# alxn3/nbody-llm

Hardware: AMD Instinct MI355X
Metric: pairwise_interactions_per_sec (higher is better)
Workload: dtype f32

## Files before the change

nbody-llm_amd/csrc/kernels.h:

```cpp
#pragma once
#include <hip/hip_runtime.h>
#include <cstdint>
#include <vector>

#include "shard.h"

namespace nbody {

struct Tuning {
    int cross_sym = 1;
    int sym_packed = 1;
    int bf_fast_variant = 0;
    int bh_walk_duo = -1;
    int bh_walk_xcd = 1;
    int let_list_div = 4;
    int sym_ipt = 0;
    int sym_wpb = 4;
    int sym_rounds = 1;
    int sym_k = 0;
    int sym_min_bodies = 1024;
    int sym_reduce_split = 1;
    int sym_opp_rot = 1;
    int cross_slots = 3072;
    int cross_ipt = 0;
    int cross_wpb = 4;
    int bh_walk_split = 0;
    int bh_walk_order = 1;
    int bh_reduce_split = 1;
    int tree_max_tie = 64;
    int bf64_min_bodies = 10240;
    int bf64_ipt = 0;
    int bf64_rot = 0;
    int bf64_waves = 0;
    int bh_walk_variant = 0;
    int bh_walk_lds_block = 1024;
    int bh_hot_cap = 2048;
    int bh_walk_debug = 0;
    int sym_debug = 0;
};
const Tuning& tuning();
struct WalkPlan { int bodies_per_lane; int segments; };
WalkPlan walk_plan(size_t n_order, bool fast_math, int max_segments, float theta2);
void bind_tuning(const Tuning* t);

template <class F>
void launch_aos_to_soa(hipStream_t s, const F* aos, int stride, int n, typename ShardT<F>::V4* pos, typename ShardT<F>::V4* vel,
                       typename ShardT<F>::V4* acc);
template <class F>
void launch_soa_to_aos(hipStream_t s, F* aos, int stride, int n, const typename ShardT<F>::V4* pos, const typename ShardT<F>::V4* vel,
                       const typename ShardT<F>::V4* acc);
template <class F> void launch_drift_half(hipStream_t s, const ShardT<F>& sh, int n_upper, F dt, const typename RealTypes<F>::Bounds& b);
template <class F> void launch_compact(hipStream_t s, const ShardT<F>& sh, int n_upper);
template <class F> void launch_kick_drift(hipStream_t s, const ShardT<F>& sh, int n_upper, F dt);

void launch_bf_forces_strict(hipStream_t s, const Shard& sh, int n_upper, float g, float g_soft2);
void launch_bf_forces_fast(hipStream_t s, const Shard& sh, int n_upper, float g, float g_soft2);

struct SymPlan {
    int ipt = 8;
    int A = 0;
    int K = 0;
    int wpb = 16;
    int res_combine = 0;
    int k_res = 0;
    int sym_sets = 0;
    int opp = 0;
    int n_trav = 0;
    int n_planes = 0;
    int k_os = 0;
    size_t n_pad = 0;
    size_t plane_stride = 0;
    std::vector<int> bounds;
    std::vector<int> bounds_long;
};
SymPlan make_sym_plan(int n_upper);
int sym_bodies_per_lane(size_t n);
uint64_t sym_main_pairs(const SymPlan& p, size_t n);
void launch_bf_sym_main(hipStream_t s, const Shard& sh, const SymPlan& p, const int* d_bounds, float4* planes,
                        int n_upper, float g_soft2);
void launch_bf_os(hipStream_t s, const Shard& sh, int A, int K, float4* planes, size_t plane_stride, float g_soft2);
void launch_bf_sym_tail(hipStream_t s, const Shard& sh, const SymPlan& p, float4* planes, int n_upper, float g,
                        float g_soft2, const float* kick_dt);

struct CrossPartners {
    static constexpr int kMax = 8;
    int n = 0;
    int seg[kMax];
    int c0[kMax], c1[kMax];
    int a0[kMax], a1[kMax];
};
struct CrossPlan {
    static constexpr int kMaxPlanes = 256;
    int ipt = 8;
    int A = 0;
    CrossPartners parts;
    int n_recv = 0;
    int recv_from[CrossPartners::kMax];
    int k_res = 0;
    std::vector<int4> slices;
};
CrossPlan make_cross_plan(int rank, int world, int seg_cap, int n_own_upper);
void launch_bf_cross(hipStream_t s, const Shard& sh, const CrossPlan& p, const int4* d_slices, float4* res_planes,
                     float4* xplanes, float4* send, size_t plane_stride, float g_soft2);

constexpr int kMaxSplit = 64, kMaxAnc = 192;
constexpr size_t kSplitInts = size_t(kMaxSplit) + 1 + kMaxSplit + size_t(kMaxSplit) * kMaxAnc;
struct TreeDev {
    const float4* nodes = nullptr;
    int n_nodes = 0;
    const int* order = nullptr;
    int n_order = 0;
    int n_split = 1;
    const int* split_first = nullptr;
    const int* split_anc = nullptr;
    const int* split_n_anc = nullptr;
    float4* split_planes = nullptr;
    size_t split_stride = 0;
    float4* nested_stack = nullptr;
    size_t nested_stride = 0;
    float4* walk = nullptr;
    float4* hot = nullptr;
    int* unified = nullptr;
    int* hot_info = nullptr;
    int hot_cap = 0;
    int hot_threshold = 0;
    const int* poison = nullptr;
    const int* n_order_dev = nullptr;
    int store_work = 0;
    float4* bfs = nullptr;
    void* bfs_ws = nullptr;
    size_t bfs_cap = 0;
};
struct TreeDevWork {
    const unsigned long long* keys = nullptr;
    const signed char* delta = nullptr;
    const int* base = nullptr;
    const int* ids = nullptr;
    const unsigned long long* keys2 = nullptr;
    const int* wpre = nullptr;
    const void* incl = nullptr;
};
struct TreeCatLists {
    int* flags = nullptr;
    int* base = nullptr;
    int* own_order = nullptr;
    int* info = nullptr;
};
template <class P4>
struct TreeCat : TreeCatLists {
    P4* pos = nullptr;
};
size_t tree_build_workspace_bytes(size_t n_cap);
size_t tree_build_tmp_bytes(size_t n_cap);
inline size_t tree_cat_align(size_t b) { return (b + 255) / 256 * 256; }
template <class P4> size_t tree_cat_bytes(size_t n_cap) { return tree_cat_align(n_cap * sizeof(P4)) + 3 * tree_cat_align(n_cap * 4) + 256; }
template <class P4>
TreeCat<P4> tree_cat_layout(void* buf, size_t n_cap) {
    char* p = static_cast<char*>(buf);
    TreeCat<P4> c;
    c.pos = reinterpret_cast<P4*>(p); p += tree_cat_align(n_cap * sizeof(P4));
    c.flags = reinterpret_cast<int*>(p); p += tree_cat_align(n_cap * 4);
    c.base = reinterpret_cast<int*>(p); p += tree_cat_align(n_cap * 4);
    c.own_order = reinterpret_cast<int*>(p); p += tree_cat_align(n_cap * 4);
    c.info = reinterpret_cast<int*>(p);
    return c;
}
void launch_tree_cat(hipStream_t s, const Shard& sh, const TreeCat<float4>& c);
void launch_tree_cat(hipStream_t s, const ShardT<double>& sh, const TreeCat<double4>& c);
int launch_tree_own_order(hipStream_t s, const int* order, const TreeCatLists& c, int n_total_upper, void* tmp, size_t tmp_bytes);
struct TreeSplitReq { int n_split = 0; int* first = nullptr; int* n_anc = nullptr; int* anc = nullptr; int max_anc = 0; const int* info = nullptr; int* poison = nullptr; };
int build_octree_device(hipStream_t s, const float4* pos, const int* d_count, int n_upper, const float center[3],
                        float width, void* workspace, size_t n_cap, float4* nodes, int node_cap, int* order,
                        int* out_info, TreeDevWork* work, int want_hot = 0 , const TreeSplitReq* split = nullptr);
size_t bfs_workspace_bytes(size_t n_cap);
int build_bfs_layout(hipStream_t s, const float4* nodes, int n_nodes, void* workspace, size_t n_cap, float4* out);
}
namespace nbody64 { struct Node64; }
namespace nbody {
int build_octree_device(hipStream_t s, const double4* pos, const int* d_count, int n_upper, const double center[3], double width,
                        void* workspace, size_t n_cap, nbody64::Node64* nodes, int node_cap, int* order, int* out_info,
                        TreeDevWork* work, int want_hot = 0, const TreeSplitReq* split = nullptr);
int tree_sort_keys(hipStream_t s, const float4* pos, const int* d_count, int n_upper, const float center[3], float width,
                   void* workspace, size_t n_cap, int* out_info, TreeDevWork* work);
int tree_emit_sorted(hipStream_t s, const float4* pos, const int* d_count, int n_upper, float width, void* workspace, size_t n_cap,
                     float4* nodes, int node_cap, int* order, int* out_info, int want_hot, const int* edge, const TreeSplitReq* split = nullptr);
int tree_scan_sorted(hipStream_t s, const float4* pos, const int* d_count, int n_upper, void* workspace, size_t n_cap, int* out_info,
                     const int* edge, const float4* weight_src = nullptr );
__host__ __device__ inline int body_weight(float visits) { const int v = int(visits) >> 4; return v < 1 ? 1 : v; }
int tree_emit_nodes(hipStream_t s, const float4* pos, const int* d_count, int n_upper, float width, void* workspace, size_t n_cap,
                    float4* nodes, int node_cap, int slice_cap, int* order, int* out_info, int want_hot, const int* edge,
                    const int* node_offset, int* parent, unsigned char* depth);
void launch_tree_split_anc(hipStream_t s, const TreeDevWork& work, int n, int n_nodes, int n_split, int* first,
                           int* n_anc, int* anc, int max_anc, const int* info = nullptr ,
                           int* poison = nullptr );

#define NBODY_WALK_COUNTER_SLOTS 1024u
void launch_walk_split_scan(hipStream_t s, const float4* nodes, const int* range, int n_split, int* first, int* n_anc, int* anc, int first_given = 0);
void launch_bh_walk(hipStream_t s, const Shard& sh, const TreeDev& t, float g, float g_soft2, float theta2,
                    int fast_math, unsigned long long* counters , int leaf_direct = 0,
                    const float* kick_dt = nullptr ,
                    int* kicked = nullptr );
void launch_bh_reduce(hipStream_t s, const Shard& sh, const TreeDev& t, int fast_math, const float* kick_dt, int* kicked);

void launch_energy(hipStream_t s, const Shard& sh, int n_upper, double g_soft2, double* out2);

}
```

nbody-llm_amd/csrc/kernels_bf_sym.hip:

```cpp
#include "kernels.h"
#include "bf_pair.h"
#include "real.h"

#include <algorithm>

namespace nbody {

namespace {

#ifdef NBODY_TUNING
__device__ unsigned long long nbody_sym_stamps[3 * 8192];
#endif

}

template <int IPT>
__device__ __forceinline__ void sym_rest_wave(const float4* __restrict__ pos, int n, int A, int opp, int group, int slice,
                                              int n_slices, float& ax, float& ay, float& az, float eps2);

template <int IPT, int NW>
__device__ __forceinline__ void sym_rest_block(const float4* __restrict__ pos, int n, int A, int opp, int group,
                                               float4* __restrict__ plane, float eps2, float (*red)[3][64]);

template <int IPT, int WPB, int DBG = 0, bool PK = false>
__global__ __launch_bounds__(WPB * 64) void k_bf_sym(const float4* __restrict__ pos, const int* __restrict__ count,
                                                     int A, int K, const int* __restrict__ bounds, int n_trav, int opp,
                                                     float4* __restrict__ planes, size_t plane_stride, float eps2,
                                                     int res_combine) {
    const int lane = threadIdx.x & 63;
    const int wslot = __builtin_amdgcn_readfirstlane(threadIdx.x >> 6);
    const int n_main_blocks = (A * K + WPB - 1) / WPB;
    if (int(blockIdx.x) >= n_main_blocks) {
        __shared__ float red[WPB - 1][3][64];
        sym_rest_block<IPT, WPB>(pos, *count, A, opp, blockIdx.x - n_main_blocks,
                                 planes + size_t(n_trav + (res_combine ? K / WPB : K)) * plane_stride, eps2, red);
        return;
    }
    const int gw = blockIdx.x * WPB + (wslot & 3) * (WPB / 4) + (wslot >> 2);
    if (gw >= A * K) return;
    const int a = gw / K;
    const int part = gw - a * K;
    const int n = *count;
    const int Cn = A * IPT;
    const int* __restrict__ cuts = bounds + ((opp && a < (A >> 1)) ? 128 : 0);
    const int k0 = cuts[part], k1 = cuts[part + 1];
    const int src_lane = ((lane + 63) & 63) * 4;
    const int src_lane2 = ((lane + 62) & 63) * 4;
    float eps2v = eps2;
    asm volatile("" : "+v"(eps2v));

    float xi[IPT], yi[IPT], zi[IPT], mi[IPT], axi[IPT], ayi[IPT], azi[IPT];
#pragma unroll
    for (int q = 0; q < IPT; ++q) {
        const int i = (a * IPT + q) * 64 + lane;
        const float4 p = (i < n) ? pos[i] : make_float4(PAD_POS, PAD_POS, PAD_POS, 0.f);
        xi[q] = p.x; yi[q] = p.y; zi[q] = p.z; mi[q] = p.w;
        axi[q] = ayi[q] = azi[q] = 0.f;
    }

    auto chunk_of = [&](int k) {
        int c = (a + 1) * IPT + k;
        if (c >= Cn) c -= Cn;
        return c;
    };
    auto load_chunk = [&](int k) {
        const int j = chunk_of(k) * 64 + lane;
        return (j < n) ? pos[j] : make_float4(PAD_POS, PAD_POS, PAD_POS, 0.f);
    };

    [[maybe_unused]] unsigned long long t_beg = 0, r_beg = 0;
    if (DBG & 4) { t_beg = __builtin_amdgcn_s_memtime(); r_beg = __builtin_amdgcn_s_memrealtime(); }
    float4 nxt = (k0 < k1) ? load_chunk(k0) : make_float4(0.f, 0.f, 0.f, 0.f);
    v2f xi2[IPT / 2], yi2[IPT / 2], zi2[IPT / 2], mi2[IPT / 2], axi2[IPT / 2], ayi2[IPT / 2], azi2[IPT / 2];
    if (PK) {
        pack_pairs<IPT>(xi, xi2); pack_pairs<IPT>(yi, yi2); pack_pairs<IPT>(zi, zi2); pack_pairs<IPT>(mi, mi2);
        pack_pairs<IPT>(axi, axi2); pack_pairs<IPT>(ayi, ayi2); pack_pairs<IPT>(azi, azi2);
    }
    for (int k = k0; k < k1; ++k) {
        float xj = nxt.x, yj = nxt.y, zj = nxt.z, mj = nxt.w;
        float axj = 0.f, ayj = 0.f, azj = 0.f;
        v2f axj2 = {0.f, 0.f}, ayj2 = {0.f, 0.f}, azj2 = {0.f, 0.f};
        if (k + 1 < k1) nxt = load_chunk(k + 1);
        switch ((4 * (k1 - k) - 1) / (k1 - k0)) {
            case 3: __builtin_amdgcn_s_setprio(3); break;
            case 2: __builtin_amdgcn_s_setprio(2); break;
            case 1: __builtin_amdgcn_s_setprio(1); break;
            default: __builtin_amdgcn_s_setprio(0); break;
        }
        if (PK) {
            for (int s = 0; s < 64; s += 2) {
                const float x1 = rotl(xj, src_lane), y1 = rotl(yj, src_lane), z1 = rotl(zj, src_lane), m1 = rotl(mj, src_lane);
                pair_evals_pk<IPT / 2, DBG>(xi2, yi2, zi2, mi2, axi2, ayi2, azi2, xj, yj, zj, mj, axj2, ayj2, azj2, eps2v);
                axj2.x = rotl(axj2.x, src_lane); ayj2.x = rotl(ayj2.x, src_lane); azj2.x = rotl(azj2.x, src_lane);
                axj2.y = rotl(axj2.y, src_lane); ayj2.y = rotl(ayj2.y, src_lane); azj2.y = rotl(azj2.y, src_lane);
                xj = rotl(x1, src_lane); yj = rotl(y1, src_lane); zj = rotl(z1, src_lane); mj = rotl(m1, src_lane);
                pair_evals_pk<IPT / 2, DBG>(xi2, yi2, zi2, mi2, axi2, ayi2, azi2, x1, y1, z1, m1, axj2, ayj2, azj2, eps2v);
                axj2.x = rotl(axj2.x, src_lane); ayj2.x = rotl(ayj2.x, src_lane); azj2.x = rotl(azj2.x, src_lane);
                axj2.y = rotl(axj2.y, src_lane); ayj2.y = rotl(ayj2.y, src_lane); azj2.y = rotl(azj2.y, src_lane);
            }
        } else {
            float x1 = rotl(xj, src_lane), y1 = rotl(yj, src_lane), z1 = rotl(zj, src_lane), m1 = rotl(mj, src_lane);
#pragma unroll 2
            for (int s = 0; s < 64; ++s) {
                const float x2 = rotl(xj, src_lane2), y2 = rotl(yj, src_lane2), z2 = rotl(zj, src_lane2), m2 = rotl(mj, src_lane2);
                pair_evals<IPT, DBG>(xi, yi, zi, mi, axi, ayi, azi, xj, yj, zj, mj, axj, ayj, azj, eps2v);
                axj = rotl(axj, src_lane); ayj = rotl(ayj, src_lane); azj = rotl(azj, src_lane);
                xj = x1; yj = y1; zj = z1; mj = m1;
                x1 = x2; y1 = y2; z1 = z2; m1 = m2;
            }
        }
        if (PK) { axj = axj2.x + axj2.y; ayj = ayj2.x + ayj2.y; azj = azj2.x + azj2.y; }
        const int d = k / IPT + 1;
        planes[size_t(d - 1) * plane_stride + size_t(chunk_of(k)) * 64 + lane] = make_float4(axj, ayj, azj, 0.f);
    }
    if (PK) { unpack_pairs<IPT>(axi2, axi); unpack_pairs<IPT>(ayi2, ayi); unpack_pairs<IPT>(azi2, azi); }

#ifdef NBODY_TUNING
    if (DBG & 4) {
        const unsigned long long t_end = __builtin_amdgcn_s_memtime(), r_end = __builtin_amdgcn_s_memrealtime();
        if (lane == 0 && gw < 8192) {
            nbody_sym_stamps[gw * 3 + 0] = t_end - t_beg;
            nbody_sym_stamps[gw * 3 + 1] = r_end - r_beg;
            const unsigned hw = __builtin_amdgcn_s_getreg((4 ) | (0 << 6) | (31 << 11));
            const unsigned xcc = __builtin_amdgcn_s_getreg((20 ) | (0 << 6) | (31 << 11));
            nbody_sym_stamps[gw * 3 + 2] = (unsigned long long)(k1 - k0) | ((unsigned long long)hw << 16) | ((unsigned long long)(xcc & 0xF) << 48);
        }
    }
#endif
    if (res_combine) {
        __shared__ float comb[WPB - 1][3 * IPT][64];
        const int first_part = (part / WPB) * WPB;
        const int rel = part - first_part;
        if (rel > 0) {
#pragma unroll
            for (int q = 0; q < IPT; ++q) {
                comb[rel - 1][3 * q + 0][lane] = axi[q];
                comb[rel - 1][3 * q + 1][lane] = ayi[q];
                comb[rel - 1][3 * q + 2][lane] = azi[q];
            }
        }
        __syncthreads();
        if (rel == 0) {
            float4* __restrict__ out = planes + size_t(n_trav + part / WPB) * plane_stride;
#pragma unroll
            for (int q = 0; q < IPT; ++q) {
                float sx = axi[q], sy = ayi[q], sz = azi[q];
                for (int w = 0; w < WPB - 1; ++w) { sx += comb[w][3 * q + 0][lane]; sy += comb[w][3 * q + 1][lane]; sz += comb[w][3 * q + 2][lane]; }
                out[size_t(a * IPT + q) * 64 + lane] = make_float4(sx, sy, sz, 0.f);
            }
        }
        return;
    }
    float4* __restrict__ out = planes + size_t(n_trav + part) * plane_stride;
#pragma unroll
    for (int q = 0; q < IPT; ++q) out[size_t(a * IPT + q) * 64 + lane] = make_float4(axi[q], ayi[q], azi[q], 0.f);
}

template <int IPT, int WPB, bool PK>
__global__ __launch_bounds__(WPB * 64) void k_bf_os(const float4* __restrict__ pos_all,
                                                    const int* __restrict__ seg_count, int n_seg, int seg_cap,
                                                    int my_seg, int A, int K, float4* __restrict__ planes,
                                                    size_t plane_stride, float eps2) {
    __shared__ float4 stage[WPB][2][64];
    const int lane = threadIdx.x & 63;
    const int wslot = __builtin_amdgcn_readfirstlane(threadIdx.x >> 6);
    const int gw = blockIdx.x * WPB + (wslot & 3) * (WPB / 4) + (wslot >> 2);
    if (gw >= A * K) return;
    const int a = gw / K, part = gw - a * K;
    const int n_own = seg_count[my_seg];
    const float4* __restrict__ own = pos_all + size_t(my_seg) * seg_cap;
    float eps2v = eps2;
    asm volatile("" : "+v"(eps2v));

    float xi[IPT], yi[IPT], zi[IPT], mi[IPT], axi[IPT], ayi[IPT], azi[IPT];
#pragma unroll
    for (int q = 0; q < IPT; ++q) {
        const int i = (a * IPT + q) * 64 + lane;
        const float4 p = (i < n_own) ? own[i] : make_float4(PAD_POS, PAD_POS, PAD_POS, 0.f);
        xi[q] = p.x; yi[q] = p.y; zi[q] = p.z; mi[q] = p.w;
        axi[q] = ayi[q] = azi[q] = 0.f;
    }
    long long R = 0;
    for (int s = 0; s < n_seg; ++s) if (s != my_seg) R += seg_count[s];
    const long long r0 = R * part / K, r1 = R * (part + 1) / K;
    long long seg_first = 0;
    float dummy_x = 0.f, dummy_y = 0.f, dummy_z = 0.f;
    v2f dummy2 = {0.f, 0.f};
    v2f xi2[IPT / 2], yi2[IPT / 2], zi2[IPT / 2], mi2[IPT / 2], axi2[IPT / 2], ayi2[IPT / 2], azi2[IPT / 2];
    if (PK) {
        pack_pairs<IPT>(xi, xi2); pack_pairs<IPT>(yi, yi2); pack_pairs<IPT>(zi, zi2); pack_pairs<IPT>(mi, mi2);
        pack_pairs<IPT>(axi, axi2); pack_pairs<IPT>(ayi, ayi2); pack_pairs<IPT>(azi, azi2);
    }
    for (int s = 0; s < n_seg; ++s) {
        if (s == my_seg) continue;
        const int ns = seg_count[s];
        const long long lo = r0 > seg_first ? r0 : seg_first;
        const long long hi = r1 < seg_first + ns ? r1 : seg_first + ns;
        const float4* __restrict__ ps = pos_all + size_t(s) * seg_cap - seg_first;
        int buf = 0;
        if (lo < hi) {
            const long long j = lo + lane;
            stage[wslot][0][lane] = (j < hi) ? ps[j] : make_float4(PAD_POS, PAD_POS, PAD_POS, 0.f);
        }
        for (long long c0 = lo; c0 < hi; c0 += 64) {
            const long long jn = c0 + 64 + lane;
            float4 nxt = make_float4(PAD_POS, PAD_POS, PAD_POS, 0.f);
            if (c0 + 64 < hi && jn < hi) nxt = ps[jn];
            const int cnt = int(hi - c0 < 64 ? hi - c0 : 64);
            switch (int((4 * (r1 - c0) - 1) / (r1 - r0))) {
                case 3: __builtin_amdgcn_s_setprio(3); break;
                case 2: __builtin_amdgcn_s_setprio(2); break;
                case 1: __builtin_amdgcn_s_setprio(1); break;
                default: __builtin_amdgcn_s_setprio(0); break;
            }
            float4 pj = stage[wslot][buf][0];
            for (int t = 0; t < cnt; ++t) {
                const float4 pn = stage[wslot][buf][(t + 1) & 63];
                if (PK)
                    pair_evals_pk<IPT / 2, 0, false>(xi2, yi2, zi2, mi2, axi2, ayi2, azi2, pj.x, pj.y, pj.z, pj.w, dummy2,
                                                     dummy2, dummy2, eps2v);
                else
                    pair_evals<IPT, 0, false>(xi, yi, zi, mi, axi, ayi, azi, pj.x, pj.y, pj.z, pj.w, dummy_x, dummy_y,
                                              dummy_z, eps2v);
                pj = pn;
            }
            buf ^= 1;
            stage[wslot][buf][lane] = nxt;
        }
        seg_first += ns;
    }
    if (PK) { unpack_pairs<IPT>(axi2, axi); unpack_pairs<IPT>(ayi2, ayi); unpack_pairs<IPT>(azi2, azi); }
    float4* __restrict__ out = planes + size_t(part) * plane_stride;
#pragma unroll
    for (int q = 0; q < IPT; ++q) out[size_t(a * IPT + q) * 64 + lane] = make_float4(axi[q], ayi[q], azi[q], 0.f);
}

template <int IPT>
__device__ __forceinline__ void sym_rest_wave(const float4* __restrict__ pos, int n, int A, int opp, int group, int slice,
                                              int n_slices, float& ax, float& ay, float& az, float eps2) {
    constexpr int SET = 64 * IPT;
    const int lane = threadIdx.x & 63;
    const int i = group * 64 + lane;
    const int a = (group * 64) / SET;
    const float4 pi = (i < n) ? pos[i] : make_float4(PAD_POS, PAD_POS, PAD_POS, 0.f);
    ax = ay = az = 0.f;
    const int n_win = (A % 2 == 0 && A > 1 && !opp) ? 2 : 1;
    for (int w = 0; w < n_win; ++w) {
        int set = (w == 0) ? a : a + A / 2;
        if (set >= A) set -= A;
        const int j0 = set * SET + SET * slice / n_slices;
        const int j1 = min(n, set * SET + SET * (slice + 1) / n_slices);
#pragma unroll 8
        for (int j = j0; j < j1; ++j) {
            const float4 pj = pos[j];
            const float dx = pj.x - pi.x, dy = pj.y - pi.y, dz = pj.z - pi.z;
            const float r2 = __builtin_fmaf(dz, dz, __builtin_fmaf(dy, dy, __builtin_fmaf(dx, dx, eps2)));
            const float rinv = __builtin_amdgcn_rsqf(r2);
            float sj = pj.w * ((rinv * rinv) * rinv);
            sj = (j == i) ? 0.f : sj;
            ax = __builtin_fmaf(dx, sj, ax);
            ay = __builtin_fmaf(dy, sj, ay);
            az = __builtin_fmaf(dz, sj, az);
        }
    }
}

template <int IPT, int NW>
__device__ __forceinline__ void sym_rest_block(const float4* __restrict__ pos, int n, int A, int opp, int group,
                                               float4* __restrict__ plane, float eps2, float (*red)[3][64]) {
    const int lane = threadIdx.x & 63;
    const int wv = __builtin_amdgcn_readfirstlane(threadIdx.x >> 6);
    float ax, ay, az;
    sym_rest_wave<IPT>(pos, n, A, opp, group, wv, NW, ax, ay, az, eps2);
    if (wv > 0) { red[wv - 1][0][lane] = ax; red[wv - 1][1][lane] = ay; red[wv - 1][2][lane] = az; }
    __syncthreads();
    if (wv == 0) {
#pragma unroll
        for (int w = 0; w < NW - 1; ++w) { ax += red[w][0][lane]; ay += red[w][1][lane]; az += red[w][2][lane]; }
        plane[group * 64 + lane] = make_float4(ax, ay, az, 0.f);
    }
}

template <int IPT>
__global__ __launch_bounds__(512) void k_bf_sym_rest(const float4* __restrict__ pos, const int* __restrict__ count,
                                                     int A, float4* __restrict__ plane, float eps2) {
    __shared__ float red[7][3][64];
    sym_rest_block<IPT, 8>(pos, *count, A, 0, blockIdx.x, plane, eps2, red);
}

template <bool KICK>
__global__ __launch_bounds__(256) void k_bf_sym_reduce(const float4* __restrict__ planes, int n_planes,
                                                       size_t plane_stride, const int* __restrict__ count, float g,
                                                       float4* __restrict__ acc, float4* __restrict__ pos,
                                                       float4* __restrict__ vel, float dt, const int* __restrict__ seg_count,
                                                       int n_seg, unsigned long long* __restrict__ inter, int opp_plane,
                                                       int opp_first) {
    const int i = blockIdx.x * 256 + threadIdx.x;
    if (inter && i == 0) {
        long long tot = 0;
        for (int s = 0; s < n_seg; ++s) tot += seg_count[s];
        if (tot > 0) atomicAdd(inter, (unsigned long long)(*count) * (unsigned long long)(tot - 1));
    }
    if (i >= *count) return;
    float sx = 0.f, sy = 0.f, sz = 0.f, cx = 0.f, cy = 0.f, cz = 0.f;
    for (int p = 0; p < n_planes; ++p) {
        if (p == opp_plane && i < opp_first) continue;
        const float4 v = planes[size_t(p) * plane_stride + i];
        const float yx = v.x - cx, yy = v.y - cy, yz = v.z - cz;
        const float tx = sx + yx, ty = sy + yy, tz = sz + yz;
        cx = (tx - sx) - yx; cy = (ty - sy) - yy; cz = (tz - sz) - yz;
        sx = tx; sy = ty; sz = tz;
    }
    const float4 a = make_float4(g * sx, g * sy, g * sz, 0.f);
    acc[i] = a;
    if (KICK) kick_half_drift(pos, vel, i, a.x, a.y, a.z, dt);
}

template <bool KICK, int Q>
__global__ __launch_bounds__(64 * Q) void k_bf_sym_reduce_split(const float4* __restrict__ planes, int n_planes, size_t plane_stride,
                                                                const int* __restrict__ count, float g, float4* __restrict__ acc,
                                                                float4* __restrict__ pos, float4* __restrict__ vel, float dt,
                                                                const int* __restrict__ seg_count, int n_seg,
                                                                unsigned long long* __restrict__ inter, int opp_plane, int opp_first) {
    __shared__ float part[Q][3][64];
    const int lane = threadIdx.x & 63, q = threadIdx.x >> 6;
    const int i = blockIdx.x * 64 + lane;
    if (inter && blockIdx.x == 0 && threadIdx.x == 0) {
        long long tot = 0;
        for (int s = 0; s < n_seg; ++s) tot += seg_count[s];
        if (tot > 0) atomicAdd(inter, (unsigned long long)(*count) * (unsigned long long)(tot - 1));
    }
    const int n = *count;
    float sx = 0.f, sy = 0.f, sz = 0.f, cx = 0.f, cy = 0.f, cz = 0.f;
    if (i < n) {
        const int p0 = int((long long)n_planes * q / Q), p1 = int((long long)n_planes * (q + 1) / Q);
        for (int p = p0; p < p1; ++p) {
            if (p == opp_plane && i < opp_first) continue;
            const float4 v = planes[size_t(p) * plane_stride + i];
            const float yx = v.x - cx, yy = v.y - cy, yz = v.z - cz;
            const float tx = sx + yx, ty = sy + yy, tz = sz + yz;
            cx = (tx - sx) - yx; cy = (ty - sy) - yy; cz = (tz - sz) - yz;
            sx = tx; sy = ty; sz = tz;
        }
    }
    part[q][0][lane] = sx; part[q][1][lane] = sy; part[q][2][lane] = sz;
    __syncthreads();
    if (q != 0 || i >= n) return;
    sx = sy = sz = cx = cy = cz = 0.f;
    for (int w = 0; w < Q; ++w) {
        const float yx = part[w][0][lane] - cx, yy = part[w][1][lane] - cy, yz = part[w][2][lane] - cz;
        const float tx = sx + yx, ty = sy + yy, tz = sz + yz;
        cx = (tx - sx) - yx; cy = (ty - sy) - yy; cz = (tz - sz) - yz;
        sx = tx; sy = ty; sz = tz;
    }
    const float4 a = make_float4(g * sx, g * sy, g * sz, 0.f);
    acc[i] = a;
    if (KICK) kick_half_drift(pos, vel, i, a.x, a.y, a.z, dt);
}

}
#ifdef NBODY_TUNING
namespace nbody { int read_sym_stamps(unsigned long long* out, int n_waves); }
extern "C" int nbody_sym_read_stamps(unsigned long long* out, int n_waves) { return nbody::read_sym_stamps(out, n_waves); }
#endif
namespace nbody {

int sym_bodies_per_lane(size_t n) {
    const Tuning& t = tuning();
    if (!t.sym_packed || t.sym_wpb != 4 || t.sym_ipt == 8) return 8;
    if (t.sym_ipt == 4) return 4;
    return n <= 10240 ? 4 : 8;
}

SymPlan make_sym_plan(int n_upper) {
    SymPlan p;
    const int IPT = sym_bodies_per_lane(size_t(n_upper));
    p.ipt = IPT;
    p.A = (n_upper + 64 * IPT - 1) / (64 * IPT);
    p.sym_sets = (p.A + 1) / 2 - 1;
    const int L = IPT * p.sym_sets;
    const int want = tuning().sym_wpb;
    p.wpb = want == 8 ? 8 : want == 12 ? 12 : want == 16 ? 16 : 4;
    int K = 1;
    if (p.wpb == 4) {
        K = L <= 100 ? L : L <= 160 ? (L + 1) / 2 : 64;
    } else {
        const int resident_wgs_per_cu = (p.wpb == 8) ? 2 : 1;
        const int slots = 256 * resident_wgs_per_cu * p.wpb;
        double best = 0.0;
        const int k_hi = std::min(126, std::min(L, std::max(1, slots * std::max(1, tuning().sym_rounds) * 4 / p.A)));
        for (int k = 1; k <= k_hi; ++k) {
            const long long waves = (long long)p.A * k;
            const long long rounds = (waves + slots - 1) / slots;
            if (rounds > 4 * std::max(1, tuning().sym_rounds) && k > 1) break;
            const double fill = double(waves) / double(rounds * slots);
            const double even = (L % k == 0) ? 1.0 : double(L / k) / double(L / k + 1);
            const double per_wave = double(L) / k / (double(L) / k + 0.3);
            if (fill * even * per_wave > best + 1e-9) { best = fill * even * per_wave; K = k; }
        }
    }
    if (tuning().sym_k > 0) K = std::min(126, tuning().sym_k);
    if (K > L) K = L;
    if (K < 1) K = 1;
    p.K = K;
    p.res_combine = (K % p.wpb == 0) ? 1 : 0;
    p.k_res = p.res_combine ? K / p.wpb : K;
    p.opp = (tuning().sym_opp_rot && p.A % 2 == 0 && p.sym_sets >= 1) ? 1 : 0;
    p.n_trav = p.sym_sets + p.opp;
    p.n_planes = p.n_trav + p.k_res + 1;
    p.n_pad = size_t(p.A) * 64 * IPT;
    p.plane_stride = p.n_pad;
    p.bounds.resize(K + 1);
    for (int part = 0; part <= K; ++part) p.bounds[part] = int((long long)L * part / K);
    const int L_long = L + (p.opp ? IPT : 0);
    p.bounds_long.resize(K + 1);
    for (int part = 0; part <= K; ++part) p.bounds_long[part] = int((long long)L_long * part / K);
    return p;
}

#ifdef NBODY_TUNING
int read_sym_stamps(unsigned long long* out, int n_waves) {
    return hipMemcpyFromSymbol(out, HIP_SYMBOL(nbody_sym_stamps), sizeof(unsigned long long) * 3 * n_waves) == hipSuccess ? 0 : -1;
}
#endif

uint64_t sym_main_pairs(const SymPlan& p, size_t n) {
    const size_t set = size_t(64) * p.ipt;
    auto size_of = [&](int a) { size_t lo = size_t(a) * set; return lo >= n ? size_t(0) : std::min(set, n - lo); };
    uint64_t pairs = 0;
    for (int a = 0; a < p.A; ++a)
        for (int d = 1; d <= p.sym_sets; ++d) pairs += uint64_t(size_of(a)) * uint64_t(size_of((a + d) % p.A));
    if (p.opp)
        for (int a = 0; a < p.A / 2; ++a) pairs += uint64_t(size_of(a)) * uint64_t(size_of(a + p.A / 2));
    return pairs;
}

void launch_bf_sym_main(hipStream_t s, const Shard& sh, const SymPlan& p, const int* d_bounds, float4* planes,
                        int n_upper, float g_soft2) {
    if (n_upper <= 0 || p.sym_sets <= 0) return;
    const int main_blocks = (p.A * p.K + p.wpb - 1) / p.wpb;
    const int rest_blocks = int(p.n_pad / 64);
    const dim3 grid(main_blocks + rest_blocks), block(p.wpb * 64);
#define SYM_LAUNCH(WPB, DBG) hipLaunchKernelGGL((k_bf_sym<8, WPB, DBG, PKV>), grid, block, 0, s, sh.own_pos(), sh.own_count(), p.A, p.K, d_bounds, p.n_trav, p.opp, planes, p.plane_stride, g_soft2, p.res_combine)
#ifdef NBODY_TUNING
    const int dbg = tuning().sym_debug;
#else
    constexpr int dbg = 0;
#endif
    if (p.ipt == 4) {
        hipLaunchKernelGGL((k_bf_sym<4, 4, 0, true>), grid, block, 0, s, sh.own_pos(), sh.own_count(), p.A, p.K, d_bounds, p.n_trav, p.opp, planes, p.plane_stride, g_soft2, p.res_combine);
        return;
    }
    if (tuning().sym_packed) {
        constexpr bool PKV = true;
        if (dbg == 4) {
#ifdef NBODY_TUNING
            if (p.wpb == 12) SYM_LAUNCH(12, 4); else if (p.wpb == 8) SYM_LAUNCH(8, 4); else if (p.wpb == 4) SYM_LAUNCH(4, 4); else SYM_LAUNCH(16, 4);
#endif
        } else {
            if (p.wpb == 12) SYM_LAUNCH(12, 0); else if (p.wpb == 8) SYM_LAUNCH(8, 0); else if (p.wpb == 4) SYM_LAUNCH(4, 0); else SYM_LAUNCH(16, 0);
        }
    } else {
        constexpr bool PKV = false;
        if (dbg >= 4 && dbg <= 7) {
#ifdef NBODY_TUNING
            if (dbg == 4) { if (p.wpb == 12) SYM_LAUNCH(12, 4); else if (p.wpb == 8) SYM_LAUNCH(8, 4); else if (p.wpb == 4) SYM_LAUNCH(4, 4); else SYM_LAUNCH(16, 4); }
            else if (dbg == 5) SYM_LAUNCH(16, 5);
            else if (dbg == 6) SYM_LAUNCH(16, 6);
            else SYM_LAUNCH(16, 7);
#endif
        } else {
            if (p.wpb == 12) SYM_LAUNCH(12, 0); else if (p.wpb == 8) SYM_LAUNCH(8, 0); else if (p.wpb == 4) SYM_LAUNCH(4, 0); else SYM_LAUNCH(16, 0);
        }
    }
#undef SYM_LAUNCH
}

void launch_bf_os(hipStream_t s, const Shard& sh, int A, int K, float4* planes, size_t plane_stride, float g_soft2) {
    if (A <= 0 || K <= 0) return;
    const int wpb = 12;
    if (tuning().sym_packed)
        hipLaunchKernelGGL((k_bf_os<8, 12, true>), dim3((A * K + wpb - 1) / wpb), dim3(wpb * 64), 0, s, sh.pos_all,
                           sh.seg_count, sh.n_seg, sh.seg_cap, sh.my_seg, A, K, planes, plane_stride, g_soft2);
    else
        hipLaunchKernelGGL((k_bf_os<8, 12, false>), dim3((A * K + wpb - 1) / wpb), dim3(wpb * 64), 0, s, sh.pos_all,
                           sh.seg_count, sh.n_seg, sh.seg_cap, sh.my_seg, A, K, planes, plane_stride, g_soft2);
}

void launch_bf_sym_tail(hipStream_t s, const Shard& sh, const SymPlan& p, float4* planes, int n_upper, float g,
                        float g_soft2, const float* kick_dt) {
    if (n_upper <= 0) return;
    if (p.sym_sets == 0) {
        float4* resident0 = planes + size_t(p.n_trav) * p.plane_stride;
        (void)hipMemsetAsync(resident0, 0, size_t(p.k_res) * p.plane_stride * sizeof(float4), s);
        if (p.ipt == 4)
            hipLaunchKernelGGL(k_bf_sym_rest<4>, dim3(int(p.n_pad / 64)), dim3(512), 0, s, sh.own_pos(),
                               sh.own_count(), p.A, planes + size_t(p.n_trav + p.k_res) * p.plane_stride, g_soft2);
        else
        hipLaunchKernelGGL(k_bf_sym_rest<8>, dim3(int(p.n_pad / 64)), dim3(512), 0, s, sh.own_pos(),
                           sh.own_count(), p.A, planes + size_t(p.n_trav + p.k_res) * p.plane_stride, g_soft2);
    }
    const float dt = kick_dt ? *kick_dt : 0.f;
#define REDUCE_ARGS planes, p.n_planes, p.plane_stride, sh.own_count(), g, sh.acc, sh.own_pos(), sh.vel, dt, sh.seg_count, sh.n_seg, sh.inter, (p.opp ? p.n_trav - 1 : -1), int(p.n_pad / 2)
    if (tuning().sym_reduce_split && p.n_planes >= 16) {
        const dim3 grid((n_upper + 63) / 64);
        if (n_upper <= 16384) {
            if (kick_dt) hipLaunchKernelGGL((k_bf_sym_reduce_split<true, 16>), grid, dim3(1024), 0, s, REDUCE_ARGS);
            else hipLaunchKernelGGL((k_bf_sym_reduce_split<false, 16>), grid, dim3(1024), 0, s, REDUCE_ARGS);
        } else {
            if (kick_dt) hipLaunchKernelGGL((k_bf_sym_reduce_split<true, 4>), grid, dim3(256), 0, s, REDUCE_ARGS);
            else hipLaunchKernelGGL((k_bf_sym_reduce_split<false, 4>), grid, dim3(256), 0, s, REDUCE_ARGS);
        }
    } else {
        const dim3 grid((n_upper + 255) / 256);
        if (kick_dt) hipLaunchKernelGGL(k_bf_sym_reduce<true>, grid, dim3(256), 0, s, REDUCE_ARGS);
        else hipLaunchKernelGGL(k_bf_sym_reduce<false>, grid, dim3(256), 0, s, REDUCE_ARGS);
    }
#undef REDUCE_ARGS
}

}
```

nbody-llm_amd/csrc/kernels_integrate.hip:

```cpp
#include "real.h"
#include "retain.h"

#include <algorithm>

namespace nbody {

template <class F>
__global__ __launch_bounds__(256) void k_aos_to_soa(const F* __restrict__ aos, int stride, int n, typename Real<F>::V4* __restrict__ pos,
                                                    typename Real<F>::V4* __restrict__ vel, typename Real<F>::V4* __restrict__ acc) {
    const int k = blockIdx.x * 256 + threadIdx.x;
    if (k >= n) return;
    const F* p = aos + size_t(k) * stride;
    pos[k] = Real<F>::make4(p[0], p[1], p[2], p[9]);
    if (vel) vel[k] = Real<F>::make4(p[3], p[4], p[5], F(0));
    if (acc) acc[k] = Real<F>::make4(p[6], p[7], p[8], F(0));
}

template <class F>
__global__ __launch_bounds__(256) void k_soa_to_aos(F* __restrict__ aos, int stride, int n, const typename Real<F>::V4* __restrict__ pos,
                                                    const typename Real<F>::V4* __restrict__ vel,
                                                    const typename Real<F>::V4* __restrict__ acc) {
    const int k = blockIdx.x * 256 + threadIdx.x;
    if (k >= n) return;
    const typename Real<F>::V4 p = pos[k], v = vel[k], a = acc[k];
    F* o = aos + size_t(k) * stride;
    o[0] = p.x; o[1] = p.y; o[2] = p.z;
    o[3] = v.x; o[4] = v.y; o[5] = v.z;
    o[6] = a.x; o[7] = a.y; o[8] = a.z;
    o[9] = p.w;
}

template <class F>
__global__ __launch_bounds__(256) void k_drift_half(typename Real<F>::V4* __restrict__ pos, const typename Real<F>::V4* __restrict__ vel,
                                                    const int* __restrict__ count, unsigned char* __restrict__ keep,
                                                    int* __restrict__ escaped, F dt, typename Real<F>::Bounds b,
                                                    const int* __restrict__ poison) {
    if (poison && *poison) return;
    const int k = blockIdx.x * 256 + threadIdx.x;
    if (k >= *count) return;
    typename Real<F>::V4 p = pos[k];
    const typename Real<F>::V4 v = vel[k];
    p.x += (v.x * Real<F>::half) * dt;
    p.y += (v.y * Real<F>::half) * dt;
    p.z += (v.z * Real<F>::half) * dt;
    pos[k] = p;
    const bool in = (p.x >= b.lo[0]) && (p.x <= b.hi[0]) && (p.y >= b.lo[1]) && (p.y <= b.hi[1]) &&
                    (p.z >= b.lo[2]) && (p.z <= b.hi[2]);
    keep[k] = in ? 1 : 0;
    if (!in) atomicAdd(escaped, 1);
}

template <class F>
__global__ __launch_bounds__(256) void k_kick_drift(typename Real<F>::V4* __restrict__ pos, typename Real<F>::V4* __restrict__ vel,
                                                    const typename Real<F>::V4* __restrict__ acc, const int* __restrict__ count,
                                                    F dt, int* __restrict__ poison) {
    if (poison && *poison) return;
    const int k = blockIdx.x * 256 + threadIdx.x;
    if (k == 0 && poison) atomicAdd(poison + 1, 1);
    if (k >= *count) return;
    typename Real<F>::V4 p = pos[k], v = vel[k];
    const typename Real<F>::V4 a = acc[k];
    v.x += a.x * dt;
    v.y += a.y * dt;
    v.z += a.z * dt;
    p.x += (v.x * Real<F>::half) * dt;
    p.y += (v.y * Real<F>::half) * dt;
    p.z += (v.z * Real<F>::half) * dt;
    vel[k] = v;
    pos[k] = p;
}

template <class F>
__global__ __launch_bounds__(kCompactTile) void k_compact(typename Real<F>::V4* __restrict__ pos, typename Real<F>::V4* __restrict__ vel,
                                                          typename Real<F>::V4* __restrict__ acc, const unsigned char* __restrict__ keep,
                                                          int* __restrict__ count, int* __restrict__ escaped,
                                                          unsigned long long* __restrict__ tile_state, int* __restrict__ epoch_p,
                                                          const int* __restrict__ poison, int* __restrict__ ids) {
    if (poison && *poison) return;
    if (*escaped == 0) return;
    typename Real<F>::V4 p = Real<F>::make4(0, 0, 0, 0), v = p, a = p;
    int id = 0;
    retain_tile(keep, count, escaped, tile_state, epoch_p,
                [&](int k) { p = pos[k]; v = vel[k]; a = acc[k]; if (ids) id = ids[k]; },
                [&](int d) { pos[d] = p; vel[d] = v; acc[d] = a; if (ids) ids[d] = id; });
}

static inline int blocks_for(int n, int bs) { return n <= 0 ? 0 : (n + bs - 1) / bs; }

template <class F>
void launch_aos_to_soa(hipStream_t s, const F* aos, int stride, int n, typename ShardT<F>::V4* pos, typename ShardT<F>::V4* vel,
                       typename ShardT<F>::V4* acc) {
    if (n <= 0) return;
    hipLaunchKernelGGL(k_aos_to_soa<F>, dim3(blocks_for(n, 256)), dim3(256), 0, s, aos, stride, n, pos, vel, acc);
}
template <class F>
void launch_soa_to_aos(hipStream_t s, F* aos, int stride, int n, const typename ShardT<F>::V4* pos, const typename ShardT<F>::V4* vel,
                       const typename ShardT<F>::V4* acc) {
    if (n <= 0) return;
    hipLaunchKernelGGL(k_soa_to_aos<F>, dim3(blocks_for(n, 256)), dim3(256), 0, s, aos, stride, n, pos, vel, acc);
}
template <class F>
void launch_drift_half(hipStream_t s, const ShardT<F>& sh, int n_upper, F dt, const typename RealTypes<F>::Bounds& b) {
    if (n_upper <= 0) return;
    hipLaunchKernelGGL(k_drift_half<F>, dim3(blocks_for(n_upper, 256)), dim3(256), 0, s, sh.own_pos(), sh.vel, sh.own_count(), sh.keep,
                       sh.escaped, dt, b, sh.poison);
}
template <class F>
void launch_compact(hipStream_t s, const ShardT<F>& sh, int n_upper) {
    if (n_upper <= 0) return;
    hipLaunchKernelGGL(k_compact<F>, dim3(blocks_for(n_upper, kCompactTile)), dim3(kCompactTile), 0, s, sh.own_pos(), sh.vel, sh.acc,
                       sh.keep, sh.own_count(), sh.escaped, sh.tile_state, sh.epoch, sh.poison, sh.ids);
}
template <class F>
void launch_kick_drift(hipStream_t s, const ShardT<F>& sh, int n_upper, F dt) {
    const int blocks = blocks_for(n_upper, 256);
    if (blocks == 0 && !sh.poison) return;
    hipLaunchKernelGGL(k_kick_drift<F>, dim3(std::max(1, blocks)), dim3(256), 0, s, sh.own_pos(), sh.vel, sh.acc, sh.own_count(), dt,
                       sh.poison);
}

#define NBODY_INTEGRATE_LAUNCHERS(F, V4)                                                                              \
    template void launch_aos_to_soa<F>(hipStream_t, const F*, int, int, V4*, V4*, V4*);                               \
    template void launch_soa_to_aos<F>(hipStream_t, F*, int, int, const V4*, const V4*, const V4*);                   \
    template void launch_drift_half<F>(hipStream_t, const ShardT<F>&, int, F, const RealTypes<F>::Bounds&);           \
    template void launch_compact<F>(hipStream_t, const ShardT<F>&, int);                                              \
    template void launch_kick_drift<F>(hipStream_t, const ShardT<F>&, int, F);
NBODY_INTEGRATE_LAUNCHERS(float, float4)
NBODY_INTEGRATE_LAUNCHERS(double, double4)
#undef NBODY_INTEGRATE_LAUNCHERS

}

namespace nbody64 {
void launch_aos_to_pos(hipStream_t s, const double* aos, int stride_d, int n, double4* pos) {
    nbody::launch_aos_to_soa<double>(s, aos, stride_d, n, pos, nullptr, nullptr);
}
}
```

nbody-llm_amd/csrc/nbody_api.cpp:

```cpp
#include "nbody_engine.h"
#include "nbody_let.h"
#include "nbody_pot.h"
#include "nbody_field.h"
#include "nbody_tracer.h"
#include "nbody_external.h"
#include "nbody_diag.h"
#include "nbody_pairs.h"
#include "nbody_fof.h"
#include "nbody_cells.h"

#include <algorithm>
#include <chrono>
#include <cmath>
#include <cstdio>
#include <cstdlib>
#include <cstring>
#include <memory>
#include <string>
#include <thread>
#include <vector>


static thread_local std::string g_create_err;

int fail(NbodyHandle* h, int code, const std::string& msg) {
    if (h) h->err = msg; else g_create_err = msg;
    return code;
}

int comm_check(NbodyHandle* h) {
    if (!h->tp) return NBODY_OK;
    int rc = h->tp->check();
    return rc ? fail(h, rc, h->tp->error()) : NBODY_OK;
}

namespace {

int use_device(NbodyHandle* h) {
    nbody::bind_tuning(&h->tune);
    HIP_TRY(h, hipSetDevice(h->device));
    return NBODY_OK;
}

int check_stride(NbodyHandle* h, size_t stride) {
    const size_t e = h->f64 ? sizeof(double) : sizeof(float);
    if (stride >= 10 * e && stride % e == 0) return NBODY_OK;
    return fail(h, NBODY_ERR_INVALID, h->f64 ? "f64 handle: stride must be a multiple of 8 and >= 80 bytes" : "stride must be a multiple of 4 and >= 40 bytes");
}

const char* tree_quadrupole_refusal(const NbodyHandle* h) {
    if (h->cfg.method != NBODY_BARNES_HUT) return "this mode needs a Barnes-Hut handle (brute-force handles have no tree to expand)";
    if (h->f64 || h->cfg.dtype != NBODY_F32) return "this mode is not possible on NBODY_F64 handles (the cells' tensors exist for NBODY_F32)";
    if (h->let || h->cfg.shard_mode != NBODY_SHARD_INDEX) return "this mode is not possible on NBODY_SHARD_SPATIAL handles";
    if (h->cfg.world_size != 1) return "this mode is not possible on handles of a multi-rank world (world_size > 1)";
    return nullptr;
}

int potentials_device(NbodyHandle* h, int mode, size_t* n_own, nbody::PotBodies* bodies, double* g, bool field = false) {
    if (mode != NBODY_POTENTIAL_PAIRS && mode != NBODY_POTENTIAL_TREE && mode != NBODY_POTENTIAL_TREE_QUADRUPOLE)
        return fail(h, NBODY_ERR_INVALID, "mode must be NBODY_POTENTIAL_PAIRS, NBODY_POTENTIAL_TREE or NBODY_POTENTIAL_TREE_QUADRUPOLE");
    if (mode == NBODY_POTENTIAL_TREE_QUADRUPOLE)
        if (const char* why = tree_quadrupole_refusal(h)) return fail(h, NBODY_ERR_INVALID, std::string("NBODY_POTENTIAL_TREE_QUADRUPOLE: ") + why);
    if (h->let && field)
        return fail(h, NBODY_ERR_INVALID, "nbody_field_at is not possible on NBODY_SHARD_SPATIAL handles: a rank holds neither the world's bodies nor the tree around a foreign point");
    if (h->let && mode == NBODY_POTENTIAL_PAIRS)
        return fail(h, NBODY_ERR_INVALID, "NBODY_POTENTIAL_PAIRS is not possible on NBODY_SHARD_SPATIAL handles (a rank does not hold the world's bodies): NBODY_POTENTIAL_TREE is the mode for them");
    if (mode != NBODY_POTENTIAL_PAIRS && h->cfg.method != NBODY_BARNES_HUT) return fail(h, NBODY_ERR_INVALID, "NBODY_POTENTIAL_TREE needs a Barnes-Hut handle");
    if (h->f64) return nbody64::potentials_device(h, mode, n_own, bodies, g, field);
    return nbody32::potentials_device(h, mode, n_own, bodies, g, field);
}

void free_all(NbodyHandle* h) {
    if (!h) return;
    (void)hipSetDevice(h->device);
    if (h->stream) (void)hipStreamSynchronize(h->stream);
    if (h->comm_stream) (void)hipStreamSynchronize(h->comm_stream);
    h->tp.reset();
    if (h->ev_drifted) (void)hipEventDestroy(h->ev_drifted);
    if (h->ev_gathered) (void)hipEventDestroy(h->ev_gathered);
    if (h->comm_stream) (void)hipStreamDestroy(h->comm_stream);
    for (auto& ev : h->ev_pending) { (void)hipEventDestroy(ev.first); (void)hipEventDestroy(ev.second); }
    for (auto& ev : h->ev_free) { (void)hipEventDestroy(ev.first); (void)hipEventDestroy(ev.second); }
    nbody::let::destroy(h);
    nbody32::destroy(h);
    nbody64::destroy(h);
    h->mem.release_all();
    if (h->stream) (void)hipStreamDestroy(h->stream);
    delete h;
}

int create_impl(const NbodyConfig* cfg, NbodyHandle** out) {
    if (!cfg || !out) return fail(nullptr, NBODY_ERR_INVALID, "null argument");
    constexpr uint32_t kOldConfigSize = 48;
    NbodyConfig full{};
    if (cfg->struct_size == kOldConfigSize) { std::memcpy(&full, cfg, kOldConfigSize); full.struct_size = sizeof(NbodyConfig); cfg = &full; }
    if (cfg->struct_size != sizeof(NbodyConfig)) return fail(nullptr, NBODY_ERR_INVALID, "NbodyConfig.struct_size mismatch");
    if (cfg->shard_mode != NBODY_SHARD_INDEX && cfg->shard_mode != NBODY_SHARD_SPATIAL) return fail(nullptr, NBODY_ERR_INVALID, "unknown shard_mode");
    if (cfg->shard_mode == NBODY_SHARD_SPATIAL && (cfg->method != NBODY_BARNES_HUT || cfg->math_mode != NBODY_MATH_FAST || cfg->dtype != NBODY_F32))
        return fail(nullptr, NBODY_ERR_INVALID, "NBODY_SHARD_SPATIAL is the fast-math f32 Barnes-Hut path (halo exchange over the device-built tree)");
    if (cfg->method != NBODY_BRUTE_FORCE && cfg->method != NBODY_BARNES_HUT) return fail(nullptr, NBODY_ERR_INVALID, "unknown method");
    if (cfg->math_mode != NBODY_MATH_STRICT && cfg->math_mode != NBODY_MATH_FAST) return fail(nullptr, NBODY_ERR_INVALID, "unknown math_mode");
    if (cfg->leaf_mode != NBODY_LEAF_REFERENCE && cfg->leaf_mode != NBODY_LEAF_DIRECT) return fail(nullptr, NBODY_ERR_INVALID, "unknown leaf_mode");
    if (cfg->tree_build != NBODY_TREE_HOST && cfg->tree_build != NBODY_TREE_DEVICE && cfg->tree_build != NBODY_TREE_AUTO)
        return fail(nullptr, NBODY_ERR_INVALID, "unknown tree_build");
    if (cfg->world_size < 1 || cfg->rank < 0 || cfg->rank >= cfg->world_size) return fail(nullptr, NBODY_ERR_INVALID, "bad rank/world_size");
    if (cfg->capacity == 0 || cfg->capacity > (1ull << 30)) return fail(nullptr, NBODY_ERR_INVALID, "capacity must be in [1, 2^30]");
    if (cfg->dtype != NBODY_F32 && cfg->dtype != NBODY_F64) return fail(nullptr, NBODY_ERR_INVALID, "unknown dtype");
    if (cfg->dtype == NBODY_F64 && cfg->world_size != 1 && cfg->shard_mode != NBODY_SHARD_INDEX)
        return fail(nullptr, NBODY_ERR_INVALID, "f64 worlds are sharded by index blocks (NBODY_SHARD_INDEX)");

    int ndev = 0;
    if (hipGetDeviceCount(&ndev) != hipSuccess || ndev <= 0)
        return fail(nullptr, NBODY_ERR_NO_DEVICE, "no HIP device (this library has no CPU fallback)");
    int dev = cfg->device;
    if (dev < 0) {
        const char* lr = std::getenv("LOCAL_RANK");
        dev = lr ? std::atoi(lr) % ndev : 0;
    }
    if (dev >= ndev) return fail(nullptr, NBODY_ERR_INVALID, "device ordinal out of range");

    NbodyHandle* h = new NbodyHandle();
    h->cfg = *cfg;
    if (h->cfg.tree_build == NBODY_TREE_AUTO)
        h->cfg.tree_build = cfg->math_mode == NBODY_MATH_FAST ? NBODY_TREE_DEVICE : NBODY_TREE_HOST;
    if (h->cfg.dtype == NBODY_F64) {
        if (cfg->tree_build == NBODY_TREE_AUTO) h->cfg.tree_build = h->cfg.math_mode == NBODY_MATH_FAST ? NBODY_TREE_DEVICE : NBODY_TREE_HOST;
        if (cfg->world_size > 1 && h->cfg.math_mode != NBODY_MATH_FAST) h->cfg.tree_build = NBODY_TREE_HOST;
    }
    if (h->cfg.shard_mode == NBODY_SHARD_SPATIAL) h->cfg.tree_build = NBODY_TREE_DEVICE;
    cfg = &h->cfg;
    h->device = dev;
    *out = nullptr;
    auto bail = [&](int rc) { g_create_err = h->err; free_all(h); return rc; };
#define CREATE_TRY(expr)                                                                                  \
    do {                                                                                                  \
        const int rc_ = [&] { HIP_TRY(h, expr); return int(NBODY_OK); }();                                \
        if (rc_) return bail(rc_);                                                                        \
    } while (0)
    CREATE_TRY(hipSetDevice(dev));
    CREATE_TRY(hipStreamCreateWithFlags(&h->stream, hipStreamNonBlocking));
    CREATE_TRY(h->mem.pin(h->h_poison, 8 * sizeof(int)));
    if (cfg->method == NBODY_BARNES_HUT) {
        int threads = cfg->host_threads > 0 ? cfg->host_threads : std::min(16, std::max(1, int(std::thread::hardware_concurrency()) - 2));
        h->pool.reset(new nbody::WorkerPool(std::max(1, threads)));
        CREATE_TRY(h->mem.dev(h->d_counters, 2 * NBODY_WALK_COUNTER_SLOTS * sizeof(unsigned long long)));
        CREATE_TRY(hipMemsetAsync(h->d_counters, 0, 2 * NBODY_WALK_COUNTER_SLOTS * sizeof(unsigned long long), h->stream));
        CREATE_TRY(h->mem.pin(h->h_counters, 2 * NBODY_WALK_COUNTER_SLOTS * sizeof(unsigned long long)));
    }
#undef CREATE_TRY
    ShardShape& sh = h->shape;
    sh.n_seg = cfg->world_size;
    sh.my_seg = cfg->rank;
    sh.seg_cap = int((cfg->capacity + cfg->world_size - 1) / cfg->world_size);
    if (cfg->dtype == NBODY_F64) {
        int rc64 = nbody64::create(h);
        if (rc64) return bail(rc64);
        *out = h;
        return NBODY_OK;
    }
    const bool spatial = cfg->shard_mode == NBODY_SHARD_SPATIAL;
    if (spatial) {
        sh.n_seg = 1;
        sh.my_seg = 0;
        if (cfg->world_size > 1) sh.seg_cap = int(std::min<uint64_t>(cfg->capacity, 4 * uint64_t(sh.seg_cap) + 64));
    }
    {
        int rc = nbody32::create(h);
        if (rc) return bail(rc);
    }
    if (spatial) {
        int rc_let = nbody::let::create(h);
        if (rc_let) return bail(rc_let);
    }
    {
        nbody::Tuning& t = h->tune;
        const struct { const char* env; int* knob; } table[] = {
            {"NBODY_BF_VARIANT", &t.bf_fast_variant}, {"NBODY_CROSS_SYM", &t.cross_sym}, {"NBODY_SYM_PACKED", &t.sym_packed},
            {"NBODY_BH_SPLIT", &t.bh_walk_split}, {"NBODY_SYM_WPB", &t.sym_wpb}, {"NBODY_SYM_IPT", &t.sym_ipt}, {"NBODY_BH_DUO", &t.bh_walk_duo}, {"NBODY_BH_XCD", &t.bh_walk_xcd},
#ifdef NBODY_TUNING
            {"NBODY_BH_VARIANT", &t.bh_walk_variant}, {"NBODY_BH_HOT", &t.bh_hot_cap}, {"NBODY_BH_LDS_BLOCK", &t.bh_walk_lds_block},
#endif
        };
        for (const auto& e : table)
            if (const char* v = std::getenv(e.env)) *e.knob = std::atoi(v);
    }
    *out = h;
    return NBODY_OK;
}

}

extern "C" {

int nbody_abi_version(void) { return NBODY_ABI_VERSION; }

int nbody_device_count(void) {
    int n = 0;
    if (hipGetDeviceCount(&n) != hipSuccess) return 0;
    return n;
}

const char* nbody_last_error(const NbodyHandle* h) { return h ? h->err.c_str() : g_create_err.c_str(); }

int nbody_create(const NbodyConfig* cfg, NbodyHandle** out) { return create_impl(cfg, out); }

void nbody_destroy(NbodyHandle* h) { free_all(h); }

int nbody_clone(const NbodyHandle* src, NbodyHandle** out) {
    if (!src || !out) return fail(nullptr, NBODY_ERR_INVALID, "null argument");
    NbodyHandle* s = const_cast<NbodyHandle*>(src);
    int rc = use_device(s);
    if (rc) return rc;
    rc = nbody32::resolve_async(s);
    if (rc) return rc;
    NbodyHandle* h = nullptr;
    rc = create_impl(&src->cfg, &h);
    if (rc) return rc;
    h->tune = src->tune;
    h->ext = src->ext;
    if (src->f64) rc = nbody64::clone_state(s, h);
    else {
        rc = nbody32::clone_state(s, h);
        if (!rc && src->let) rc = nbody::let::clone_state(s, h);
        if (!rc) rc = nbody::tracer::clone_state(s, h);
    }
    if (rc) { g_create_err = h->err; free_all(h); return rc; }
    *out = h;
    return NBODY_OK;
}

int nbody_upload(NbodyHandle* h, const void* aos, size_t n, size_t stride) {
    if (!h || (!aos && n)) return fail(h, NBODY_ERR_INVALID, "null argument");
    int rc = check_stride(h, stride);
    if (rc) return rc;
    if (n > h->cfg.capacity) return fail(h, NBODY_ERR_CAPACITY, "more bodies than NbodyConfig.capacity");
    rc = use_device(h);
    if (rc) return rc;
    if (h->f64) return nbody64::upload(h, aos, n, stride);
    if (h->let) return nbody::let::upload(h, aos, n, stride);
    return nbody32::upload(h, aos, n, stride);
}

int nbody_download(NbodyHandle* h, void* aos, size_t cap, size_t stride, size_t* n_out) {
    if (!h) return NBODY_ERR_INVALID;
    int rc = check_stride(h, stride);
    if (rc) return rc;
    rc = use_device(h);
    if (rc) return rc;
    if (h->f64) return nbody64::download(h, aos, cap, stride, n_out);
    return nbody32::download(h, aos, cap, stride, n_out);
}

int nbody_count(NbodyHandle* h, size_t* n_out) {
    if (!h || !n_out) return NBODY_ERR_INVALID;
    int rc = use_device(h);
    if (rc) return rc;
    if (h->f64) return nbody64::count(h, n_out);
    return nbody32::count(h, n_out);
}

int nbody_count_global(NbodyHandle* h, size_t* n_out) {
    if (!h || !n_out) return NBODY_ERR_INVALID;
    int rc = use_device(h);
    if (rc) return rc;
    if (h->f64) return nbody64::count_global(h, n_out);
    if (h->let) return nbody::let::count_global(h, n_out);
    return nbody32::count_global(h, n_out);
}

int nbody_add_point(NbodyHandle* h, const void* particle) {
    if (!h || !particle) return NBODY_ERR_INVALID;
    int rc = use_device(h);
    if (rc) return rc;
    if (h->f64) return nbody64::add_point(h, particle);
    if (h->let) return nbody::let::add_point(h, particle);
    return nbody32::add_point(h, particle);
}

int nbody_remove_point(NbodyHandle* h, size_t index) {
    if (!h) return NBODY_ERR_INVALID;
    int rc = use_device(h);
    if (rc) return rc;
    if (h->f64) return nbody64::remove_point(h, index);
    if (h->let) return nbody::let::remove_point(h, index);
    return nbody32::remove_point(h, index);
}

int nbody_set_settings_f64(NbodyHandle* h, double g, double g_soft, double dt, double theta2) {
    if (!h) return NBODY_ERR_INVALID;
    if (h->f64) return nbody64::set_settings(h, g, g_soft, dt, theta2);
    nbody32::bodies(h).set_settings(float(g), float(g_soft), float(dt), float(theta2));
    return NBODY_OK;
}

int nbody_set_settings(NbodyHandle* h, float g, float g_soft, float dt, float theta2) {
    return nbody_set_settings_f64(h, double(g), double(g_soft), double(dt), double(theta2));
}

int nbody_get_settings_f64(const NbodyHandle* h, double* g, double* g_soft, double* dt, double* theta2) {
    if (!h) return NBODY_ERR_INVALID;
    return with_bodies(h, [&](const auto& b) { b.get_settings(g, g_soft, dt, theta2); return int(NBODY_OK); });
}

int nbody_get_settings(const NbodyHandle* h, float* g, float* g_soft, float* dt, float* theta2) {
    if (!h) return NBODY_ERR_INVALID;
    return with_bodies(h, [&](const auto& b) { b.get_settings(g, g_soft, dt, theta2); return int(NBODY_OK); });
}

int nbody_set_bounds_f64(NbodyHandle* h, const double center[3], double width) {
    if (!h || !center) return NBODY_ERR_INVALID;
    if (h->f64) return nbody64::set_bounds(h, center, width);
    const float c[3] = {float(center[0]), float(center[1]), float(center[2])};
    nbody32::bodies(h).set_bounds(c, float(width));
    return NBODY_OK;
}

int nbody_set_bounds(NbodyHandle* h, const float center[3], float width) {
    if (!h || !center) return NBODY_ERR_INVALID;
    const double c[3] = {double(center[0]), double(center[1]), double(center[2])};
    return nbody_set_bounds_f64(h, c, double(width));
}

int nbody_init(NbodyHandle* h) {
    if (!h) return NBODY_ERR_INVALID;
    if (h->f64) return nbody64::init(h);
    return nbody32::init(h);
}

int nbody_step_by(NbodyHandle* h, float dt) {
    if (!h) return NBODY_ERR_INVALID;
    int rc = use_device(h);
    if (rc) return rc;
    if (h->f64) return nbody64::step_by(h, double(dt));
    if (h->let) return nbody::let::step(h, dt);
    return nbody32::step_by(h, dt);
}

int nbody_step_by_f64(NbodyHandle* h, double dt) {
    if (!h) return NBODY_ERR_INVALID;
    int rc = use_device(h);
    if (rc) return rc;
    if (h->f64) return nbody64::step_by(h, dt);
    if (h->let) return nbody::let::step(h, float(dt));
    return nbody32::step_by(h, float(dt));
}

int nbody_steps(NbodyHandle* h, int k) {
    if (!h || k < 0) return NBODY_ERR_INVALID;
    int rc = use_device(h);
    if (rc) return rc;
    if (h->f64) return nbody64::steps(h, k);
    if (h->let) {
        for (int i = 0; i < k; ++i) { rc = nbody::let::step(h, nbody32::bodies(h).dt); if (rc) return rc; }
        return NBODY_OK;
    }
    return nbody32::steps(h, k);
}

int nbody_update_forces(NbodyHandle* h) {
    if (!h) return NBODY_ERR_INVALID;
    int rc = use_device(h);
    if (rc) return rc;
    if (h->f64) return nbody64::update_forces(h);
    if (h->let) return nbody32::bodies(h).bounds_set ? nbody::let::update_forces(h) : fail(h, NBODY_ERR_INVALID, "nbody_set_bounds has not been called");
    return nbody32::update_forces(h);
}

namespace {
int external_enter(NbodyHandle* h, const char* call) {
    int rc = use_device(h);
    if (rc) return rc;
    if (const char* why = nbody::ext::refusal(h)) return fail(h, NBODY_ERR_INVALID, std::string(call) + ": " + why);
    return nbody32::resolve_async(h);
}
double g_of(const NbodyHandle* h) { return with_bodies(h, [](const auto& b) { return double(b.g); }); }
int external_potentials(NbodyHandle* h, bool want_phi, double* phi, size_t cap, size_t* n_out, double* energy, const char* call) {
    return with_bodies(h, [&](auto& b) {
        const int rc = b.sync_count(h, h->stream);
        if (rc) return rc;
        const size_t n = b.n_local;
        if (n_out) *n_out = n;
        if (want_phi && n > cap) return fail(h, NBODY_ERR_CAPACITY, std::string(call) + ": buffer too small");
        if (want_phi && n && !phi) return fail(h, NBODY_ERR_INVALID, std::string(call) + ": phi is NULL");
        return nbody::ext::potentials(h, b.sh, n, double(b.g), phi, energy);
    });
}
}

int nbody_set_external_field(NbodyHandle* h, const NbodyExternalComponent* comps, size_t n) {
    if (!h) return NBODY_ERR_INVALID;
    int rc = external_enter(h, "nbody_set_external_field");
    if (rc) return rc;
    const std::string why = nbody::ext::invalid(comps, n, !h->f64);
    if (!why.empty()) return fail(h, NBODY_ERR_INVALID, "nbody_set_external_field: " + why);
    if (n > 0 && h->f64 && nbody64::get_integrator(h) == NBODY_INTEGRATOR_HERMITE4)
        return fail(h, NBODY_ERR_INVALID, "nbody_set_external_field: the handle runs the Hermite integrator, which would need the field's jerk (out of scope)");
    h->ext = ExternalField{};
    h->ext.n = int(n);
    std::copy(comps, comps + n, h->ext.given);
    return NBODY_OK;
}

int nbody_get_external_field(const NbodyHandle* h, NbodyExternalComponent* comps, size_t cap, size_t* n_out) {
    if (!h) return NBODY_ERR_INVALID;
    NbodyHandle* hh = const_cast<NbodyHandle*>(h);
    if (const char* why = nbody::ext::refusal(h)) return fail(hh, NBODY_ERR_INVALID, std::string("nbody_get_external_field: ") + why);
    const size_t n = size_t(h->ext.n);
    if (n_out) *n_out = n;
    if (n > cap) return fail(hh, NBODY_ERR_CAPACITY, "nbody_get_external_field: buffer too small");
    if (n && !comps) return fail(hh, NBODY_ERR_INVALID, "nbody_get_external_field: comps is NULL");
    std::copy(h->ext.given, h->ext.given + n, comps);
    return NBODY_OK;
}

int nbody_external_potentials(NbodyHandle* h, double* phi, size_t cap, size_t* n_out) {
    if (!h) return NBODY_ERR_INVALID;
    int rc = external_enter(h, "nbody_external_potentials");
    if (rc) return rc;
    return external_potentials(h, true, phi, cap, n_out, nullptr, "nbody_external_potentials");
}

int nbody_external_energy(NbodyHandle* h, double* potential) {
    if (!h) return NBODY_ERR_INVALID;
    int rc = external_enter(h, "nbody_external_energy");
    if (rc) return rc;
    if (!potential) return fail(h, NBODY_ERR_INVALID, "nbody_external_energy: potential is NULL");
    return external_potentials(h, false, nullptr, 0, nullptr, potential, "nbody_external_energy");
}

int nbody_external_at(NbodyHandle* h, const double* xyz, size_t n_points, double* acc, double* phi) {
    if (!h) return NBODY_ERR_INVALID;
    int rc = external_enter(h, "nbody_external_at");
    if (rc) return rc;
    if (n_points > (size_t(1) << 30)) return fail(h, NBODY_ERR_INVALID, "nbody_external_at: n_points must not exceed 2^30");
    if (!xyz && n_points > 0) return fail(h, NBODY_ERR_INVALID, "nbody_external_at: xyz is NULL");
    return nbody::ext::at(h, g_of(h), xyz, n_points, acc, phi);
}

namespace {
int diag_enter(NbodyHandle* h, const char* call) {
    int rc = use_device(h);
    if (rc) return rc;
    if (const char* why = nbody::diag::refusal(h)) return fail(h, NBODY_ERR_INVALID, std::string(call) + ": " + why);
    return nbody32::resolve_async(h);
}
}

int nbody_moments(NbodyHandle* h, double out[10]) {
    if (!h) return NBODY_ERR_INVALID;
    int rc = diag_enter(h, "nbody_moments");
    if (rc) return rc;
    if (!out) return fail(h, NBODY_ERR_INVALID, "nbody_moments: out is NULL");
    return with_bodies(h, [&](auto& b) { return nbody::diag::moments(h, b.sh, b.n_local, out); });
}

int nbody_lagrangian_radii(NbodyHandle* h, const double center[3], const double* fractions, size_t n_frac, double* radii, double* mass_out) {
    if (!h) return NBODY_ERR_INVALID;
    int rc = diag_enter(h, "nbody_lagrangian_radii");
    if (rc) return rc;
    if (n_frac > (size_t(1) << 20)) return fail(h, NBODY_ERR_INVALID, "nbody_lagrangian_radii: n_frac must not exceed 2^20");
    if (n_frac > 0 && !fractions) return fail(h, NBODY_ERR_INVALID, "nbody_lagrangian_radii: fractions is NULL");
    if (n_frac > 0 && !radii) return fail(h, NBODY_ERR_INVALID, "nbody_lagrangian_radii: radii is NULL");
    for (size_t k = 0; k < n_frac; ++k)
        if (!(fractions[k] >= 0.0 && fractions[k] <= 1.0))
            return fail(h, NBODY_ERR_INVALID, "nbody_lagrangian_radii: fraction " + std::to_string(k) + " is not in [0, 1]");
    return with_bodies(h, [&](auto& b) { return nbody::diag::lagrangian_radii(h, b.sh, b.n_local, center, fractions, n_frac, radii, mass_out); });
}

int nbody_partners(NbodyHandle* h, int32_t* partner, double* energy, size_t cap, size_t* n_out) {
    if (!h) return NBODY_ERR_INVALID;
    int rc = diag_enter(h, "nbody_partners");
    if (rc) return rc;
    return with_bodies(h, [&](auto& b) { return nbody::pairs::partners(h, b.sh, b.n_local, double(b.g), double(b.g_soft), partner, energy, cap, n_out); });
}

int nbody_bound_pairs(NbodyHandle* h, NbodyBoundPair* pairs, size_t cap, size_t* n_pairs, double* binding_sum) {
    if (!h) return NBODY_ERR_INVALID;
    int rc = diag_enter(h, "nbody_bound_pairs");
    if (rc) return rc;
    return with_bodies(h, [&](auto& b) { return nbody::pairs::bound_pairs(h, b.sh, b.n_local, double(b.g), double(b.g_soft), pairs, cap, n_pairs, binding_sum); });
}

namespace {
int contact_radius(NbodyHandle* h, const char* call, double radius) {
    if (std::isfinite(radius) && radius > 0.0) return NBODY_OK;
    return fail(h, NBODY_ERR_INVALID, std::string(call) + ": radius must be finite and > 0");
}
}

int nbody_nearest(NbodyHandle* h, int32_t* nearest, double* dist2, size_t cap, size_t* n_out) {
    if (!h) return NBODY_ERR_INVALID;
    int rc = diag_enter(h, "nbody_nearest");
    if (rc) return rc;
    return with_bodies(h, [&](auto& b) { return nbody::pairs::nearest(h, b.sh, b.n_local, nearest, dist2, cap, n_out); });
}

int nbody_contacts(NbodyHandle* h, double radius, NbodyContact* list, size_t cap, size_t* n_contacts) {
    if (!h) return NBODY_ERR_INVALID;
    int rc = diag_enter(h, "nbody_contacts");
    if (!rc) rc = contact_radius(h, "nbody_contacts", radius);
    if (rc) return rc;
    return with_bodies(h, [&](auto& b) { return nbody::pairs::contacts(h, b.sh, b.n_local, radius, list, cap, n_contacts); });
}

int nbody_merge_contacts(NbodyHandle* h, double radius, NbodyContact* list, size_t cap, size_t* n_contacts) {
    if (!h) return NBODY_ERR_INVALID;
    int rc = diag_enter(h, "nbody_merge_contacts");
    if (!rc) rc = contact_radius(h, "nbody_merge_contacts", radius);
    if (rc) return rc;
    if (h->f64) return nbody64::merge_contacts(h, radius, list, cap, n_contacts);
    return nbody32::merge_contacts(h, radius, list, cap, n_contacts);
}

namespace {
int fof_enter(NbodyHandle* h, const char* call, double linking_length) {
    int rc = diag_enter(h, call);
    if (rc) return rc;
    if (std::isfinite(linking_length) && linking_length > 0.0) return NBODY_OK;
    return fail(h, NBODY_ERR_INVALID, std::string(call) + ": linking_length must be finite and > 0");
}
}

int nbody_fof_labels(NbodyHandle* h, double linking_length, int32_t* label, size_t cap, size_t* n_out, size_t* n_groups_out) {
    if (!h) return NBODY_ERR_INVALID;
    int rc = fof_enter(h, "nbody_fof_labels", linking_length);
    if (rc) return rc;
    return with_bodies(h, [&](auto& b) { return nbody::fof::labels(h, b.sh, b.n_local, linking_length, label, cap, n_out, n_groups_out); });
}

int nbody_fof_groups(NbodyHandle* h, double linking_length, int min_members, NbodyGroup* groups, size_t group_cap, size_t* n_groups,
                     int32_t* members, size_t member_cap, size_t* n_members) {
    if (!h) return NBODY_ERR_INVALID;
    int rc = fof_enter(h, "nbody_fof_groups", linking_length);
    if (rc) return rc;
    if (min_members < 1) return fail(h, NBODY_ERR_INVALID, "nbody_fof_groups: min_members must be >= 1");
    return with_bodies(h, [&](auto& b) {
        return nbody::fof::groups(h, b.sh, b.n_local, linking_length, min_members, groups, group_cap, n_groups, members, member_cap, n_members);
    });
}

namespace {
int search_refusal(NbodyHandle* h, const char* call) {
    if (const char* why = nbody::diag::refusal(h)) return fail(h, NBODY_ERR_INVALID, std::string(call) + ": " + why);
    return NBODY_OK;
}
}

int nbody_set_pair_search(NbodyHandle* h, int mode) {
    if (!h) return NBODY_ERR_INVALID;
    if (int rc = search_refusal(h, "nbody_set_pair_search")) return rc;
    if (mode != NBODY_SEARCH_ALL_PAIRS && mode != NBODY_SEARCH_CELLS)
        return fail(h, NBODY_ERR_INVALID, "nbody_set_pair_search: mode must be NBODY_SEARCH_ALL_PAIRS (0) or NBODY_SEARCH_CELLS (1)");
    h->search.mode = mode;
    return NBODY_OK;
}

int nbody_get_pair_search(const NbodyHandle* h, int* mode) {
    if (!h) return NBODY_ERR_INVALID;
    NbodyHandle* hh = const_cast<NbodyHandle*>(h);
    if (int rc = search_refusal(hh, "nbody_get_pair_search")) return rc;
    if (!mode) return fail(hh, NBODY_ERR_INVALID, "nbody_get_pair_search: mode is NULL");
    *mode = h->search.mode;
    return NBODY_OK;
}

int nbody_pair_search_stats(NbodyHandle* h, uint64_t out[4]) {
    if (!h) return NBODY_ERR_INVALID;
    if (int rc = search_refusal(h, "nbody_pair_search_stats")) return rc;
    if (!out) return fail(h, NBODY_ERR_INVALID, "nbody_pair_search_stats: out is NULL");
    std::copy(h->search.last, h->search.last + 4, out);
    return NBODY_OK;
}

int nbody_host_cell_grid(const double* xyz, size_t n, double length, double lo[3], double* side, uint64_t* key, int* usable) {
    if ((!xyz && n) || !lo || !side || !usable) return NBODY_ERR_INVALID;
    if (!(std::isfinite(length) && length > 0.0)) return NBODY_ERR_INVALID;
    nbody::cells::Grid g;
    (void)nbody::cells::host_grid(xyz, n, 3, length, &g, key);
    std::copy(g.lo, g.lo + 3, lo);
    *side = g.side;
    *usable = g.usable;
    return NBODY_OK;
}

namespace {
int tracer_enter(NbodyHandle* h, const char* call) {
    int rc = use_device(h);
    if (rc) return rc;
    if (const char* why = nbody::tracer::refusal(h)) return fail(h, NBODY_ERR_INVALID, std::string(call) + ": " + why);
    return nbody32::resolve_async(h);
}
}

int nbody_tracers_upload(NbodyHandle* h, const void* aos, size_t n, size_t stride, size_t capacity) {
    if (!h) return NBODY_ERR_INVALID;
    int rc = tracer_enter(h, "nbody_tracers_upload");
    if (rc) return rc;
    if (!aos && n) return fail(h, NBODY_ERR_INVALID, "nbody_tracers_upload: null argument");
    if (stride < 40 || stride % 4) return fail(h, NBODY_ERR_INVALID, "nbody_tracers_upload: stride must be a multiple of 4 and >= 40 bytes");
    return nbody::tracer::upload(h, aos, n, stride, capacity);
}

int nbody_tracers_download(NbodyHandle* h, void* aos, size_t cap, size_t stride, size_t* n_out) {
    if (!h) return NBODY_ERR_INVALID;
    int rc = tracer_enter(h, "nbody_tracers_download");
    if (rc) return rc;
    if (stride < 40 || stride % 4) return fail(h, NBODY_ERR_INVALID, "nbody_tracers_download: stride must be a multiple of 4 and >= 40 bytes");
    return nbody::tracer::download(h, aos, cap, stride, n_out);
}

int nbody_tracers_count(NbodyHandle* h, size_t* n_out) {
    if (!h) return NBODY_ERR_INVALID;
    int rc = tracer_enter(h, "nbody_tracers_count");
    if (rc) return rc;
    if (!n_out) return fail(h, NBODY_ERR_INVALID, "nbody_tracers_count: null argument");
    return nbody::tracer::count(h, n_out);
}

int nbody_tracer_stats(NbodyHandle* h, uint64_t out[2]) {
    if (!h) return NBODY_ERR_INVALID;
    int rc = tracer_enter(h, "nbody_tracer_stats");
    if (rc) return rc;
    if (!out) return fail(h, NBODY_ERR_INVALID, "nbody_tracer_stats: null argument");
    return nbody::tracer::stats(h, out);
}

int nbody_host_tracer_plan(size_t n_tracers, size_t n_bodies, int out[4]) {
    if (!out) return NBODY_ERR_INVALID;
    const nbody::TracerPlan p = nbody::tracer_plan(n_tracers, n_bodies);
    out[0] = p.ipt; out[1] = p.groups; out[2] = p.K; out[3] = p.slice_len;
    return NBODY_OK;
}

int nbody_elapsed(const NbodyHandle* h, float* out) {
    if (!h || !out) return NBODY_ERR_INVALID;
    *out = with_bodies(h, [](const auto& b) { return float(b.elapsed); });
    return NBODY_OK;
}

int nbody_elapsed_f64(const NbodyHandle* h, double* out) {
    if (!h || !out) return NBODY_ERR_INVALID;
    *out = with_bodies(h, [](const auto& b) { return double(b.elapsed); });
    return NBODY_OK;
}

int nbody_sync(NbodyHandle* h) {
    if (!h) return NBODY_ERR_INVALID;
    int rc = use_device(h);
    if (rc) return rc;
    rc = nbody32::resolve_async(h);
    if (rc) return rc;
    HIP_TRY(h, hipStreamSynchronize(h->stream));
    return comm_check(h);
}

int nbody_set_profiling(NbodyHandle* h, int on) {
    if (!h) return NBODY_ERR_INVALID;
    h->profiling = on != 0;
    h->profile_every = on > 1 ? on : 1;
    h->profile_tick = 0;
    return NBODY_OK;
}

int nbody_stats(NbodyHandle* h, NbodyStats* out) {
    if (!h || !out) return NBODY_ERR_INVALID;
    int rc = use_device(h);
    if (rc) return rc;
    rc = nbody32::resolve_async(h);
    if (rc) return rc;
    rc = drain_events(h);
    if (rc) return rc;
    if (h->f64) return nbody64::stats(h, out);
    return nbody32::stats(h, out);
}

int nbody_reset_stats(NbodyHandle* h) {
    if (!h) return NBODY_ERR_INVALID;
    int rc = use_device(h);
    if (rc) return rc;
    rc = nbody32::resolve_async(h);
    if (rc) return rc;
    rc = drain_events(h);
    if (rc) return rc;
    uint64_t nodes = h->stats.tree_nodes;
    h->stats = NbodyStats{};
    h->stats.tree_nodes = nodes;
    if (h->let) { rc = nbody::let::reset_stats(h); if (rc) return rc; }
    rc = h->f64 ? nbody64::reset_stats(h) : nbody32::reset_stats(h);
    if (rc) return rc;
    rc = nbody::tracer::reset_stats(h);
    if (rc) return rc;
    if (h->d_counters) {
        HIP_TRY(h, hipMemsetAsync(h->d_counters, 0, 2 * NBODY_WALK_COUNTER_SLOTS * sizeof(unsigned long long), h->stream));
        HIP_TRY(h, hipStreamSynchronize(h->stream));
    }
    return NBODY_OK;
}

int nbody_energy(NbodyHandle* h, double* kinetic, double* potential) {
    if (!h) return NBODY_ERR_INVALID;
    int rc = use_device(h);
    if (rc) return rc;
    if (h->f64) return nbody64::energy(h, kinetic, potential);
    if (h->let && h->cfg.world_size > 1)
        return fail(h, NBODY_ERR_INVALID, "nbody_energy is not supported on NBODY_SHARD_SPATIAL handles of a world of more than one rank");
    return nbody32::energy(h, kinetic, potential);
}

int nbody_potentials(NbodyHandle* h, int mode, double* phi, size_t cap, size_t* n_out, uint64_t counts[2]) {
    if (!h) return NBODY_ERR_INVALID;
    int rc = use_device(h);
    if (rc) return rc;
    size_t n = 0;
    nbody::PotBodies bodies;
    double g = 0.0;
    rc = potentials_device(h, mode, &n, &bodies, &g);
    if (rc) return rc;
    return nbody::pot::download(h, n, g, phi, cap, n_out, counts);
}

namespace {
int probes_begin(NbodyHandle* h, const char* who, int mode, const double* xyz, size_t n_points, nbody::PotBodies* bodies, double* g) {
    if (n_points > (size_t(1) << 30)) return fail(h, NBODY_ERR_INVALID, std::string(who) + ": n_points must not exceed 2^30");
    if (!xyz && n_points > 0) return fail(h, NBODY_ERR_INVALID, std::string(who) + ": xyz is NULL");
    h->field.n_points = n_points;
    h->field.nodes = nullptr; h->field.n_nodes = 0; h->field.K = 1; h->field.quad = nullptr;
    size_t n = 0;
    return potentials_device(h, mode, &n, bodies, g, true);
}
}

int nbody_field_at(NbodyHandle* h, int mode, const double* xyz, size_t n_points, double* acc, double* phi, uint64_t counts[2]) {
    if (!h) return NBODY_ERR_INVALID;
    int rc = use_device(h);
    if (rc) return rc;
    nbody::PotBodies bodies;
    double g = 0.0;
    rc = probes_begin(h, "nbody_field_at", mode, xyz, n_points, &bodies, &g);
    if (rc) return rc;
    nbody::field::Out out;
    out.acc = acc; out.phi = phi;
    return nbody::field::run(h, mode, bodies, g, xyz, n_points, out, counts);
}

int nbody_tidal_at(NbodyHandle* h, int mode, const double* xyz, size_t n_points, double* tidal6, uint64_t counts[2]) {
    if (!h) return NBODY_ERR_INVALID;
    int rc = use_device(h);
    if (rc) return rc;
    if (mode == NBODY_POTENTIAL_TREE_QUADRUPOLE)
        return fail(h, NBODY_ERR_INVALID, "nbody_tidal_at: NBODY_POTENTIAL_TREE_QUADRUPOLE is not supported (the quadrupole term's share of the tensor is out of scope): NBODY_POTENTIAL_TREE is the tree mode");
    if (h->let)
        return fail(h, NBODY_ERR_INVALID, "nbody_tidal_at is not possible on NBODY_SHARD_SPATIAL handles: a rank holds neither the world's bodies nor the tree around a foreign point");
    nbody::PotBodies bodies;
    double g = 0.0;
    rc = probes_begin(h, "nbody_tidal_at", mode, xyz, n_points, &bodies, &g);
    if (rc) {
        const std::string why = h->err;
        return why.find("nbody_tidal_at") == std::string::npos ? fail(h, rc, "nbody_tidal_at: " + why) : rc;
    }
    nbody::field::Out out;
    out.tidal6 = tidal6; out.tidal = true;
    return nbody::field::run(h, mode, bodies, g, xyz, n_points, out, counts);
}

int nbody_energy_world(NbodyHandle* h, int mode, double* kinetic, double* potential) {
    if (!h) return NBODY_ERR_INVALID;
    int rc = use_device(h);
    if (rc) return rc;
    size_t n = 0;
    nbody::PotBodies bodies;
    double g = 0.0;
    rc = potentials_device(h, mode, &n, &bodies, &g);
    if (rc) return rc;
    return nbody::pot::energy(h, bodies, n, g, kinetic, potential);
}

int nbody_tree_export(NbodyHandle* h, float* com_mass, float* width, int32_t* skip, size_t cap, size_t* n_nodes) {
    if (!h) return NBODY_ERR_INVALID;
    if (h->cfg.method != NBODY_BARNES_HUT) return fail(h, NBODY_ERR_INVALID, "not a Barnes-Hut handle");
    if (h->f64) {
        if (com_mass || width) return fail(h, NBODY_ERR_INVALID, "f64 handle: use nbody_tree_export_f64");
        return nbody_tree_export_f64(h, nullptr, nullptr, skip, cap, n_nodes);
    }
    if (h->let)
        return fail(h, NBODY_ERR_INVALID, "nbody_tree_export is not supported on NBODY_SHARD_SPATIAL handles");
    {
        int rc = use_device(h);
        if (rc) return rc;
        rc = nbody32::resolve_async(h);
        if (rc) return rc;
    }
    return nbody32::bodies(h).tree.export_nodes(h, com_mass, width, skip, cap, n_nodes);
}

namespace {
const char* quadrupole_refusal(const NbodyHandle* h) {
    if (h->cfg.method != NBODY_BARNES_HUT) return "brute-force handles sum every pair exactly: there is no expansion to raise";
    if (h->f64 || h->cfg.dtype != NBODY_F32) return "NBODY_F64 handles walk monopoles only (quadrupoles exist for NBODY_F32)";
    if (h->cfg.math_mode != NBODY_MATH_FAST) return "NBODY_MATH_STRICT reproduces the reference's monopole sums: quadrupoles need NBODY_MATH_FAST";
    if (h->let || h->cfg.shard_mode != NBODY_SHARD_INDEX) return "NBODY_SHARD_SPATIAL handles walk monopoles only";
    if (h->cfg.world_size != 1) return "sharded worlds (world_size > 1) walk monopoles only";
    return nullptr;
}
}

int nbody_set_multipole(NbodyHandle* h, int order) {
    if (!h) return NBODY_ERR_INVALID;
    if (order != NBODY_MULTIPOLE_MONOPOLE && order != NBODY_MULTIPOLE_QUADRUPOLE)
        return fail(h, NBODY_ERR_INVALID, "nbody_set_multipole: order must be NBODY_MULTIPOLE_MONOPOLE (1) or NBODY_MULTIPOLE_QUADRUPOLE (2)");
    if (order == NBODY_MULTIPOLE_QUADRUPOLE)
        if (const char* why = quadrupole_refusal(h)) return fail(h, NBODY_ERR_INVALID, std::string("nbody_set_multipole: ") + why);
    if (order != h->multipole) {
        int rc = use_device(h);
        if (!rc) rc = nbody32::resolve_async(h);
        if (rc) return rc;
    }
    h->multipole = order;
    return NBODY_OK;
}

int nbody_get_multipole(const NbodyHandle* h, int* order) {
    if (!h || !order) return NBODY_ERR_INVALID;
    *order = h->multipole;
    return NBODY_OK;
}

int nbody_set_integrator(NbodyHandle* h, int integrator) {
    if (!h) return NBODY_ERR_INVALID;
    if (integrator != NBODY_INTEGRATOR_LEAPFROG && integrator != NBODY_INTEGRATOR_HERMITE4)
        return fail(h, NBODY_ERR_INVALID, "nbody_set_integrator: integrator must be NBODY_INTEGRATOR_LEAPFROG (0) or NBODY_INTEGRATOR_HERMITE4 (1)");
    if (integrator == NBODY_INTEGRATOR_HERMITE4) {
        const char* why = h->cfg.method != NBODY_BRUTE_FORCE ? "Barnes-Hut handles step with the leapfrog only"
                        : !h->f64                           ? "NBODY_F32 handles step with the leapfrog only"
                        : h->cfg.world_size != 1            ? "handles of a multi-rank world step with the leapfrog only"
                                                            : nullptr;
        if (why) return fail(h, NBODY_ERR_INVALID, std::string("nbody_set_integrator(NBODY_INTEGRATOR_HERMITE4): ") + why + " (brute-force NBODY_F64 handles with world_size == 1 take it)");
        if (nbody::ext::on(h))
            return fail(h, NBODY_ERR_INVALID, "nbody_set_integrator(NBODY_INTEGRATOR_HERMITE4): an external field is set, and the Hermite step would need its jerk (nbody_set_external_field with n == 0 removes it)");
    }
    if (!h->f64) return NBODY_OK;
    int rc = use_device(h);
    if (rc) return rc;
    return nbody64::set_integrator(h, integrator);
}

int nbody_get_integrator(const NbodyHandle* h, int* integrator) {
    if (!h || !integrator) return NBODY_ERR_INVALID;
    *integrator = h->f64 ? nbody64::get_integrator(h) : NBODY_INTEGRATOR_LEAPFROG;
    return NBODY_OK;
}

int nbody_download_jerk(NbodyHandle* h, double* jerk3, size_t cap, size_t* n_out) {
    if (!h) return NBODY_ERR_INVALID;
    if (!h->f64) return fail(h, NBODY_ERR_INVALID, "nbody_download_jerk: the handle runs the leapfrog integrator (nbody_set_integrator)");
    int rc = use_device(h);
    if (rc) return rc;
    return nbody64::download_jerk(h, jerk3, cap, n_out);
}

int nbody_suggest_dt(NbodyHandle* h, double eta, double* dt_out) {
    if (!h || !dt_out) return h ? fail(h, NBODY_ERR_INVALID, "null argument") : NBODY_ERR_INVALID;
    if (!h->f64) return fail(h, NBODY_ERR_INVALID, "nbody_suggest_dt: the handle runs the leapfrog integrator (nbody_set_integrator)");
    int rc = use_device(h);
    if (rc) return rc;
    return nbody64::suggest_dt(h, eta, dt_out);
}

int nbody_set_block_steps(NbodyHandle* h, double eta, int max_level) {
    if (!h) return NBODY_ERR_INVALID;
    if (!h->f64) return fail(h, NBODY_ERR_INVALID, "nbody_set_block_steps: the handle runs the leapfrog integrator (nbody_set_integrator)");
    int rc = use_device(h);
    if (rc) return rc;
    return nbody64::set_block_steps(h, eta, max_level);
}

int nbody_get_block_steps(const NbodyHandle* h, double* eta, int* max_level) {
    if (!h || !h->f64) return NBODY_ERR_INVALID;
    return nbody64::get_block_steps(h, eta, max_level);
}

int nbody_download_levels(NbodyHandle* h, int32_t* level, size_t cap, size_t* n_out) {
    if (!h) return NBODY_ERR_INVALID;
    if (!h->f64) return fail(h, NBODY_ERR_INVALID, "nbody_download_levels: the handle runs the leapfrog integrator (nbody_set_integrator)");
    int rc = use_device(h);
    if (rc) return rc;
    return nbody64::download_levels(h, level, cap, n_out);
}

int nbody_block_step_counts(NbodyHandle* h, uint64_t out[2]) {
    if (!h || !out) return h ? fail(h, NBODY_ERR_INVALID, "null argument") : NBODY_ERR_INVALID;
    if (!h->f64) return fail(h, NBODY_ERR_INVALID, "nbody_block_step_counts: the handle runs the leapfrog integrator (nbody_set_integrator)");
    return nbody64::block_step_counts(h, out);
}

int nbody_debug_hermite_forces_of(NbodyHandle* h, const int32_t* ids, size_t n_ids, double* acc3, double* jerk3) {
    if (!h) return NBODY_ERR_INVALID;
    if (!h->f64) return fail(h, NBODY_ERR_INVALID, "nbody_debug_hermite_forces_of: the handle runs the leapfrog integrator (nbody_set_integrator)");
    int rc = use_device(h);
    if (rc) return rc;
    return nbody64::debug_hermite_forces_of(h, ids, n_ids, acc3, jerk3);
}

int nbody_tree_export_quadrupoles(NbodyHandle* h, float* q6, size_t cap, size_t* n_nodes) {
    if (!h) return NBODY_ERR_INVALID;
    if (h->cfg.method != NBODY_BARNES_HUT) return fail(h, NBODY_ERR_INVALID, "not a Barnes-Hut handle");
    if (!h->quad_pass && !h->quad_call)
        return fail(h, NBODY_ERR_INVALID, "nbody_tree_export_quadrupoles: neither did the last force pass walk with quadrupoles (nbody_set_multipole) nor was the last tree built by a call in NBODY_POTENTIAL_TREE_QUADRUPOLE");
    int rc = use_device(h);
    return rc ? rc : nbody32::tree_export_quadrupoles(h, q6, cap, n_nodes);
}

int nbody_tree_export_f64(NbodyHandle* h, double* com_mass, double* width, int32_t* skip, size_t cap, size_t* n_nodes) {
    if (!h) return NBODY_ERR_INVALID;
    if (h->cfg.method != NBODY_BARNES_HUT) return fail(h, NBODY_ERR_INVALID, "not a Barnes-Hut handle");
    if (!h->f64) return fail(h, NBODY_ERR_INVALID, "f32 handle: use nbody_tree_export");
    int rc = use_device(h);
    return rc ? rc : nbody64::bodies(h).tree.export_nodes(h, com_mass, width, skip, cap, n_nodes);
}

extern "C++" {
namespace {
template <class F>
void cells_from_preorder(const F* com_mass, const int32_t* skip, size_t n, const F root_center[3], F root_width, float* min_max6, int32_t* depth) {
    struct Open { size_t end; F c[3]; F half; int depth; };
    std::vector<Open> stack;
    for (size_t i = 0; i < n; ++i) {
        while (!stack.empty() && stack.back().end <= i) stack.pop_back();
        Open me;
        me.end = size_t(skip[i]);
        if (stack.empty()) {
            for (int k = 0; k < 3; ++k) me.c[k] = root_center[k];
            me.half = root_width * F(0.5);
            me.depth = 0;
        } else {
            const Open& p = stack.back();
            me.half = p.half * F(0.5);
            for (int k = 0; k < 3; ++k) me.c[k] = com_mass[4 * i + k] > p.c[k] ? p.c[k] + me.half : p.c[k] - me.half;
            me.depth = p.depth + 1;
        }
        if (min_max6)
            for (int k = 0; k < 3; ++k) {
                min_max6[6 * i + k] = float(me.c[k] + (-me.half));
                min_max6[6 * i + 3 + k] = float(me.c[k] + me.half);
            }
        if (depth) depth[i] = me.depth;
        if (me.end > i + 1) stack.push_back(me);
    }
}
}
}

int nbody_tree_export_cells(NbodyHandle* h, float* min_max6, int32_t* depth, size_t cap, size_t* n_nodes) {
    if (!h) return NBODY_ERR_INVALID;
    size_t n = 0;
    int rc = h->f64 ? nbody_tree_export_f64(h, nullptr, nullptr, nullptr, 0, &n) : nbody_tree_export(h, nullptr, nullptr, nullptr, 0, &n);
    if (rc) return rc;
    if (n_nodes) *n_nodes = n;
    if (!min_max6 && !depth) return NBODY_OK;
    if (n > cap) return fail(h, NBODY_ERR_CAPACITY, "tree export buffer too small");
    return with_bodies(h, [&](auto& b) {
        using F = std::remove_reference_t<decltype(b.width)>;
        std::vector<F> cm(4 * n);
        std::vector<int32_t> sk(n);
        const int rc2 = b.tree.export_nodes(h, cm.data(), nullptr, sk.data(), n, &n);
        if (!rc2) cells_from_preorder<F>(cm.data(), sk.data(), n, b.center, b.width, min_max6, depth);
        return rc2;
    });
}

int nbody_comm_unique_id(void* id_bytes) {
    if (!id_bytes) return NBODY_ERR_INVALID;
    const char* v = std::getenv("NBODY_TRANSPORT");
    std::string err;
    int rc = nbody::transport_make_id((v && std::strcmp(v, "ipc") == 0) ? nbody::kTransportIpc : nbody::kTransportRccl, id_bytes, &err);
    return rc ? fail(nullptr, rc, err) : NBODY_OK;
}

int nbody_comm_local_id(void* id_bytes) {
    if (!id_bytes) return NBODY_ERR_INVALID;
    std::string err;
    int rc = nbody::transport_make_id(nbody::kTransportIpc, id_bytes, &err);
    return rc ? fail(nullptr, rc, err) : NBODY_OK;
}

struct Agreement {
    int32_t abi, method, math_mode, leaf_mode, tree_build, dtype, shard_mode, world, seg_cap;
    int32_t cross_sym, sym_packed, bf_variant, walk_variant, walk_split;
    uint64_t capacity;
};
static const char* const kAgreementFields[] = {"ABI version", "method", "math_mode", "leaf_mode", "tree_build", "dtype", "shard_mode", "world_size",
                                               "shard capacity", "NBODY_CROSS_SYM", "NBODY_SYM_PACKED", "NBODY_BF_VARIANT", "NBODY_BH_VARIANT",
                                               "NBODY_BH_SPLIT"};

int nbody_comm_init(NbodyHandle* h, const void* id_bytes) {
    if (!h || !id_bytes) return NBODY_ERR_INVALID;
    int rc = use_device(h);
    if (rc) return rc;
    h->comm_ready = false;
    h->tp.reset();
    {
        std::string err;
        int code = NBODY_ERR_COMM;
        h->tp.reset(nbody::transport_create(id_bytes, h->cfg.rank, h->cfg.world_size, h->device, &err, &code));
        if (!h->tp) return fail(h, code, err);
    }
    if (!h->comm_stream) {
        HIP_TRY(h, hipStreamCreateWithFlags(&h->comm_stream, hipStreamNonBlocking));
        HIP_TRY(h, hipEventCreateWithFlags(&h->ev_drifted, hipEventDisableTiming));
        HIP_TRY(h, hipEventCreateWithFlags(&h->ev_gathered, hipEventDisableTiming));
    }
    Agreement mine{NBODY_ABI_VERSION, h->cfg.method, h->cfg.math_mode, h->cfg.leaf_mode, h->cfg.tree_build, h->cfg.dtype, h->cfg.shard_mode,
                   h->cfg.world_size, h->shape.seg_cap, nbody::tuning().cross_sym, nbody::tuning().sym_packed, nbody::tuning().bf_fast_variant, nbody::tuning().bh_walk_variant,
                   nbody::tuning().bh_walk_split, h->cfg.capacity};
    std::vector<Agreement> all(size_t(h->cfg.world_size));
    TP_TRY(h, h->tp->host_all_gather(&mine, all.data(), sizeof(Agreement)));
    for (int r = 0; r < h->cfg.world_size; ++r) {
        const int32_t* a = reinterpret_cast<const int32_t*>(&all[size_t(r)]);
        const int32_t* m = reinterpret_cast<const int32_t*>(&mine);
        for (size_t f = 0; f < sizeof(kAgreementFields) / sizeof(kAgreementFields[0]); ++f)
            if (a[f] != m[f]) {
                h->tp.reset();
                return fail(h, NBODY_ERR_COMM, std::string("nbody_comm_init: rank ") + std::to_string(r) + " and rank " + std::to_string(h->cfg.rank) + " disagree on " +
                                                   kAgreementFields[f] + " (" + std::to_string(a[f]) + " vs " + std::to_string(m[f]) + "): every rank of a world must be created alike");
            }
        if (all[size_t(r)].capacity != mine.capacity) {
            h->tp.reset();
            return fail(h, NBODY_ERR_COMM, "nbody_comm_init: ranks disagree on NbodyConfig.capacity");
        }
    }
    h->comm_ready = true;
    return NBODY_OK;
}

namespace {
struct Knob { const char* name; int nbody::Tuning::*field; bool tuning_build_only; };
const Knob kKnobs[] = {
    {"cross_sym", &nbody::Tuning::cross_sym, false}, {"sym_packed", &nbody::Tuning::sym_packed, false},
    {"bf_fast_variant", &nbody::Tuning::bf_fast_variant, false}, {"sym_wpb", &nbody::Tuning::sym_wpb, false}, {"sym_ipt", &nbody::Tuning::sym_ipt, false}, {"let_list_div", &nbody::Tuning::let_list_div, false}, {"bh_walk_duo", &nbody::Tuning::bh_walk_duo, false}, {"bh_walk_xcd", &nbody::Tuning::bh_walk_xcd, false},
    {"sym_rounds", &nbody::Tuning::sym_rounds, false}, {"sym_k", &nbody::Tuning::sym_k, false},
    {"sym_min_bodies", &nbody::Tuning::sym_min_bodies, false}, {"sym_reduce_split", &nbody::Tuning::sym_reduce_split, false},
    {"sym_opp_rot", &nbody::Tuning::sym_opp_rot, false},
    {"cross_slots", &nbody::Tuning::cross_slots, false}, {"cross_ipt", &nbody::Tuning::cross_ipt, false},
    {"cross_wpb", &nbody::Tuning::cross_wpb, false}, {"bh_walk_split", &nbody::Tuning::bh_walk_split, false},
    {"bh_walk_order", &nbody::Tuning::bh_walk_order, false}, {"bh_reduce_split", &nbody::Tuning::bh_reduce_split, false},
    {"tree_max_tie", &nbody::Tuning::tree_max_tie, false},
    {"bf64_min_bodies", &nbody::Tuning::bf64_min_bodies, false}, {"bf64_ipt", &nbody::Tuning::bf64_ipt, false},
    {"bf64_rot", &nbody::Tuning::bf64_rot, false}, {"bf64_waves", &nbody::Tuning::bf64_waves, false},
    {"bh_walk_variant", &nbody::Tuning::bh_walk_variant, true}, {"bh_walk_lds_block", &nbody::Tuning::bh_walk_lds_block, true},
    {"bh_hot_cap", &nbody::Tuning::bh_hot_cap, true}, {"bh_walk_debug", &nbody::Tuning::bh_walk_debug, true},
    {"sym_debug", &nbody::Tuning::sym_debug, true},
};
}

int nbody_set_tuning(NbodyHandle* h, const char* name, int value) {
    if (!h || !name) return NBODY_ERR_INVALID;
    for (const Knob& k : kKnobs)
        if (std::strcmp(k.name, name) == 0) {
#ifndef NBODY_TUNING
            if (k.tuning_build_only && value != nbody::Tuning{}.*(k.field))
                return fail(h, NBODY_ERR_INVALID, std::string("nbody_set_tuning: '") + name + "' selects code only the tuning build carries (make -C nbody-llm_amd/csrc tuning)");
#endif
            if (h->comm_ready && (std::strcmp(name, "cross_sym") == 0 || std::strcmp(name, "sym_packed") == 0 || std::strcmp(name, "bf_fast_variant") == 0))
                return fail(h, NBODY_ERR_INVALID, std::string("nbody_set_tuning: '") + name + "' is part of what the ranks agreed on at nbody_comm_init: set it before");
            h->tune.*(k.field) = value;
            return NBODY_OK;
        }
    return fail(h, NBODY_ERR_INVALID, std::string("nbody_set_tuning: unknown knob '") + name + "'");
}

int nbody_get_tuning(const NbodyHandle* h, const char* name, int* value) {
    if (!h || !name || !value) return NBODY_ERR_INVALID;
    for (const Knob& k : kKnobs)
        if (std::strcmp(k.name, name) == 0) { *value = h->tune.*(k.field); return NBODY_OK; }
    return NBODY_ERR_INVALID;
}

int nbody_get_config(const NbodyHandle* h, NbodyConfig* out) {
    if (!h || !out) return NBODY_ERR_INVALID;
    *out = h->cfg;
    return NBODY_OK;
}

int nbody_is_tuning_build(void) {
#ifdef NBODY_TUNING
    return 1;
#else
    return 0;
#endif
}

int nbody_comm_transport(const NbodyHandle* h, char* out, size_t cap) {
    if (!h || !out || cap == 0) return NBODY_ERR_INVALID;
    std::snprintf(out, cap, "%s", h->tp ? h->tp->name() : "none");
    return NBODY_OK;
}

int nbody_download_ids(NbodyHandle* h, int32_t* ids, size_t cap, size_t* n_out) {
    if (!h) return NBODY_ERR_INVALID;
    int rc = use_device(h);
    if (rc) return rc;
    if (!h->let) return fail(h, NBODY_ERR_INVALID, "nbody_download_ids is for NBODY_SHARD_SPATIAL handles (index-block shards: nbody_local_range)");
    return nbody::let::download_ids(h, ids, cap, n_out);
}

int nbody_let_stats(NbodyHandle* h, NbodyLetStats* out) {
    if (!h || !out) return NBODY_ERR_INVALID;
    if (!h->let) return fail(h, NBODY_ERR_INVALID, "not an NBODY_SHARD_SPATIAL handle");
    return nbody::let::stats(h, out);
}

int nbody_debug_let_phase(NbodyHandle* h, int phase, float dt) {
    if (!h) return NBODY_ERR_INVALID;
    int rc = use_device(h);
    if (rc) return rc;
    if (!h->let) return fail(h, NBODY_ERR_INVALID, "not an NBODY_SHARD_SPATIAL handle");
    return nbody::let::debug_phase(h, phase, dt);
}

int nbody_debug_let_exchange(NbodyHandle* h, NbodyHandle* peer, int which) {
    if (!h || !peer) return NBODY_ERR_INVALID;
    int rc = use_device(h);
    if (rc) return rc;
    if (!h->let || !peer->let) return fail(h, NBODY_ERR_INVALID, "not an NBODY_SHARD_SPATIAL handle");
    return nbody::let::debug_exchange(h, peer, which);
}

int nbody_debug_let_set_prune(NbodyHandle* h, int prune);

int nbody_local_range(const NbodyHandle* h, size_t* first, size_t* count) {
    if (!h) return NBODY_ERR_INVALID;
    if (first) *first = h->first_global;
    if (count) *count = h->n_at_upload;
    return NBODY_OK;
}

int nbody_debug_step_begin(NbodyHandle* h, float dt) {
    if (!h) return NBODY_ERR_INVALID;
    if (h->f64) return fail(h, NBODY_ERR_INVALID, "f64 handles are single-shard");
    int rc = use_device(h);
    return rc ? rc : nbody32::step_begin(h, dt);
}

int nbody_debug_import_segment(NbodyHandle* h, NbodyHandle* peer) {
    if (!h || !peer) return NBODY_ERR_INVALID;
    if (h->f64 || peer->f64) return fail(h, NBODY_ERR_INVALID, "f64 handles are single-shard");
    auto& b = nbody32::bodies(h);
    const Shard& from = nbody32::bodies(peer).sh;
    if (b.sh.n_seg != from.n_seg || b.sh.seg_cap != from.seg_cap) return fail(h, NBODY_ERR_INVALID, "peer has a different sharding");
    int rc = use_device(h);
    if (rc) return rc;
    const int s = from.my_seg;
    HIP_TRY(h, hipStreamSynchronize(peer->stream));
    HIP_TRY(h, hipMemcpyAsync(b.sh.pos_all + size_t(s) * b.sh.seg_cap, from.own_pos(), size_t(b.sh.seg_cap) * sizeof(float4), hipMemcpyDeviceToDevice, h->stream));
    HIP_TRY(h, hipMemcpyAsync(b.sh.seg_count + s, from.own_count(), sizeof(int), hipMemcpyDeviceToDevice, h->stream));
    HIP_TRY(h, hipStreamSynchronize(h->stream));
    b.count_dirty = true;
    return NBODY_OK;
}

int nbody_debug_step_forces(NbodyHandle* h, float dt) {
    if (!h) return NBODY_ERR_INVALID;
    if (h->f64) return fail(h, NBODY_ERR_INVALID, "f64 handles are single-shard");
    int rc = use_device(h);
    return rc ? rc : nbody32::step_forces(h, dt);
}

int nbody_debug_import_partials(NbodyHandle* h, NbodyHandle* peer) {
    if (!h || !peer) return NBODY_ERR_INVALID;
    if (h->f64 || peer->f64) return fail(h, NBODY_ERR_INVALID, "f64 handles are single-shard");
    int rc = use_device(h);
    return rc ? rc : nbody32::debug_import_partials(h, peer);
}

int nbody_debug_step_end(NbodyHandle* h, float dt) {
    if (!h) return NBODY_ERR_INVALID;
    if (h->f64) return fail(h, NBODY_ERR_INVALID, "f64 handles are single-shard");
    int rc = use_device(h);
    return rc ? rc : nbody32::step_finish(h, dt);
}

int nbody_host_cross_plan(int rank, int world, int seg_cap, int n_own, int* ipt, int* n_sets, int* n_parts, int* parts,
                          int* n_recv, int* recv_from) {
    if (world < 2 || rank < 0 || rank >= world || seg_cap <= 0 || n_own < 0 || n_own > seg_cap) return NBODY_ERR_INVALID;
    if (world > 2 * (nbody::CrossPartners::kMax - 1)) return NBODY_ERR_INVALID;
    const nbody::CrossPlan p = nbody::make_cross_plan(rank, world, seg_cap, n_own);
    if (ipt) *ipt = p.ipt;
    if (n_sets) *n_sets = p.A;
    if (n_parts) *n_parts = p.parts.n;
    if (parts)
        for (int i = 0; i < p.parts.n; ++i) {
            parts[5 * i + 0] = p.parts.seg[i]; parts[5 * i + 1] = p.parts.c0[i]; parts[5 * i + 2] = p.parts.c1[i];
            parts[5 * i + 3] = p.parts.a0[i]; parts[5 * i + 4] = p.parts.a1[i];
        }
    if (n_recv) *n_recv = p.n_recv;
    if (recv_from) for (int i = 0; i < p.n_recv; ++i) recv_from[i] = p.recv_from[i];
    return NBODY_OK;
}

int nbody_host_launch_plan(size_t n_bodies, float theta2, int fast_math, int out[3]) {
    if (!out) return NBODY_ERR_INVALID;
    nbody::bind_tuning(nullptr);
    const nbody::WalkPlan p = nbody::walk_plan(n_bodies, fast_math != 0, nbody::kMaxSplit, theta2);
    out[0] = p.bodies_per_lane; out[1] = p.segments; out[2] = nbody::sym_bodies_per_lane(n_bodies);
    return NBODY_OK;
}

int nbody_host_exchange_layout(const int* matrix, int world, int rank, long long clamp, int packed_send, size_t send_stride,
                               size_t* out_at, size_t* n_out, size_t* in_at, size_t* n_in, size_t* total_in) {
    if (!matrix || world < 1 || world > 16 || rank < 0 || rank >= world || !out_at || !n_out || !in_at || !n_in) return NBODY_ERR_INVALID;
    const size_t t = nbody::let::exchange_layout(matrix, world, rank, clamp, packed_send != 0, send_stride, out_at, n_out, in_at, n_in);
    if (total_in) *total_in = t;
    return NBODY_OK;
}

int nbody_host_build_tree(const float* pos4, size_t n, const float center[3], float width, int threads,
                          float* com_mass, float* node_width, int32_t* skip, int32_t* leaf_body, int32_t* order,
                          size_t cap, size_t* n_nodes) {
    if ((!pos4 && n) || !center || !n_nodes) return NBODY_ERR_INVALID;
    if (n > (1ull << 30)) return NBODY_ERR_INVALID;
    static thread_local std::unique_ptr<nbody::WorkerPool> tl_pool;
    static thread_local int tl_threads = 0;
    static thread_local nbody::BuildScratch scratch;
    static thread_local nbody::HostTree tree;
    const int want = threads > 0 ? threads : 1;
    if (!tl_pool || tl_threads != want) { tl_pool.reset(new nbody::WorkerPool(want)); tl_threads = want; }
    nbody::WorkerPool& pool = *tl_pool;
    int cnt = int(n);
    nbody::build_octree(pos4, 1, int(n), &cnt, center, width, pool, scratch, tree);
    if (tree.too_deep) return NBODY_ERR_TREE_DEPTH;
    *n_nodes = tree.n_nodes;
    if (!com_mass) return NBODY_OK;
    if (tree.n_nodes > cap) return NBODY_ERR_CAPACITY;
    for (size_t i = 0; i < tree.n_nodes; ++i) {
        const nbody::NodeRec& r = tree.nodes[i];
        com_mass[4 * i] = r.a.x; com_mass[4 * i + 1] = r.a.y; com_mass[4 * i + 2] = r.a.z; com_mass[4 * i + 3] = r.a.m;
        if (node_width) node_width[i] = std::sqrt(r.b.w2);
        if (skip) skip[i] = r.b.skip;
        if (leaf_body) leaf_body[i] = r.b.body;
    }
    if (order) std::memcpy(order, tree.order, tree.n_order * sizeof(int32_t));
    return NBODY_OK;
}

}
```

nbody-llm_amd/csrc/nbody_f32.cpp:

```cpp
#include "nbody_engine.h"
#include "nbody_let.h"
#include "nbody_pot.h"
#include "nbody_tracer.h"
#include "nbody_external.h"
#include "nbody_pairs.h"

#include <algorithm>
#include <cmath>
#include <cstdlib>
#include <string>
#include <vector>

namespace nbody32 {

struct State : EngineBodies<float> {
    nbody::SymPlan sym_plan;
    int* d_sym_bounds = nullptr;
    float4* d_planes = nullptr;
    size_t planes_cap = 0;
    int sym_waves = 0;
    uint64_t sym_pairs = 0;
    size_t sym_pairs_n = 0;
    nbody::CrossPlan cross;
    bool cross_on = false;
    int4* d_cross_slices = nullptr;
    size_t cross_slices_cap = 0;
    float4* d_xplanes = nullptr;
    float4* d_send = nullptr;
    size_t xplanes_cap = 0, send_cap = 0;
    int recv_plane0 = 0;
    bool tail_pending = false;
    bool partials_in_flight = false;
    hipEvent_t ev_partials_ready = nullptr, ev_partials_done = nullptr;
    bool kick_pending = false;
    float kick_dt = 0.f;
    bool tracer_kick = false;

    bool async_bh = false;
    struct PendingStep { float dt; float elapsed_before; };
    std::vector<PendingStep> pending;
    bool last_step_async = false;
    bool host_tree_once = false;

    float4* d_walk = nullptr;
    int* d_unified = nullptr;
    size_t walk_cap = 0;
    float4* d_bfs = nullptr;
    void* d_bfs_ws = nullptr;
    size_t bfs_cap = 0;
    float4* d_hot = nullptr;
    int hot_cap = 0;
    int* d_hot_info = nullptr;
    int* h_hot_info = nullptr;
    int hot_threshold = 0;
    size_t hot_threshold_n = 0;
};

namespace {

using engine::total_upper;

int exchange_begin(NbodyHandle* h) {
    State& s = *h->f32;
    if (s.sh.n_seg == 1 && !h->comm_ready) return NBODY_OK;
    if (!h->comm_ready) return fail(h, NBODY_ERR_COMM, "world_size > 1 but nbody_comm_init has not been called");
    HIP_TRY(h, hipEventRecord(h->ev_drifted, h->stream));
    HIP_TRY(h, hipStreamWaitEvent(h->comm_stream, h->ev_drifted, 0));
    TP_TRY(h, h->tp->group_begin());
    TP_TRY(h, h->tp->all_gather(s.sh.pos_all, size_t(s.sh.seg_cap) * sizeof(float4), h->comm_stream));
    TP_TRY(h, h->tp->all_gather(s.sh.seg_count, sizeof(int), h->comm_stream));
    TP_TRY(h, h->tp->group_end());
    HIP_TRY(h, hipEventRecord(h->ev_gathered, h->comm_stream));
    h->exchange_in_flight = true;
    return NBODY_OK;
}

int exchange_wait(NbodyHandle* h) {
    if (!h->exchange_in_flight) return NBODY_OK;
    HIP_TRY(h, hipStreamWaitEvent(h->stream, h->ev_gathered, 0));
    h->exchange_in_flight = false;
    return NBODY_OK;
}

int fail_if_hip(NbodyHandle* h, hipError_t e) { return e == hipSuccess ? NBODY_OK : fail(h, NBODY_ERR_HIP, hipGetErrorString(e)); }

int sharded_counts_exact(NbodyHandle* h) {
    State& s = *h->f32;
    if (!h->comm_ready) return fail(h, NBODY_ERR_COMM, "world_size > 1 but nbody_comm_init has not been called");
    int rc = exchange_wait(h);
    if (rc) return rc;
    HIP_TRY(h, hipStreamSynchronize(h->stream));
    TP_TRY(h, h->tp->all_gather(s.sh.seg_count, sizeof(int), h->stream));
    s.count_dirty = true;
    return s.sync_count(h, h->stream);
}

int sharded_add_point(NbodyHandle* h, const void* particle) {
    State& s = *h->f32;
    int rc = sharded_counts_exact(h);
    if (rc) return rc;
    const int G = s.sh.n_seg, last = G - 1;
    if (total_upper(s) >= h->cfg.capacity || s.seg_count_host[last] >= s.sh.seg_cap)
        return fail(h, NBODY_ERR_CAPACITY, "capacity exhausted (a push goes to the end of the vector: the last rank's block is full)");
    if (s.sh.my_seg == last) return s.push_one(h, h->stream, particle);
    s.seg_count_host[last] += 1;
    return NBODY_OK;
}

int sharded_remove_point(NbodyHandle* h, size_t index) {
    State& s = *h->f32;
    int rc = sharded_counts_exact(h);
    if (rc) return rc;
    const int G = s.sh.n_seg, me = s.sh.my_seg;
    if (index >= total_upper(s)) return fail(h, NBODY_ERR_INVALID, "swap_remove index out of range");
    int r = 0, last = G - 1;
    size_t j = index;
    while (j >= size_t(s.seg_count_host[r])) { j -= size_t(s.seg_count_host[r]); ++r; }
    while (s.seg_count_host[last] == 0) --last;
    const size_t tail = size_t(s.seg_count_host[last]) - 1;
    if (r == last) {
        if (me == r && j != tail) {
            HIP_TRY(h, hipMemcpyAsync(s.sh.own_pos() + j, s.sh.own_pos() + tail, sizeof(float4), hipMemcpyDeviceToDevice, h->stream));
            HIP_TRY(h, hipMemcpyAsync(s.sh.vel + j, s.sh.vel + tail, sizeof(float4), hipMemcpyDeviceToDevice, h->stream));
            HIP_TRY(h, hipMemcpyAsync(s.sh.acc + j, s.sh.acc + tail, sizeof(float4), hipMemcpyDeviceToDevice, h->stream));
        }
    } else if (me == last || me == r) {
        rc = s.ensure_aos(h, 2);
        if (rc) return rc;
        if (me == last) {
            nbody::launch_soa_to_aos(h->stream, s.d_aos, 10, 1, s.sh.own_pos() + tail, s.sh.vel + tail, s.sh.acc + tail);
            TP_TRY(h, h->tp->send(s.d_aos, 40, r, h->stream));
        } else {
            TP_TRY(h, h->tp->recv(s.d_aos, 40, last, h->stream));
            nbody::launch_aos_to_soa(h->stream, s.d_aos, 10, 1, s.sh.own_pos() + j, s.sh.vel + j, s.sh.acc + j);
        }
        HIP_TRY(h, hipGetLastError());
    }
    if (me == last) {
        s.n_local = tail;
        rc = s.push_own_count(h, h->stream);
        if (rc) return rc;
    } else {
        HIP_TRY(h, hipStreamSynchronize(h->stream));
    }
    s.seg_count_host[last] -= 1;
    return comm_check(h);
}

constexpr size_t kShardedSymMinBodies = 2048;

int ensure_sym_plan(NbodyHandle* h) {
    State& s = *h->f32;
    const size_t set = size_t(64) * size_t(nbody::sym_bodies_per_lane(std::max<size_t>(1, s.n_local)));
    const int A = int((std::max<size_t>(1, s.n_local) + set - 1) / set);
    const int knobs = nbody::tuning().sym_wpb * 100 + nbody::tuning().sym_rounds + nbody::tuning().sym_k * 10000 + nbody::tuning().sym_ipt * 1000000 + (nbody::tuning().sym_opp_rot ? 500000000 : 0);
    if (s.sym_plan.A == A && s.sym_plan.ipt * 64 == int(set) && s.d_sym_bounds && s.sym_waves == knobs) return NBODY_OK;
    s.sym_waves = knobs;
    s.sym_plan = nbody::make_sym_plan(int(std::max<size_t>(1, s.n_local)));
    nbody::SymPlan& p = s.sym_plan;
    s.cross_on = false;
    if (s.sh.n_seg > 1) {
        const size_t cap_pad = (size_t(s.sh.seg_cap) + 63) / 64 * 64;
        p.plane_stride = std::max(p.n_pad, cap_pad);
        if (nbody::tuning().cross_sym && s.sh.n_seg <= 2 * (nbody::CrossPartners::kMax - 1)) {
            s.cross = nbody::make_cross_plan(s.sh.my_seg, s.sh.n_seg, s.sh.seg_cap, int(std::max<size_t>(1, s.n_local)));
            s.cross_on = true;
            s.recv_plane0 = p.n_planes + s.cross.k_res;
            p.n_planes += s.cross.k_res + s.cross.n_recv;
        } else {
            const int a_os = int((p.n_pad + 511) / 512);
            p.k_os = std::max(1, std::min(256, 3072 / std::max(1, a_os)));
            p.plane_stride = std::max(p.plane_stride, size_t(a_os) * 512);
            p.n_planes += p.k_os;
        }
    }
    if (!s.d_sym_bounds) HIP_TRY(h, h->mem.dev(s.d_sym_bounds, 2 * 128 * sizeof(int)));
    HIP_TRY(h, hipMemcpyAsync(s.d_sym_bounds, p.bounds.data(), p.bounds.size() * sizeof(int), hipMemcpyHostToDevice, h->stream));
    HIP_TRY(h, hipMemcpyAsync(s.d_sym_bounds + 128, p.bounds_long.data(), p.bounds_long.size() * sizeof(int), hipMemcpyHostToDevice, h->stream));
    HIP_TRY(h, hipStreamSynchronize(h->stream));
    HIP_TRY(h, grow_dev(h, s.d_planes, s.planes_cap, size_t(p.n_planes) * p.plane_stride, sizeof(float4), Grow::exact));
    if (s.cross_on) {
        const nbody::CrossPlan& c = s.cross;
        if (c.slices.size() > s.cross_slices_cap)
            HIP_TRY(h, grow_dev(h, s.d_cross_slices, s.cross_slices_cap, c.slices.size() + 64, sizeof(int4), Grow::exact));
        if (!c.slices.empty()) {
            HIP_TRY(h, hipMemcpyAsync(s.d_cross_slices, c.slices.data(), c.slices.size() * sizeof(int4), hipMemcpyHostToDevice, h->stream));
            HIP_TRY(h, hipStreamSynchronize(h->stream));
        }
        const size_t xneed = size_t(std::max(1, c.parts.n)) * size_t(c.A) * p.plane_stride;
        HIP_TRY(h, grow_dev(h, s.d_xplanes, s.xplanes_cap, xneed, sizeof(float4), Grow::exact));
        const size_t sneed = size_t(std::max(1, c.parts.n)) * p.plane_stride;
        HIP_TRY(h, grow_dev(h, s.d_send, s.send_cap, sneed, sizeof(float4), Grow::exact));
    }
    return NBODY_OK;
}

int bf_forces(NbodyHandle* h) {
    State& s = *h->f32;
    const float eps2 = s.g_soft * s.g_soft;
    const bool fast = h->cfg.math_mode == NBODY_MATH_FAST && nbody::tuning().bf_fast_variant == 0;
    const bool sharded = s.sh.n_seg > 1;
    const bool sym = fast && (sharded ? size_t(s.sh.seg_cap) >= kShardedSymMinBodies : s.n_local >= size_t(std::max(1024, nbody::tuning().sym_min_bodies)));
    const size_t tot = total_upper(s);
    if (sym) {
        int rc = ensure_sym_plan(h);
        if (rc) return rc;
        if (s.sym_pairs_n != s.n_local) {
            s.sym_pairs = nbody::sym_main_pairs(s.sym_plan, s.n_local);
            s.sym_pairs_n = s.n_local;
        }
    }
    const nbody::SymPlan& p = s.sym_plan;
    uint64_t timed = 0;
    if (!(sym && sharded)) {
        int rc = exchange_wait(h);
        if (rc) return rc;
    }
    if (!sym) {
        ForceTimer t(h);
        if (h->cfg.math_mode == NBODY_MATH_STRICT) nbody::launch_bf_forces_strict(h->stream, s.sh, int(s.n_local), s.g, eps2);
        else nbody::launch_bf_forces_fast(h->stream, s.sh, int(s.n_local), s.g, eps2);
        timed = tot > 0 ? uint64_t(s.n_local) * uint64_t(tot - 1) : 0;
    } else if (!sharded) {
        {
            ForceTimer t(h);
            nbody::launch_bf_sym_main(h->stream, s.sh, p, s.d_sym_bounds, s.d_planes, int(s.n_local), eps2);
        }
        timed = 2 * s.sym_pairs;
        s.tail_pending = true;
    } else {
        nbody::launch_bf_sym_main(h->stream, s.sh, p, s.d_sym_bounds, s.d_planes, int(s.n_local), eps2);
        {
            int rc = exchange_wait(h);
            if (rc) return rc;
        }
        if (s.cross_on) {
            const nbody::CrossPlan& c = s.cross;
            {
                ForceTimer t(h);
                nbody::launch_bf_cross(h->stream, s.sh, c, s.d_cross_slices,
                                       s.d_planes + size_t(s.recv_plane0 - c.k_res) * p.plane_stride, s.d_xplanes,
                                       s.d_send, p.plane_stride, eps2);
            }
            for (int i = 0; i < c.parts.n; ++i) {
                const long long set = 64LL * c.ipt;
                const long long own = std::max(0LL, std::min<long long>(s.n_local, set * c.parts.a1[i]) - set * c.parts.a0[i]);
                const long long theirs = std::max(0LL, std::min<long long>(s.seg_count_host[c.parts.seg[i]], 64LL * c.parts.c1[i]) - 64LL * c.parts.c0[i]);
                timed += 2ull * uint64_t(own) * uint64_t(theirs);
            }
        } else {
            ForceTimer t(h);
            nbody::launch_bf_os(h->stream, s.sh, int((p.n_pad + 511) / 512), p.k_os, s.d_planes + size_t(p.n_planes - p.k_os) * p.plane_stride, p.plane_stride, eps2);
            timed = uint64_t(s.n_local) * uint64_t(tot - s.n_local);
        }
        s.tail_pending = true;
    }
    HIP_TRY(h, hipGetLastError());
    if (tot > 0 && h->timed_this) h->stats.force_kernel_interactions += timed;
    return NBODY_OK;
}

int bh_walk_device_tree(NbodyHandle* h, bool* fell_back);
int bh_walk_device_tree_async(NbodyHandle* h);
int bh_walk_host_tree(NbodyHandle* h);
int step_end(NbodyHandle* h, float dt);
int step_impl(NbodyHandle* h, float dt);

int setup_nested_walk(NbodyHandle* h, nbody::TreeDev* td) {
    State& s = *h->f32;
    if (h->cfg.math_mode != NBODY_MATH_STRICT || h->cfg.leaf_mode != NBODY_LEAF_REFERENCE) return NBODY_OK;
    int rc = s.tree.ensure_stack(h, s.sh.seg_cap, (s.tree.on_device ? 43 : s.tree.host.max_depth) + 2);
    if (rc) return rc;
    td->nested_stack = s.tree.d_stack;
    td->nested_stride = s.tree.stack_lanes;
    return NBODY_OK;
}

int setup_lds_walk(NbodyHandle* h, nbody::TreeDev* td, size_t n_tree) {
#ifndef NBODY_TUNING
    (void)h; (void)td; (void)n_tree;
    return NBODY_OK;
#else
    State& s = *h->f32;
    if (h->cfg.math_mode == NBODY_MATH_FAST && nbody::tuning().bh_walk_variant == 5 && (s.tree.on_device || s.tree.host.max_depth <= 42)) {
        if (s.bfs_cap < s.tree.node_cap) {
            s.bfs_cap = 0;
            HIP_TRY(h, h->mem.dev(s.d_bfs, s.tree.node_cap * 2 * sizeof(float4)));
            HIP_TRY(h, h->mem.dev(s.d_bfs_ws, nbody::bfs_workspace_bytes(s.tree.node_cap)));
            s.bfs_cap = s.tree.node_cap;
        }
        td->bfs = s.d_bfs; td->bfs_ws = s.d_bfs_ws; td->bfs_cap = s.bfs_cap;
        return NBODY_OK;
    }
    if (h->cfg.math_mode != NBODY_MATH_FAST || nbody::tuning().bh_walk_variant != 3 || nbody::tuning().bh_hot_cap <= 0) return NBODY_OK;
    const int M = std::min(nbody::tuning().bh_hot_cap, 5000);
    if (s.walk_cap < s.tree.node_cap) {
        s.walk_cap = 0;
        HIP_TRY(h, h->mem.dev(s.d_walk, (s.tree.node_cap + 1) * 2 * sizeof(float4)));
        HIP_TRY(h, h->mem.dev(s.d_unified, (s.tree.node_cap + 1) * sizeof(int)));
        s.walk_cap = s.tree.node_cap;
    }
    if (s.hot_cap != M) {
        s.hot_cap = 0;
        HIP_TRY(h, h->mem.dev(s.d_hot, size_t(M) * 2 * sizeof(float4)));
        HIP_TRY(h, hipMemsetAsync(s.d_hot, 0, size_t(M) * 2 * sizeof(float4), h->stream));
        s.hot_cap = M;
        s.hot_threshold_n = 0;
    }
    if (!s.d_hot_info) {
        HIP_TRY(h, h->mem.dev(s.d_hot_info, 2 * sizeof(int)));
        HIP_TRY(h, hipMemsetAsync(s.d_hot_info, 0, 2 * sizeof(int), h->stream));
        HIP_TRY(h, h->mem.pin(s.h_hot_info, 2 * sizeof(int)));
        s.h_hot_info[0] = s.h_hot_info[1] = 0;
    }
    if (s.hot_threshold_n == 0 || n_tree > 2 * s.hot_threshold_n || 2 * n_tree < s.hot_threshold_n) {
        s.hot_threshold = int(std::max<size_t>(8, n_tree / 64));
        s.hot_threshold_n = std::max<size_t>(1, n_tree);
    } else {
        const int flagged = s.h_hot_info[1];
        if (flagged > M) s.hot_threshold = s.hot_threshold + s.hot_threshold / 8 + 1;
        else if (flagged < M - M / 3 && s.hot_threshold > 2) s.hot_threshold = s.hot_threshold - s.hot_threshold / 8 - 1;
    }
    td->walk = s.d_walk; td->unified = s.d_unified; td->hot = s.d_hot; td->hot_info = s.d_hot_info;
    td->hot_cap = M; td->hot_threshold = s.hot_threshold;
    return NBODY_OK;
#endif
}

int fill_quadrupoles(NbodyHandle* h, const nbody::TreeDev& td, bool any_nodes) {
    State& s = *h->f32;
    HIP_TRY(h, grow_dev(h, h->d_quad, h->quad_cap, s.tree.node_cap, nbody::kQuadRecBytes, Grow::quarter));
    const bool counted_on_device = td.n_order_dev != nullptr;
    if (any_nodes) nbody::launch_tree_quad(h->stream, td.nodes, td.n_nodes, h->d_quad, counted_on_device ? s.tree.bufs.d_info : nullptr, td.poison);
    return NBODY_OK;
}

int tracer_tree_forces(NbodyHandle* h, const nbody::TreeDev& td) {
    State& s = *h->f32;
    const bool kick = s.tracer_kick;
    s.tracer_kick = false;
    return nbody::tracer::tree_forces(h, td, kick ? &s.kick_dt : nullptr);
}

int walk_tree(NbodyHandle* h, nbody::TreeDev& td, size_t n_tree) {
    State& s = *h->f32;
    if (h->pot.walking) {
        h->quad_call = h->pot.quad;
        if (h->pot.quad) {
            int rc = fill_quadrupoles(h, td, td.n_nodes > 0);
            if (rc) return rc;
        }
    }
    if (h->pot.walking == kWalkField) {
        FieldBufs& f = h->field;
        f.nodes = td.nodes; f.n_nodes = td.n_nodes; f.K = td.n_split;
        f.first = td.split_first; f.anc = td.split_anc; f.n_anc = td.split_n_anc;
        f.quad = h->pot.quad ? h->d_quad : nullptr;
        HIP_TRY(h, hipGetLastError());
        return NBODY_OK;
    }
    if (h->pot.walking) {
        const size_t stride = (size_t(std::max(td.n_order, 1)) + 63) / 64 * 64;
        int rc = nbody::pot::ensure_planes(h, size_t(td.n_split) * stride);
        if (rc) return rc;
        if (h->pot.quad)
            nbody::launch_bh_pot_walk_quad(h->stream, s.sh.own_pos(), td, h->d_quad, s.g_soft * s.g_soft, s.theta2, h->pot.d_planes, stride,
                                           h->pot.d_sum, h->pot.d_counts);
        else
            nbody::launch_bh_pot_walk(h->stream, s.sh.own_pos(), td, s.g_soft * s.g_soft, s.theta2, h->pot.d_planes, stride, h->pot.d_sum,
                                      h->pot.d_counts);
        HIP_TRY(h, hipGetLastError());
        return NBODY_OK;
    }
    h->quad_pass = h->multipole == NBODY_MULTIPOLE_QUADRUPOLE;
    h->quad_call = false;
    if (h->quad_pass) {
        int rc = fill_quadrupoles(h, td, td.n_order > 0);
        if (rc) return rc;
        ForceTimer t(h);
        int kicked = 0;
        nbody::launch_bh_walk_quad(h->stream, s.sh, td, h->d_quad, s.g, s.g_soft * s.g_soft, s.theta2, h->d_counters,
                                   h->cfg.leaf_mode == NBODY_LEAF_DIRECT, s.kick_pending ? &s.kick_dt : nullptr, &kicked);
        if (kicked) s.kick_pending = false;
        HIP_TRY(h, hipGetLastError());
        return tracer_tree_forces(h, td);
    }
    int rc = setup_nested_walk(h, &td);
    if (!rc) rc = setup_lds_walk(h, &td, n_tree);
    if (rc) return rc;
    {
        ForceTimer t(h);
        int kicked = 0;
        nbody::launch_bh_walk(h->stream, s.sh, td, s.g, s.g_soft * s.g_soft, s.theta2,
                              h->cfg.math_mode == NBODY_MATH_FAST, h->d_counters, h->cfg.leaf_mode == NBODY_LEAF_DIRECT,
                              s.kick_pending ? &s.kick_dt : nullptr, &kicked);
        if (kicked) s.kick_pending = false;
    }
    if (td.hot_cap > 0) HIP_TRY(h, hipMemcpyAsync(s.h_hot_info, s.d_hot_info, 2 * sizeof(int), hipMemcpyDeviceToHost, h->stream));
    HIP_TRY(h, hipGetLastError());
    return tracer_tree_forces(h, td);
}

int split_segments(const NbodyHandle* h, const TreeBuilt& t) {
    State& s = *h->f32;
    if (h->pot.walking == kWalkField) return field_split_plan(h->field.n_points, size_t(t.n_nodes));
    return walk_split_plan(t.n_order, h->cfg.math_mode != NBODY_MATH_STRICT || h->pot.walking, s.theta2, size_t(t.n_nodes)).segments;
}
int walk_built(NbodyHandle* h, const TreeBuilt& t, int K) {
    State& s = *h->f32;
    nbody::TreeDev td;
    td.nodes = s.tree.d_nodes; td.n_nodes = t.n_nodes;
    td.order = t.order; td.n_order = int(t.n_order);
    walk_split_view(s.tree.split, K, size_t(s.sh.seg_cap), &td);
    return walk_tree(h, td, t.n_tree);
}

int bh_forces(NbodyHandle* h) {
    State& s = *h->f32;
    {
        int rc = exchange_wait(h);
        if (rc) return rc;
    }
    s.last_step_async = false;
    if (h->cfg.tree_build == NBODY_TREE_DEVICE && !s.host_tree_once) {
        const bool plain_walk = h->cfg.math_mode == NBODY_MATH_STRICT || nbody::tuning().bh_walk_variant == 0;
        if (s.async_bh && (plain_walk || h->multipole == NBODY_MULTIPOLE_QUADRUPOLE) && !nbody::tuning().bh_walk_debug) return bh_walk_device_tree_async(h);
        int rc = resolve_async(h);
        if (rc) return rc;
        bool fell_back = false;
        rc = bh_walk_device_tree(h, &fell_back);
        if (rc || !fell_back) return rc;
    }
    s.host_tree_once = false;
    return bh_walk_host_tree(h);
}

int bh_walk_host_tree(NbodyHandle* h) {
    State& s = *h->f32;
    Shard& sh = s.sh;
    TreeBuilt t;
    int rc = s.tree.build_on_host(h, s, &t);
    if (rc) return rc;
    const int K = split_segments(h, t);
    rc = s.tree.split.ensure(h, K, size_t(sh.seg_cap));
    if (!rc) rc = s.tree.split.list_on_host(h, h->stream, s.tree.host.nodes, t.n_nodes, K);
    if (rc) return rc;
    return walk_built(h, t, K);
}

int bh_walk_device_tree(NbodyHandle* h, bool* fell_back) {
    State& s = *h->f32;
    TreeBuilt t;
    int rc = s.tree.build_on_device(h, s, nbody::tuning().bh_walk_variant == 3, nullptr, &t);
    *fell_back = t.fell_back;
    if (rc || t.fell_back) return rc;
    const int K = split_segments(h, t);
    rc = s.tree.split.ensure(h, K, size_t(s.sh.seg_cap));
    if (rc) return rc;
    if (t.n_tree > 0) s.tree.split.list_on_device(h->stream, s.tree.work, int(t.n_tree), t.n_nodes, K);
    return walk_built(h, t, K);
}

int bh_walk_device_tree_async(NbodyHandle* h) {
    State& s = *h->f32;
    Shard& sh = s.sh;
    auto t1 = clk::now();
    TreeBuildBufs& tb = s.tree.bufs;
    int rc = tb.ensure(h, size_t(sh.seg_cap), 0);
    if (rc) return rc;
    const size_t n_upper = s.n_local;
    rc = s.tree.ensure_dev(h, TreeTypes<float>::kNodesPerBody * n_upper + 64, n_upper);
    if (rc) return rc;
    if (s.pending.empty()) HIP_TRY(h, hipMemsetAsync(h->d_poison + 1, 0, sizeof(int), h->stream));
    const int K = walk_split_plan(n_upper, h->cfg.math_mode != NBODY_MATH_STRICT, s.theta2, n_upper).segments;
    rc = s.tree.split.ensure(h, K, size_t(sh.seg_cap));
    if (rc) return rc;
    const nbody::TreeSplitReq req = s.tree.split.request(K, tb.d_info, h->d_poison);
    nbody::TreeDevWork& work = s.tree.work;
    if (nbody::build_octree_device(h->stream, sh.own_pos(), sh.own_count(), int(n_upper), s.center, s.width, tb.ws, size_t(sh.seg_cap),
                                   s.tree.d_nodes, int(s.tree.node_cap), s.tree.d_order, tb.d_info, &work, 0, n_upper > 0 ? &req : nullptr) != 0)
        return fail(h, NBODY_ERR_HIP, "device octree build: rocPRIM call failed");
    HIP_TRY(h, hipGetLastError());
    h->stats.tree_build_ms += ms_since(t1);
    s.tree.on_device = true;
    if (n_upper == 0)
        s.tree.split.list_on_device(h->stream, work, 0, int(s.tree.node_cap), K, tb.d_info, h->d_poison);
    nbody::TreeDev td;
    td.nodes = s.tree.d_nodes; td.n_nodes = int(s.tree.node_cap);
    td.order = s.tree.d_order; td.n_order = int(n_upper);
    td.n_order_dev = tb.d_info + 2;
    td.poison = h->d_poison;
    walk_split_view(s.tree.split, K, size_t(sh.seg_cap), &td);
    rc = walk_tree(h, td, n_upper);
    if (rc) return rc;
    s.last_step_async = true;
    s.count_dirty = true;
    return NBODY_OK;
}

int partials_begin(NbodyHandle* h) {
    State& s = *h->f32;
    if (!(s.cross_on && s.tail_pending) || s.cross.parts.n + s.cross.n_recv == 0) return NBODY_OK;
    if (!h->comm_ready) return fail(h, NBODY_ERR_COMM, "world_size > 1 but nbody_comm_init has not been called");
    const nbody::CrossPlan& c = s.cross;
    const size_t S = s.sym_plan.plane_stride;
    const size_t bytes = size_t(s.sh.seg_cap) * sizeof(float4);
    if (!s.ev_partials_ready) {
        HIP_TRY(h, hipEventCreateWithFlags(&s.ev_partials_ready, hipEventDisableTiming));
        HIP_TRY(h, hipEventCreateWithFlags(&s.ev_partials_done, hipEventDisableTiming));
    }
    HIP_TRY(h, hipEventRecord(s.ev_partials_ready, h->stream));
    HIP_TRY(h, hipStreamWaitEvent(h->comm_stream, s.ev_partials_ready, 0));
    TP_TRY(h, h->tp->group_begin());
    for (int i = 0; i < c.parts.n; ++i)
        TP_TRY(h, h->tp->send(s.d_send + size_t(i) * S, bytes, c.parts.seg[i], h->comm_stream));
    for (int i = 0; i < c.n_recv; ++i)
        TP_TRY(h, h->tp->recv(s.d_planes + size_t(s.recv_plane0 + i) * S, bytes, c.recv_from[i], h->comm_stream));
    TP_TRY(h, h->tp->group_end());
    HIP_TRY(h, hipEventRecord(s.ev_partials_done, h->comm_stream));
    s.partials_in_flight = true;
    return NBODY_OK;
}

int partials_wait(NbodyHandle* h) {
    State& s = *h->f32;
    if (!s.partials_in_flight) return NBODY_OK;
    HIP_TRY(h, hipStreamWaitEvent(h->stream, s.ev_partials_done, 0));
    s.partials_in_flight = false;
    return NBODY_OK;
}

int forces_begin(NbodyHandle* h) {
    return h->cfg.method == NBODY_BARNES_HUT ? bh_forces(h) : bf_forces(h);
}

int forces_finish(NbodyHandle* h) {
    State& s = *h->f32;
    if (!s.tail_pending) return NBODY_OK;
    s.tail_pending = false;
    const float eps2 = s.g_soft * s.g_soft;
    nbody::launch_bf_sym_tail(h->stream, s.sh, s.sym_plan, s.d_planes, int(s.n_local), s.g, eps2,
                              s.kick_pending ? &s.kick_dt : nullptr);
    s.kick_pending = false;
    HIP_TRY(h, hipGetLastError());
    return NBODY_OK;
}

int forces(NbodyHandle* h) {
    int rc = forces_begin(h);
    if (rc) return rc;
    rc = partials_begin(h);
    if (rc) return rc;
    rc = partials_wait(h);
    if (rc) return rc;
    return forces_finish(h);
}

int step_end(NbodyHandle* h, float dt) {
    int rc = step_forces(h, dt);
    if (rc) return rc;
    rc = partials_begin(h);
    if (rc) return rc;
    rc = partials_wait(h);
    if (rc) return rc;
    return step_finish(h, dt);
}

int step_impl(NbodyHandle* h, float dt) {
    State& s = *h->f32;
    const float elapsed_before = s.elapsed;
    int rc = step_begin(h, dt);
    if (rc) return rc;
    rc = exchange_begin(h);
    if (rc) return rc;
    rc = step_end(h, dt);
    if (rc) return rc;
    if (s.last_step_async) {
        s.pending.push_back(State::PendingStep{dt, elapsed_before});
        if (s.pending.size() >= 4096) rc = resolve_async(h);
    }
    return rc;
}

int spatial_walk(NbodyHandle* h, NbodyHandle* twin, int n_orig) {
    State& s = *h->f32;
    const int G = h->cfg.world_size, cap = s.sh.seg_cap;
    PotBufs& p = h->pot;
    int rc = nbody::let::potential_pass(twin);
    if (rc) return fail(h, rc, twin->err);
    rc = nbody::pot::begin(h, size_t(cap));
    if (rc) return rc;
    HIP_TRY(h, grow_dev(h, p.d_rec, p.rec_cap, size_t(G) * size_t(cap), sizeof(nbody::PotRec), Grow::quarter));
    const size_t n_ids = size_t(h->cfg.capacity) + 1;
    HIP_TRY(h, grow_dev(h, p.d_slot_of, p.slot_cap, n_ids, sizeof(int), Grow::quarter));
    if (!p.d_rec_count) HIP_TRY(h, h->mem.dev(p.d_rec_count, sizeof(int) * size_t(G)));
    HIP_TRY(h, hipStreamSynchronize(h->stream));
    hipStream_t ts = twin->stream;
    nbody::PotRec* rec = static_cast<nbody::PotRec*>(p.d_rec);
    const Shard& tsh = twin->f32->sh;
    nbody::launch_pot_pack(ts, tsh.ids, twin->pot.d_sum, tsh.own_count(), cap, rec + size_t(h->cfg.rank) * size_t(cap));
    HIP_TRY(h, hipMemcpyAsync(p.d_rec_count + h->cfg.rank, tsh.own_count(), sizeof(int), hipMemcpyDeviceToDevice, ts));
    if (twin->comm_ready) {
        TP_TRY(twin, twin->tp->group_begin());
        TP_TRY(twin, twin->tp->all_gather(rec, size_t(cap) * sizeof(nbody::PotRec), ts));
        TP_TRY(twin, twin->tp->all_gather(p.d_rec_count, sizeof(int), ts));
        TP_TRY(twin, twin->tp->group_end());
    }
    HIP_TRY(h, hipMemsetAsync(p.d_slot_of, 0xFF, n_ids * sizeof(int), ts));
    nbody::launch_pot_scatter(ts, s.sh.ids, s.sh.own_count(), n_orig, p.d_slot_of, int(std::min<size_t>(n_ids, 0x7fffffff)), rec, p.d_rec_count, G, cap, p.d_sum);
    HIP_TRY(h, hipMemcpyAsync(p.d_counts, twin->pot.d_counts, 2 * NBODY_WALK_COUNTER_SLOTS * sizeof(unsigned long long), hipMemcpyDeviceToDevice, ts));
    HIP_TRY(h, hipGetLastError());
    HIP_TRY(h, hipStreamSynchronize(ts));
    if (twin->tp) { rc = twin->tp->check(); if (rc) return fail(h, rc, twin->tp->error()); }
    return NBODY_OK;
}

int spatial_potentials(NbodyHandle* h, size_t* n_own, nbody::PotBodies* bodies, double* g) {
    State& s = *h->f32;
    if (!s.bounds_set) return fail(h, NBODY_ERR_INVALID, "nbody_set_bounds has not been called");
    if (h->cfg.world_size > 1 && !h->comm_ready) return fail(h, NBODY_ERR_COMM, "world_size > 1 but nbody_comm_init has not been called");
    NbodyHandle* twin = nullptr;
    int rc = NBODY_OK, n_orig = 0;
    {
        engine::PotView<float> view(s);
        rc = nbody_clone(h, &twin);
        n_orig = int(s.n_local);
    }
    if (rc) return fail(h, rc, std::string("nbody_potentials: scratch clone: ") + nbody_last_error(nullptr));
    twin->tp = std::move(h->tp);
    twin->comm_ready = h->comm_ready;
    nbody::bind_tuning(&twin->tune);
    rc = spatial_walk(h, twin, n_orig);
    if (rc && !twin->err.empty()) h->err = twin->err;
    h->tp = std::move(twin->tp);
    twin->comm_ready = false;
    nbody::bind_tuning(&h->tune);
    nbody_destroy(twin);
    (void)hipSetDevice(h->device);
    if (rc) return rc;
    bodies->pos_all = s.sh.pos_all; bodies->vel = s.sh.vel; bodies->seg_count = s.sh.seg_count;
    bodies->f64 = 0; bodies->n_seg = 1; bodies->seg_cap = s.sh.seg_cap; bodies->my_seg = 0;
    bodies->world = h->comm_ready ? h->cfg.world_size : 1;
    *g = double(s.g);
    *n_own = size_t(n_orig);
    return NBODY_OK;
}

}

EngineBodies<float>& bodies(NbodyHandle* h) { return *h->f32; }
const EngineBodies<float>& bodies(const NbodyHandle* h) { return *h->f32; }

int create(NbodyHandle* h) {
    State* sp = new State();
    h->f32 = sp;
    State& s = *sp;
    Shard& sh = s.sh;
    int rc = s.alloc(h, h->stream, h->shape);
    if (rc) return rc;
    HIP_TRY(h, h->mem.dev(h->d_poison, 2 * sizeof(int)));
    HIP_TRY(h, hipMemsetAsync(h->d_poison, 0, 2 * sizeof(int), h->stream));
    if (h->cfg.method == NBODY_BARNES_HUT) {
        rc = s.tree.alloc_host(h, sh);
        if (rc) return rc;
    }
    HIP_TRY(h, hipStreamSynchronize(h->stream));
    const char* v = std::getenv("NBODY_BH_ASYNC");
    sp->async_bh = h->cfg.method == NBODY_BARNES_HUT && h->cfg.tree_build == NBODY_TREE_DEVICE && h->cfg.world_size == 1 &&
                   h->cfg.shard_mode != NBODY_SHARD_SPATIAL && !(v && v[0] == '0');
    if (sp->async_bh) sh.poison = h->d_poison;
    return NBODY_OK;
}

void destroy(NbodyHandle* h) {
    State* s = h->f32;
    if (!s) return;
    if (s->ev_partials_ready) (void)hipEventDestroy(s->ev_partials_ready);
    if (s->ev_partials_done) (void)hipEventDestroy(s->ev_partials_done);
    delete s;
    h->f32 = nullptr;
}

int clone_state(NbodyHandle* src, NbodyHandle* dst) {
    int rc = src->f32->sync_count(src, src->stream);
    if (rc) return fail(dst, rc, src->err);
    rc = fail_if_hip(dst, hipStreamSynchronize(src->stream));
    if (!rc) rc = dst->f32->copy_from(dst, dst->stream, *src->f32);
    if (!rc) rc = fail_if_hip(dst, hipStreamSynchronize(dst->stream));
    if (rc) return fail(dst, rc, "clone copy: " + dst->err);
    dst->multipole = src->multipole;
    dst->search.mode = src->search.mode;
    dst->first_global = src->first_global; dst->n_at_upload = src->n_at_upload;
    return NBODY_OK;
}

int upload(NbodyHandle* h, const void* aos, size_t n, size_t stride) {
    const int rc = resolve_async(h);
    return rc ? rc : engine::upload(h, *h->f32, aos, n, stride);
}

int download(NbodyHandle* h, void* aos, size_t cap, size_t stride, size_t* n_out) {
    State& s = *h->f32;
    int rc = resolve_async(h);
    if (rc) return rc;
    return s.download_own(h, h->stream, aos, cap, stride, n_out, comm_check);
}

int count(NbodyHandle* h, size_t* n_out) {
    const int rc = resolve_async(h);
    return rc ? rc : engine::count(h, *h->f32, n_out);
}

int count_global(NbodyHandle* h, size_t* n_out) {
    const int rc = resolve_async(h);
    return rc ? rc : engine::count_global(h, *h->f32, n_out);
}

int add_point(NbodyHandle* h, const void* particle) {
    State& s = *h->f32;
    if (s.sh.n_seg != 1) return sharded_add_point(h, particle);
    int rc = resolve_async(h);
    if (rc) return rc;
    return s.push_one(h, h->stream, particle);
}

int remove_point(NbodyHandle* h, size_t index) {
    State& s = *h->f32;
    if (s.sh.n_seg != 1) return sharded_remove_point(h, index);
    int rc = resolve_async(h);
    if (rc) return rc;
    return s.swap_remove_one(h, h->stream, index);
}

int merge_contacts(NbodyHandle* h, double radius, NbodyContact* list, size_t cap, size_t* n_contacts) {
    return nbody::pairs::merge_contacts<float>(h, *h->f32, radius, list, cap, n_contacts, nullptr,
                                               [](NbodyHandle* hh, int n_upper) { nbody::launch_compact(hh->stream, hh->f32->sh, n_upper); });
}

int init(NbodyHandle* h) {
    h->f32->elapsed = 0.f;
    return NBODY_OK;
}

int resolve_async(NbodyHandle* h) {
    if (!h->f32 || !h->f32->async_bh) return NBODY_OK;
    State& s = *h->f32;
    for (int round = 0; round < 1000000; ++round) {
        HIP_TRY(h, hipMemcpyAsync(h->h_poison, h->d_poison, 2 * sizeof(int), hipMemcpyDeviceToHost, h->stream));
        if (s.tree.bufs.d_info) HIP_TRY(h, hipMemcpyAsync(h->h_poison + 2, s.tree.bufs.d_info, 3 * sizeof(int), hipMemcpyDeviceToHost, h->stream));
        HIP_TRY(h, hipStreamSynchronize(h->stream));
        const int flags = h->h_poison[0], done = h->h_poison[1];
        if (!flags) {
            if (s.tree.on_device && s.tree.bufs.d_info) {
                s.tree.n_nodes = size_t(h->h_poison[2]);
                h->stats.tree_nodes = uint64_t(h->h_poison[2]);
            }
            s.pending.clear();
            return NBODY_OK;
        }
        std::vector<State::PendingStep> rest;
        if (size_t(done) < s.pending.size()) rest.assign(s.pending.begin() + done, s.pending.end());
        s.pending.clear();
        HIP_TRY(h, hipMemsetAsync(h->d_poison, 0, 2 * sizeof(int), h->stream));
        if (flags & 2) {
            int rc = s.tree.ensure_dev(h, 2 * s.tree.node_cap + 64, s.n_local);
            if (rc) return rc;
        }
        if (rest.empty()) {
            s.host_tree_once = true;
            return NBODY_OK;
        }
        s.elapsed = rest[0].elapsed_before;
        h->stats.steps -= rest.size();
        s.host_tree_once = true;
        int rc = s.sync_count(h, h->stream);
        if (rc) return rc;
        rc = step_end(h, rest[0].dt);
        if (rc) return rc;
        for (size_t k = 1; k < rest.size(); ++k) {
            rc = step_impl(h, rest[k].dt);
            if (rc) return rc;
        }
    }
    return fail(h, NBODY_ERR_INVALID, "resolve_async did not converge");
}

int step_begin(NbodyHandle* h, float dt) {
    State& s = *h->f32;
    if (!s.bounds_set) return fail(h, NBODY_ERR_INVALID, "nbody_set_bounds has not been called");
    nbody::launch_drift_half(h->stream, s.sh, int(s.n_local), dt, s.bnd);
    nbody::launch_compact(h->stream, s.sh, int(s.n_local));
    s.count_dirty = true;
    HIP_TRY(h, hipGetLastError());
    if (nbody::tracer::on(h)) return nbody::tracer::drift_retain(h, dt);
    return NBODY_OK;
}

int step_forces(NbodyHandle* h, float dt) {
    State& s = *h->f32;
    const bool fuse = !nbody::ext::on(h);
    s.kick_pending = fuse;
    s.kick_dt = dt;
    if (nbody::tracer::on(h) && h->cfg.method == NBODY_BRUTE_FORCE) {
        int rc = nbody::tracer::forces(h, fuse ? &s.kick_dt : nullptr);
        if (rc) { s.kick_pending = false; return rc; }
    }
    s.tracer_kick = fuse && nbody::tracer::on(h);
    int rc = forces_begin(h);
    s.tracer_kick = false;
    if (rc) { s.kick_pending = false; s.tail_pending = false; }
    return rc;
}

int step_finish(NbodyHandle* h, float dt) {
    State& s = *h->f32;
    int rc = forces_finish(h);
    if (rc) { s.kick_pending = false; return rc; }
    if (nbody::ext::on(h)) {
        rc = nbody::ext::add(h, s.sh, s.n_local, s.g, &dt, true);
        if (!rc && nbody::tracer::on(h)) rc = nbody::ext::add(h, h->tr.sh, h->tr.n_host, s.g, &dt, false);
        if (rc) return rc;
    } else if (s.kick_pending) nbody::launch_kick_drift(h->stream, s.sh, int(s.n_local), dt);
    s.kick_pending = false;
    HIP_TRY(h, hipGetLastError());
    if (h->ev_pending.size() >= 4096) {
        rc = drain_events(h);
        if (rc) return rc;
    }
    s.elapsed += dt;
    h->stats.steps += 1;
    return NBODY_OK;
}

int debug_import_partials(NbodyHandle* h, NbodyHandle* peer) {
    State& s = *h->f32;
    const State& ps = *peer->f32;
    if (!(s.cross_on && s.tail_pending)) return NBODY_OK;
    if (!(ps.cross_on && ps.tail_pending)) return fail(h, NBODY_ERR_INVALID, "peer is not in the same phase");
    int src = -1, dst = -1;
    for (int i = 0; i < ps.cross.parts.n; ++i) if (ps.cross.parts.seg[i] == s.sh.my_seg) src = i;
    for (int i = 0; i < s.cross.n_recv; ++i) if (s.cross.recv_from[i] == ps.sh.my_seg) dst = i;
    if ((src < 0) != (dst < 0)) return fail(h, NBODY_ERR_INVALID, "send/receive plans of the two shards do not match");
    if (src < 0) return NBODY_OK;
    HIP_TRY(h, hipStreamSynchronize(peer->stream));
    HIP_TRY(h, hipMemcpyAsync(s.d_planes + size_t(s.recv_plane0 + dst) * s.sym_plan.plane_stride,
                              ps.d_send + size_t(src) * ps.sym_plan.plane_stride,
                              size_t(s.sh.seg_cap) * sizeof(float4), hipMemcpyDeviceToDevice, h->stream));
    HIP_TRY(h, hipStreamSynchronize(h->stream));
    return NBODY_OK;
}

int step_by(NbodyHandle* h, float dt) { return step_impl(h, dt); }

int steps(NbodyHandle* h, int k) {
    State& s = *h->f32;
    for (int i = 0; i < k; ++i) {
        int rc = step_impl(h, s.dt);
        if (rc) return rc;
    }
    return NBODY_OK;
}

int update_forces(NbodyHandle* h) {
    State& s = *h->f32;
    if (h->cfg.method == NBODY_BARNES_HUT && !s.bounds_set) return fail(h, NBODY_ERR_INVALID, "nbody_set_bounds has not been called");
    int rc = resolve_async(h);
    if (rc) return rc;
    rc = exchange_begin(h);
    if (rc) return rc;
    rc = forces(h);
    if (!rc && nbody::tracer::on(h) && h->cfg.method == NBODY_BRUTE_FORCE) rc = nbody::tracer::forces(h, nullptr);
    if (!rc && s.last_step_async) {
        s.last_step_async = false;
        rc = resolve_async(h);
        if (!rc && s.host_tree_once) rc = forces(h);
    }
    if (rc || !nbody::ext::on(h)) return rc;
    rc = nbody::ext::add<float>(h, s.sh, s.n_local, s.g, nullptr, false);
    if (!rc && nbody::tracer::on(h)) rc = nbody::ext::add<float>(h, h->tr.sh, h->tr.n_host, s.g, nullptr, false);
    return rc;
}

int stats(NbodyHandle* h, NbodyStats* out) { return engine::stats(h, *h->f32, out); }

int reset_stats(NbodyHandle* h) { return engine::reset_stats(h, *h->f32); }

int energy(NbodyHandle* h, double* kinetic, double* potential) {
    const int rc = resolve_async(h);
    return rc ? rc : engine::energy(h, *h->f32, kinetic, potential);
}

int potentials_device(NbodyHandle* h, int mode, size_t* n_own, nbody::PotBodies* bodies, double* g, bool field) {
    if (h->let) return spatial_potentials(h, n_own, bodies, g);
    State& s = *h->f32;
    const bool tree = mode != NBODY_POTENTIAL_PAIRS, quad = mode == NBODY_POTENTIAL_TREE_QUADRUPOLE;
    if (tree && !s.bounds_set) return fail(h, NBODY_ERR_INVALID, "nbody_set_bounds has not been called");
    int rc = resolve_async(h);
    if (!rc) rc = exchange_wait(h);
    if (rc) return rc;
    if (s.sh.n_seg > 1) rc = engine::gather_blocks(h, s, h->stream);
    if (rc) return rc;
    engine::PotView<float> view(s);
    const bool saved_once = s.host_tree_once;
    rc = view.begin(h, bodies, g);
    if (!rc && mode == NBODY_POTENTIAL_PAIRS) {
        const size_t n = s.n_local;
        if (!field) rc = nbody::pot::pairs(h, *bodies, n, total_upper(s) - n, double(s.g_soft) * double(s.g_soft));
    } else if (!rc) {
        PotWalkScope walking(h->pot, field ? kWalkField : kWalkPotentials, quad);
        const bool on_device = h->cfg.tree_build == NBODY_TREE_DEVICE;
        bool fell_back = false;
        if (on_device) rc = bh_walk_device_tree(h, &fell_back);
        if (!rc && (fell_back || !on_device)) rc = bh_walk_host_tree(h);
    }
    *n_own = s.n_local;
    s.host_tree_once = saved_once;
    return rc ? rc : comm_check(h);
}

int tree_export_quadrupoles(NbodyHandle* h, float* q6, size_t cap, size_t* n_nodes) {
    State& s = *h->f32;
    int rc = resolve_async(h);
    if (rc) return rc;
    const size_t n = s.tree.n_nodes;
    if (n_nodes) *n_nodes = n;
    if (!q6) return NBODY_OK;
    if (n > cap) return fail(h, NBODY_ERR_CAPACITY, "tree export buffer too small");
    if (n == 0) return NBODY_OK;
    HIP_TRY(h, grow_dev(h, h->d_quad, h->quad_cap, std::max(n, s.tree.node_cap), nbody::kQuadRecBytes, Grow::quarter));
    nbody::launch_tree_quad(h->stream, s.tree.d_nodes, int(n), h->d_quad, nullptr, nullptr);
    HIP_TRY(h, hipGetLastError());
    std::vector<float> rec(8 * n);
    HIP_TRY(h, hipMemcpyAsync(rec.data(), h->d_quad, n * nbody::kQuadRecBytes, hipMemcpyDeviceToHost, h->stream));
    HIP_TRY(h, hipStreamSynchronize(h->stream));
    for (size_t i = 0; i < n; ++i)
        for (int k = 0; k < 6; ++k) q6[6 * i + k] = rec[8 * i + k];
    return NBODY_OK;
}

}
```

nbody-llm_amd/csrc/nbody_f32.h:

```cpp
#pragma once
#include "nbody_handle.h"

namespace nbody32 {

EngineBodies<float>& bodies(NbodyHandle* h);
const EngineBodies<float>& bodies(const NbodyHandle* h);

int create(NbodyHandle* h);
void destroy(NbodyHandle* h);
int clone_state(NbodyHandle* src, NbodyHandle* dst);
int upload(NbodyHandle* h, const void* aos, size_t n, size_t stride);
int download(NbodyHandle* h, void* aos, size_t cap, size_t stride, size_t* n_out);
int count(NbodyHandle* h, size_t* n_out);
int count_global(NbodyHandle* h, size_t* n_out);
int add_point(NbodyHandle* h, const void* particle);
int remove_point(NbodyHandle* h, size_t index);
int merge_contacts(NbodyHandle* h, double radius, NbodyContact* list, size_t cap, size_t* n_contacts);
int init(NbodyHandle* h);
int step_by(NbodyHandle* h, float dt);
int steps(NbodyHandle* h, int k);
int update_forces(NbodyHandle* h);
int stats(NbodyHandle* h, NbodyStats* out);
int reset_stats(NbodyHandle* h);
int energy(NbodyHandle* h, double* kinetic, double* potential);
int tree_export_quadrupoles(NbodyHandle* h, float* q6, size_t cap, size_t* n_nodes);

int resolve_async(NbodyHandle* h);

int step_begin(NbodyHandle* h, float dt);
int step_forces(NbodyHandle* h, float dt);
int step_finish(NbodyHandle* h, float dt);
int debug_import_partials(NbodyHandle* h, NbodyHandle* peer);

}
```

nbody-llm_amd/csrc/real.h:

```cpp
#pragma once
#include "kernels.h"
#include "kernels_f64.h"

namespace nbody {

template <class F> struct Real;
template <> struct Real<float> : RealTypes<float> {
    static constexpr float half = 0.5f;
    static __device__ __forceinline__ V4 make4(float x, float y, float z, float w) { return make_float4(x, y, z, w); }
    static __device__ __forceinline__ float sqrt(float x) { return __builtin_sqrtf(x); }
    static __device__ __forceinline__ float rsqrt(float x) { return __builtin_amdgcn_rsqf(x); }
};
template <> struct Real<double> : RealTypes<double> {
    static constexpr double half = 0.5;
    static __device__ __forceinline__ V4 make4(double x, double y, double z, double w) { return make_double4(x, y, z, w); }
    static __device__ __forceinline__ double sqrt(double x) { return __builtin_sqrt(x); }
    static __device__ __forceinline__ double rsqrt(double x) { return ::rsqrt(x); }
};

__device__ __forceinline__ double4 widen(const double4 p) { return p; }
__device__ __forceinline__ double4 widen(const float4 p) { return make_double4(double(p.x), double(p.y), double(p.z), double(p.w)); }

template <class V4, class F>
__device__ __forceinline__ void kick_half_drift(V4* __restrict__ pos, V4* __restrict__ vel, int b, F ax, F ay, F az, F dt) {
    V4 p = pos[b], v = vel[b];
    v.x += ax * dt;
    v.y += ay * dt;
    v.z += az * dt;
    p.x += (v.x * Real<F>::half) * dt;
    p.y += (v.y * Real<F>::half) * dt;
    p.z += (v.z * Real<F>::half) * dt;
    vel[b] = v;
    pos[b] = p;
}

}
```

Measured before the change: 5984 billion.

## Fuse next step's half-drift and bounds check into force reduce tail, defer compaction

When brute-force single-shard stepping runs several steps, the reduce kernel now applies the kick, the next step's half-drift and the escape check in one pass. This removes the separate drift and compact launches. If a body escapes, a device poison flag makes the following kernels exit early, and the host later replays the affected steps. This removes per-step kernel launches and global-memory passes, at the cost of speculative execution, extra poison checks, and a complex rollback path that also touches stats and event bookkeeping.

```diff
diff --git a/nbody-llm_amd/csrc/kernels.h b/nbody-llm_amd/csrc/kernels.h
--- a/nbody-llm_amd/csrc/kernels.h
+++ b/nbody-llm_amd/csrc/kernels.h
@@ -20,6 +20,7 @@
     int sym_k = 0;
     int sym_min_bodies = 1024;
     int sym_reduce_split = 1;
+    int bf_step_fuse = 1;
     int sym_opp_rot = 1;
     int cross_slots = 3072;
     int cross_ipt = 0;
@@ -79,8 +80,9 @@
 void launch_bf_sym_main(hipStream_t s, const Shard& sh, const SymPlan& p, const int* d_bounds, float4* planes,
                         int n_upper, float g_soft2);
 void launch_bf_os(hipStream_t s, const Shard& sh, int A, int K, float4* planes, size_t plane_stride, float g_soft2);
+struct SymNext { BoundsF bounds; int tag; };
 void launch_bf_sym_tail(hipStream_t s, const Shard& sh, const SymPlan& p, float4* planes, int n_upper, float g,
-                        float g_soft2, const float* kick_dt);
+                        float g_soft2, const float* kick_dt, const SymNext* next = nullptr);
 
 struct CrossPartners {
     static constexpr int kMax = 8;
diff --git a/nbody-llm_amd/csrc/kernels_bf_sym.hip b/nbody-llm_amd/csrc/kernels_bf_sym.hip
--- a/nbody-llm_amd/csrc/kernels_bf_sym.hip
+++ b/nbody-llm_amd/csrc/kernels_bf_sym.hip
@@ -26,7 +26,8 @@
 __global__ __launch_bounds__(WPB * 64) void k_bf_sym(const float4* __restrict__ pos, const int* __restrict__ count,
                                                      int A, int K, const int* __restrict__ bounds, int n_trav, int opp,
                                                      float4* __restrict__ planes, size_t plane_stride, float eps2,
-                                                     int res_combine) {
+                                                     int res_combine, const int* __restrict__ poison) {
+    if (poison && *poison) return;
     const int lane = threadIdx.x & 63;
     const int wslot = __builtin_amdgcn_readfirstlane(threadIdx.x >> 6);
     const int n_main_blocks = (A * K + WPB - 1) / WPB;
@@ -283,19 +284,47 @@
 
 template <int IPT>
 __global__ __launch_bounds__(512) void k_bf_sym_rest(const float4* __restrict__ pos, const int* __restrict__ count,
-                                                     int A, float4* __restrict__ plane, float eps2) {
+                                                     int A, float4* __restrict__ plane, float eps2, const int* __restrict__ poison) {
     __shared__ float red[7][3][64];
+    if (poison && *poison) return;
     sym_rest_block<IPT, 8>(pos, *count, A, 0, blockIdx.x, plane, eps2, red);
 }
 
-template <bool KICK>
+enum : int { kTailSum = 0, kTailKick = 1, kTailNext = 2 };
+struct NextDrift { BoundsF b; unsigned char* keep; int* escaped; int tag; };
+
+__device__ __forceinline__ bool tail_poisoned(const int* poison, int own_tag) {
+    if (!poison) return false;
+    const int flags = *poison;
+    return flags != 0 && flags != own_tag;
+}
+
+template <int MODE>
+__device__ __forceinline__ void tail_body(int i, const float4 a, float4* __restrict__ acc, float4* __restrict__ pos,
+                                          float4* __restrict__ vel, float dt, const NextDrift& nx, int* __restrict__ poison) {
+    acc[i] = a;
+    if (MODE == kTailKick) kick_half_drift(pos, vel, i, a.x, a.y, a.z, dt);
+    if (MODE == kTailNext) {
+        float4 p = pos[i], v = vel[i];
+        kick_half_drift(p, v, a.x, a.y, a.z, dt);
+        vel[i] = v;
+        const bool in = half_drift_contains(p, v, dt, nx.b);
+        pos[i] = p;
+        nx.keep[i] = in ? 1 : 0;
+        if (!in) { atomicAdd(nx.escaped, 1); atomicOr(poison, nx.tag); }
+    }
+}
+
+template <int MODE>
 __global__ __launch_bounds__(256) void k_bf_sym_reduce(const float4* __restrict__ planes, int n_planes,
                                                        size_t plane_stride, const int* __restrict__ count, float g,
                                                        float4* __restrict__ acc, float4* __restrict__ pos,
                                                        float4* __restrict__ vel, float dt, const int* __restrict__ seg_count,
                                                        int n_seg, unsigned long long* __restrict__ inter, int opp_plane,
-                                                       int opp_first) {
+                                                       int opp_first, int* __restrict__ poison, const NextDrift nx) {
+    if (tail_poisoned(poison, MODE == kTailNext ? nx.tag : 0)) return;
     const int i = blockIdx.x * 256 + threadIdx.x;
+    if (MODE != kTailSum && poison && i == 0) atomicAdd(poison + 1, 1);
     if (inter && i == 0) {
         long long tot = 0;
         for (int s = 0; s < n_seg; ++s) tot += seg_count[s];
@@ -312,19 +341,21 @@
         sx = tx; sy = ty; sz = tz;
     }
     const float4 a = make_float4(g * sx, g * sy, g * sz, 0.f);
-    acc[i] = a;
-    if (KICK) kick_half_drift(pos, vel, i, a.x, a.y, a.z, dt);
-}
-
-template <bool KICK, int Q>
+    tail_body<MODE>(i, a, acc, pos, vel, dt, nx, poison);
+}
+
+template <int MODE, int Q>
 __global__ __launch_bounds__(64 * Q) void k_bf_sym_reduce_split(const float4* __restrict__ planes, int n_planes, size_t plane_stride,
                                                                 const int* __restrict__ count, float g, float4* __restrict__ acc,
                                                                 float4* __restrict__ pos, float4* __restrict__ vel, float dt,
                                                                 const int* __restrict__ seg_count, int n_seg,
-                                                                unsigned long long* __restrict__ inter, int opp_plane, int opp_first) {
+                                                                unsigned long long* __restrict__ inter, int opp_plane, int opp_first,
+                                                                int* __restrict__ poison, const NextDrift nx) {
     __shared__ float part[Q][3][64];
+    if (tail_poisoned(poison, MODE == kTailNext ? nx.tag : 0)) return;
     const int lane = threadIdx.x & 63, q = threadIdx.x >> 6;
     const int i = blockIdx.x * 64 + lane;
+    if (MODE != kTailSum && poison && blockIdx.x == 0 && threadIdx.x == 0) atomicAdd(poison + 1, 1);
     if (inter && blockIdx.x == 0 && threadIdx.x == 0) {
         long long tot = 0;
         for (int s = 0; s < n_seg; ++s) tot += seg_count[s];
@@ -354,8 +385,7 @@
         sx = tx; sy = ty; sz = tz;
     }
     const float4 a = make_float4(g * sx, g * sy, g * sz, 0.f);
-    acc[i] = a;
-    if (KICK) kick_half_drift(pos, vel, i, a.x, a.y, a.z, dt);
+    tail_body<MODE>(i, a, acc, pos, vel, dt, nx, poison);
 }
 
 }
@@ -441,14 +471,14 @@
     const int main_blocks = (p.A * p.K + p.wpb - 1) / p.wpb;
     const int rest_blocks = int(p.n_pad / 64);
     const dim3 grid(main_blocks + rest_blocks), block(p.wpb * 64);
-#define SYM_LAUNCH(WPB, DBG) hipLaunchKernelGGL((k_bf_sym<8, WPB, DBG, PKV>), grid, block, 0, s, sh.own_pos(), sh.own_count(), p.A, p.K, d_bounds, p.n_trav, p.opp, planes, p.plane_stride, g_soft2, p.res_combine)
+#define SYM_LAUNCH(WPB, DBG) hipLaunchKernelGGL((k_bf_sym<8, WPB, DBG, PKV>), grid, block, 0, s, sh.own_pos(), sh.own_count(), p.A, p.K, d_bounds, p.n_trav, p.opp, planes, p.plane_stride, g_soft2, p.res_combine, sh.poison)
 #ifdef NBODY_TUNING
     const int dbg = tuning().sym_debug;
 #else
     constexpr int dbg = 0;
 #endif
     if (p.ipt == 4) {
-        hipLaunchKernelGGL((k_bf_sym<4, 4, 0, true>), grid, block, 0, s, sh.own_pos(), sh.own_count(), p.A, p.K, d_bounds, p.n_trav, p.opp, planes, p.plane_stride, g_soft2, p.res_combine);
+        hipLaunchKernelGGL((k_bf_sym<4, 4, 0, true>), grid, block, 0, s, sh.own_pos(), sh.own_count(), p.A, p.K, d_bounds, p.n_trav, p.opp, planes, p.plane_stride, g_soft2, p.res_combine, sh.poison);
         return;
     }
     if (tuning().sym_packed) {
@@ -487,36 +517,40 @@
                            sh.seg_count, sh.n_seg, sh.seg_cap, sh.my_seg, A, K, planes, plane_stride, g_soft2);
 }
 
+namespace {
+template <int MODE>
+void launch_reduce(hipStream_t s, const Shard& sh, const SymPlan& p, float4* planes, int n_upper, float g, float dt, const NextDrift& nx) {
+#define REDUCE_ARGS planes, p.n_planes, p.plane_stride, sh.own_count(), g, sh.acc, sh.own_pos(), sh.vel, dt, sh.seg_count, sh.n_seg, sh.inter, (p.opp ? p.n_trav - 1 : -1), int(p.n_pad / 2), sh.poison, nx
+    if (tuning().sym_reduce_split && p.n_planes >= 16) {
+        const dim3 grid((n_upper + 63) / 64);
+        if (n_upper <= 16384) hipLaunchKernelGGL((k_bf_sym_reduce_split<MODE, 16>), grid, dim3(1024), 0, s, REDUCE_ARGS);
+        else hipLaunchKernelGGL((k_bf_sym_reduce_split<MODE, 4>), grid, dim3(256), 0, s, REDUCE_ARGS);
+    } else {
+        hipLaunchKernelGGL(k_bf_sym_reduce<MODE>, dim3((n_upper + 255) / 256), dim3(256), 0, s, REDUCE_ARGS);
+    }
+#undef REDUCE_ARGS
+}
+}
+
 void launch_bf_sym_tail(hipStream_t s, const Shard& sh, const SymPlan& p, float4* planes, int n_upper, float g,
-                        float g_soft2, const float* kick_dt) {
+                        float g_soft2, const float* kick_dt, const SymNext* next) {
     if (n_upper <= 0) return;
     if (p.sym_sets == 0) {
         float4* resident0 = planes + size_t(p.n_trav) * p.plane_stride;
         (void)hipMemsetAsync(resident0, 0, size_t(p.k_res) * p.plane_stride * sizeof(float4), s);
         if (p.ipt == 4)
             hipLaunchKernelGGL(k_bf_sym_rest<4>, dim3(int(p.n_pad / 64)), dim3(512), 0, s, sh.own_pos(),
-                               sh.own_count(), p.A, planes + size_t(p.n_trav + p.k_res) * p.plane_stride, g_soft2);
+                               sh.own_count(), p.A, planes + size_t(p.n_trav + p.k_res) * p.plane_stride, g_soft2, sh.poison);
         else
         hipLaunchKernelGGL(k_bf_sym_rest<8>, dim3(int(p.n_pad / 64)), dim3(512), 0, s, sh.own_pos(),
-                           sh.own_count(), p.A, planes + size_t(p.n_trav + p.k_res) * p.plane_stride, g_soft2);
-    }
-    const float dt = kick_dt ? *kick_dt : 0.f;
-#define REDUCE_ARGS planes, p.n_planes, p.plane_stride, sh.own_count(), g, sh.acc, sh.own_pos(), sh.vel, dt, sh.seg_count, sh.n_seg, sh.inter, (p.opp ? p.n_trav - 1 : -1), int(p.n_pad / 2)
-    if (tuning().sym_reduce_split && p.n_planes >= 16) {
-        const dim3 grid((n_upper + 63) / 64);
-        if (n_upper <= 16384) {
-            if (kick_dt) hipLaunchKernelGGL((k_bf_sym_reduce_split<true, 16>), grid, dim3(1024), 0, s, REDUCE_ARGS);
-            else hipLaunchKernelGGL((k_bf_sym_reduce_split<false, 16>), grid, dim3(1024), 0, s, REDUCE_ARGS);
-        } else {
-            if (kick_dt) hipLaunchKernelGGL((k_bf_sym_reduce_split<true, 4>), grid, dim3(256), 0, s, REDUCE_ARGS);
-            else hipLaunchKernelGGL((k_bf_sym_reduce_split<false, 4>), grid, dim3(256), 0, s, REDUCE_ARGS);
-        }
-    } else {
-        const dim3 grid((n_upper + 255) / 256);
-        if (kick_dt) hipLaunchKernelGGL(k_bf_sym_reduce<true>, grid, dim3(256), 0, s, REDUCE_ARGS);
-        else hipLaunchKernelGGL(k_bf_sym_reduce<false>, grid, dim3(256), 0, s, REDUCE_ARGS);
-    }
-#undef REDUCE_ARGS
-}
-
-}
+                           sh.own_count(), p.A, planes + size_t(p.n_trav + p.k_res) * p.plane_stride, g_soft2, sh.poison);
+    }
+    NextDrift nx{};
+    if (kick_dt && next && sh.poison) {
+        nx.b = next->bounds; nx.keep = sh.keep; nx.escaped = sh.escaped; nx.tag = next->tag;
+        launch_reduce<kTailNext>(s, sh, p, planes, n_upper, g, *kick_dt, nx);
+    } else if (kick_dt) launch_reduce<kTailKick>(s, sh, p, planes, n_upper, g, *kick_dt, nx);
+    else launch_reduce<kTailSum>(s, sh, p, planes, n_upper, g, 0.f, nx);
+}
+
+}
diff --git a/nbody-llm_amd/csrc/kernels_integrate.hip b/nbody-llm_amd/csrc/kernels_integrate.hip
--- a/nbody-llm_amd/csrc/kernels_integrate.hip
+++ b/nbody-llm_amd/csrc/kernels_integrate.hip
@@ -39,13 +39,8 @@
     const int k = blockIdx.x * 256 + threadIdx.x;
     if (k >= *count) return;
     typename Real<F>::V4 p = pos[k];
-    const typename Real<F>::V4 v = vel[k];
-    p.x += (v.x * Real<F>::half) * dt;
-    p.y += (v.y * Real<F>::half) * dt;
-    p.z += (v.z * Real<F>::half) * dt;
+    const bool in = half_drift_contains(p, vel[k], dt, b);
     pos[k] = p;
-    const bool in = (p.x >= b.lo[0]) && (p.x <= b.hi[0]) && (p.y >= b.lo[1]) && (p.y <= b.hi[1]) &&
-                    (p.z >= b.lo[2]) && (p.z <= b.hi[2]);
     keep[k] = in ? 1 : 0;
     if (!in) atomicAdd(escaped, 1);
 }
diff --git a/nbody-llm_amd/csrc/nbody_api.cpp b/nbody-llm_amd/csrc/nbody_api.cpp
--- a/nbody-llm_amd/csrc/nbody_api.cpp
+++ b/nbody-llm_amd/csrc/nbody_api.cpp
@@ -40,6 +40,12 @@
     nbody::bind_tuning(&h->tune);
     HIP_TRY(h, hipSetDevice(h->device));
     return NBODY_OK;
+}
+
+int settle_chain(NbodyHandle* h) {
+    if (!nbody32::chain_pending(h)) return NBODY_OK;
+    const int rc = use_device(h);
+    return rc ? rc : nbody32::settle_chain(h);
 }
 
 int check_stride(NbodyHandle* h, size_t stride) {
@@ -177,6 +183,7 @@
         const struct { const char* env; int* knob; } table[] = {
             {"NBODY_BF_VARIANT", &t.bf_fast_variant}, {"NBODY_CROSS_SYM", &t.cross_sym}, {"NBODY_SYM_PACKED", &t.sym_packed},
             {"NBODY_BH_SPLIT", &t.bh_walk_split}, {"NBODY_SYM_WPB", &t.sym_wpb}, {"NBODY_SYM_IPT", &t.sym_ipt}, {"NBODY_BH_DUO", &t.bh_walk_duo}, {"NBODY_BH_XCD", &t.bh_walk_xcd},
+            {"NBODY_BF_STEP_FUSE", &t.bf_step_fuse},
 #ifdef NBODY_TUNING
             {"NBODY_BH_VARIANT", &t.bh_walk_variant}, {"NBODY_BH_HOT", &t.bh_hot_cap}, {"NBODY_BH_LDS_BLOCK", &t.bh_walk_lds_block},
 #endif
@@ -289,6 +296,7 @@
 int nbody_set_settings_f64(NbodyHandle* h, double g, double g_soft, double dt, double theta2) {
     if (!h) return NBODY_ERR_INVALID;
     if (h->f64) return nbody64::set_settings(h, g, g_soft, dt, theta2);
+    if (int rc = settle_chain(h)) return rc;
     nbody32::bodies(h).set_settings(float(g), float(g_soft), float(dt), float(theta2));
     return NBODY_OK;
 }
@@ -310,6 +318,7 @@
 int nbody_set_bounds_f64(NbodyHandle* h, const double center[3], double width) {
     if (!h || !center) return NBODY_ERR_INVALID;
     if (h->f64) return nbody64::set_bounds(h, center, width);
+    if (int rc = settle_chain(h)) return rc;
     const float c[3] = {float(center[0]), float(center[1]), float(center[2])};
     nbody32::bodies(h).set_bounds(c, float(width));
     return NBODY_OK;
@@ -1039,7 +1048,7 @@
     {"bf_fast_variant", &nbody::Tuning::bf_fast_variant, false}, {"sym_wpb", &nbody::Tuning::sym_wpb, false}, {"sym_ipt", &nbody::Tuning::sym_ipt, false}, {"let_list_div", &nbody::Tuning::let_list_div, false}, {"bh_walk_duo", &nbody::Tuning::bh_walk_duo, false}, {"bh_walk_xcd", &nbody::Tuning::bh_walk_xcd, false},
     {"sym_rounds", &nbody::Tuning::sym_rounds, false}, {"sym_k", &nbody::Tuning::sym_k, false},
     {"sym_min_bodies", &nbody::Tuning::sym_min_bodies, false}, {"sym_reduce_split", &nbody::Tuning::sym_reduce_split, false},
-    {"sym_opp_rot", &nbody::Tuning::sym_opp_rot, false},
+    {"sym_opp_rot", &nbody::Tuning::sym_opp_rot, false}, {"bf_step_fuse", &nbody::Tuning::bf_step_fuse, false},
     {"cross_slots", &nbody::Tuning::cross_slots, false}, {"cross_ipt", &nbody::Tuning::cross_ipt, false},
     {"cross_wpb", &nbody::Tuning::cross_wpb, false}, {"bh_walk_split", &nbody::Tuning::bh_walk_split, false},
     {"bh_walk_order", &nbody::Tuning::bh_walk_order, false}, {"bh_reduce_split", &nbody::Tuning::bh_reduce_split, false},
@@ -1062,6 +1071,7 @@
 #endif
             if (h->comm_ready && (std::strcmp(name, "cross_sym") == 0 || std::strcmp(name, "sym_packed") == 0 || std::strcmp(name, "bf_fast_variant") == 0))
                 return fail(h, NBODY_ERR_INVALID, std::string("nbody_set_tuning: '") + name + "' is part of what the ranks agreed on at nbody_comm_init: set it before");
+            if (int rc = settle_chain(h)) return rc;
             h->tune.*(k.field) = value;
             return NBODY_OK;
         }
diff --git a/nbody-llm_amd/csrc/nbody_f32.cpp b/nbody-llm_amd/csrc/nbody_f32.cpp
--- a/nbody-llm_amd/csrc/nbody_f32.cpp
+++ b/nbody-llm_amd/csrc/nbody_f32.cpp
@@ -37,8 +37,15 @@
     bool tracer_kick = false;
 
     bool async_bh = false;
-    struct PendingStep { float dt; float elapsed_before; };
+    struct PendingStep {
+        float dt; float elapsed_before;
+        bool next;
+        size_t ev_mark; unsigned tick; uint64_t timed;
+    };
     std::vector<PendingStep> pending;
+    bool next_pending = false;
+    bool drift_done = false;
+    bool resolving = false;
     bool last_step_async = false;
     bool host_tree_once = false;
 
@@ -148,6 +155,18 @@
 }
 
 constexpr size_t kShardedSymMinBodies = 2048;
+
+bool sym_single(const NbodyHandle* h) {
+    const State& s = *h->f32;
+    return h->cfg.math_mode == NBODY_MATH_FAST && nbody::tuning().bf_fast_variant == 0 &&
+           s.n_local >= size_t(std::max(1024, nbody::tuning().sym_min_bodies));
+}
+
+bool bf_chain(const NbodyHandle* h) {
+    const State& s = *h->f32;
+    return nbody::tuning().bf_step_fuse != 0 && h->cfg.method == NBODY_BRUTE_FORCE && s.sh.n_seg == 1 && !h->let && !h->comm_ready &&
+           sym_single(h) && !nbody::tracer::on(h) && !nbody::ext::on(h);
+}
 
 int ensure_sym_plan(NbodyHandle* h) {
     State& s = *h->f32;
@@ -200,7 +219,7 @@
     const float eps2 = s.g_soft * s.g_soft;
     const bool fast = h->cfg.math_mode == NBODY_MATH_FAST && nbody::tuning().bf_fast_variant == 0;
     const bool sharded = s.sh.n_seg > 1;
-    const bool sym = fast && (sharded ? size_t(s.sh.seg_cap) >= kShardedSymMinBodies : s.n_local >= size_t(std::max(1024, nbody::tuning().sym_min_bodies)));
+    const bool sym = sharded ? fast && size_t(s.sh.seg_cap) >= kShardedSymMinBodies : sym_single(h);
     const size_t tot = total_upper(s);
     if (sym) {
         int rc = ensure_sym_plan(h);
@@ -264,7 +283,7 @@
 int bh_walk_device_tree_async(NbodyHandle* h);
 int bh_walk_host_tree(NbodyHandle* h);
 int step_end(NbodyHandle* h, float dt);
-int step_impl(NbodyHandle* h, float dt);
+int step_impl(NbodyHandle* h, float dt, bool next = false);
 
 int setup_nested_walk(NbodyHandle* h, nbody::TreeDev* td) {
     State& s = *h->f32;
@@ -539,9 +558,12 @@
     if (!s.tail_pending) return NBODY_OK;
     s.tail_pending = false;
     const float eps2 = s.g_soft * s.g_soft;
+    const bool next = s.next_pending && s.kick_pending && bf_chain(h);
+    const nbody::SymNext nx{s.bnd, 4 | (int(s.pending.size()) << 8)};
     nbody::launch_bf_sym_tail(h->stream, s.sh, s.sym_plan, s.d_planes, int(s.n_local), s.g, eps2,
-                              s.kick_pending ? &s.kick_dt : nullptr);
+                              s.kick_pending ? &s.kick_dt : nullptr, next ? &nx : nullptr);
     s.kick_pending = false;
+    s.drift_done = next;
     HIP_TRY(h, hipGetLastError());
     return NBODY_OK;
 }
@@ -566,18 +588,31 @@
     return step_finish(h, dt);
 }
 
-int step_impl(NbodyHandle* h, float dt) {
-    State& s = *h->f32;
-    const float elapsed_before = s.elapsed;
-    int rc = step_begin(h, dt);
+int step_impl(NbodyHandle* h, float dt, bool next) {
+    State& s = *h->f32;
+    int rc = NBODY_OK;
+    const bool chain = bf_chain(h);
+    if (!s.async_bh) {
+        if (!s.resolving && !s.pending.empty() && (!chain || h->ev_pending.size() + 1 >= 4096)) {
+            rc = resolve_async(h);
+            if (!rc) rc = drain_events(h);
+            if (rc) return rc;
+        }
+        s.sh.poison = chain ? h->d_poison : nullptr;
+        if (chain && s.pending.empty()) HIP_TRY(h, hipMemsetAsync(h->d_poison + 1, 0, sizeof(int), h->stream));
+    }
+    const State::PendingStep before{dt, s.elapsed, chain && next, h->ev_pending.size(), h->profile_tick, h->stats.force_kernel_interactions};
+    rc = step_begin(h, dt);
     if (rc) return rc;
     rc = exchange_begin(h);
     if (rc) return rc;
+    s.next_pending = before.next;
     rc = step_end(h, dt);
-    if (rc) return rc;
-    if (s.last_step_async) {
-        s.pending.push_back(State::PendingStep{dt, elapsed_before});
-        if (s.pending.size() >= 4096) rc = resolve_async(h);
+    s.next_pending = false;
+    if (rc) return rc;
+    if (s.last_step_async || chain) {
+        s.pending.push_back(before);
+        if (s.pending.size() >= 4096 && !s.resolving) rc = resolve_async(h);
     }
     return rc;
 }
@@ -742,8 +777,42 @@
     return NBODY_OK;
 }
 
+int resolve_chain(NbodyHandle* h) {
+    State& s = *h->f32;
+    for (int round = 0; round < 1000000; ++round) {
+        HIP_TRY(h, hipMemcpyAsync(h->h_poison, h->d_poison, 2 * sizeof(int), hipMemcpyDeviceToHost, h->stream));
+        HIP_TRY(h, hipStreamSynchronize(h->stream));
+        const int flags = h->h_poison[0], done = h->h_poison[1];
+        if (!flags) { s.pending.clear(); return NBODY_OK; }
+        std::vector<State::PendingStep> rest;
+        if (size_t(done) < s.pending.size()) rest.assign(s.pending.begin() + done, s.pending.end());
+        s.pending.clear();
+        HIP_TRY(h, hipMemsetAsync(h->d_poison, 0, 2 * sizeof(int), h->stream));
+        nbody::launch_compact(h->stream, s.sh, int(s.n_local));
+        HIP_TRY(h, hipGetLastError());
+        if (rest.empty()) return NBODY_OK;
+        s.elapsed = rest[0].elapsed_before;
+        h->stats.steps -= rest.size();
+        h->stats.force_kernel_interactions = rest[0].timed;
+        h->profile_tick = rest[0].tick;
+        while (h->ev_pending.size() > rest[0].ev_mark) { h->ev_free.push_back(h->ev_pending.back()); h->ev_pending.pop_back(); }
+        s.resolving = true;
+        s.drift_done = true;
+        int rc = NBODY_OK;
+        for (size_t k = 0; k < rest.size() && !rc; ++k) rc = step_impl(h, rest[k].dt, rest[k].next);
+        s.resolving = false;
+        s.drift_done = false;
+        if (rc) return rc;
+    }
+    return fail(h, NBODY_ERR_INVALID, "resolve_async did not converge");
+}
+
+bool chain_pending(const NbodyHandle* h) { return h->f32 && !h->f32->async_bh && !h->f32->pending.empty(); }
+int settle_chain(NbodyHandle* h) { return chain_pending(h) ? resolve_chain(h) : NBODY_OK; }
+
 int resolve_async(NbodyHandle* h) {
-    if (!h->f32 || !h->f32->async_bh) return NBODY_OK;
+    if (!h->f32) return NBODY_OK;
+    if (!h->f32->async_bh) return h->f32->pending.empty() ? NBODY_OK : resolve_chain(h);
     State& s = *h->f32;
     for (int round = 0; round < 1000000; ++round) {
         HIP_TRY(h, hipMemcpyAsync(h->h_poison, h->d_poison, 2 * sizeof(int), hipMemcpyDeviceToHost, h->stream));
@@ -788,8 +857,12 @@
 int step_begin(NbodyHandle* h, float dt) {
     State& s = *h->f32;
     if (!s.bounds_set) return fail(h, NBODY_ERR_INVALID, "nbody_set_bounds has not been called");
-    nbody::launch_drift_half(h->stream, s.sh, int(s.n_local), dt, s.bnd);
-    nbody::launch_compact(h->stream, s.sh, int(s.n_local));
+    const bool drifted = s.drift_done && bf_chain(h);
+    s.drift_done = false;
+    if (!drifted) {
+        nbody::launch_drift_half(h->stream, s.sh, int(s.n_local), dt, s.bnd);
+        nbody::launch_compact(h->stream, s.sh, int(s.n_local));
+    }
     s.count_dirty = true;
     HIP_TRY(h, hipGetLastError());
     if (nbody::tracer::on(h)) return nbody::tracer::drift_retain(h, dt);
@@ -855,8 +928,8 @@
 int steps(NbodyHandle* h, int k) {
     State& s = *h->f32;
     for (int i = 0; i < k; ++i) {
-        int rc = step_impl(h, s.dt);
-        if (rc) return rc;
+        int rc = step_impl(h, s.dt, i + 1 < k);
+        if (rc) { s.drift_done = false; return rc; }
     }
     return NBODY_OK;
 }
diff --git a/nbody-llm_amd/csrc/nbody_f32.h b/nbody-llm_amd/csrc/nbody_f32.h
--- a/nbody-llm_amd/csrc/nbody_f32.h
+++ b/nbody-llm_amd/csrc/nbody_f32.h
@@ -26,6 +26,8 @@
 int tree_export_quadrupoles(NbodyHandle* h, float* q6, size_t cap, size_t* n_nodes);
 
 int resolve_async(NbodyHandle* h);
+bool chain_pending(const NbodyHandle* h);
+int settle_chain(NbodyHandle* h);
 
 int step_begin(NbodyHandle* h, float dt);
 int step_forces(NbodyHandle* h, float dt);
diff --git a/nbody-llm_amd/csrc/real.h b/nbody-llm_amd/csrc/real.h
--- a/nbody-llm_amd/csrc/real.h
+++ b/nbody-llm_amd/csrc/real.h
@@ -22,16 +22,28 @@
 __device__ __forceinline__ double4 widen(const float4 p) { return make_double4(double(p.x), double(p.y), double(p.z), double(p.w)); }
 
 template <class V4, class F>
-__device__ __forceinline__ void kick_half_drift(V4* __restrict__ pos, V4* __restrict__ vel, int b, F ax, F ay, F az, F dt) {
-    V4 p = pos[b], v = vel[b];
+__device__ __forceinline__ void kick_half_drift(V4& p, V4& v, F ax, F ay, F az, F dt) {
     v.x += ax * dt;
     v.y += ay * dt;
     v.z += az * dt;
     p.x += (v.x * Real<F>::half) * dt;
     p.y += (v.y * Real<F>::half) * dt;
     p.z += (v.z * Real<F>::half) * dt;
+}
+template <class V4, class F>
+__device__ __forceinline__ void kick_half_drift(V4* __restrict__ pos, V4* __restrict__ vel, int b, F ax, F ay, F az, F dt) {
+    V4 p = pos[b], v = vel[b];
+    kick_half_drift(p, v, ax, ay, az, dt);
     vel[b] = v;
     pos[b] = p;
 }
 
+template <class V4, class F, class B>
+__device__ __forceinline__ bool half_drift_contains(V4& p, const V4& v, F dt, const B& b) {
+    p.x += (v.x * Real<F>::half) * dt;
+    p.y += (v.y * Real<F>::half) * dt;
+    p.z += (v.z * Real<F>::half) * dt;
+    return (p.x >= b.lo[0]) && (p.x <= b.hi[0]) && (p.y >= b.lo[1]) && (p.y <= b.hi[1]) && (p.z >= b.lo[2]) && (p.z <= b.hi[2]);
 }
+
+}
```

After: 6019 billion, median of 6. About the same (+0.6%).
